# fujii-team/Henbun

Hardware: AMD Instinct MI355X
Metric: elbo_samples_per_sec (higher is better)
Workload: dtype f32; 1 GPU; cfg2 SVGP ELBO step: 1-D UnitRBF, N=1e6, M=512 inducing, minibatch 8192 per GPU, diag Normal q(u), diagonal residual, Adam lr 1e-3; global_batch=8192, per_gpu_batch=8192, parallelism=dp1, N=1000000, M=512, dp_exchange=none, dp_ranks=1, contraction=native, tri_pack=False

## Files before the change

henbun_amd/_lib.py:

```python
from __future__ import annotations

import ctypes
import os
from ctypes import c_char_p, c_double, c_int, c_long, c_uint64, c_void_p

_HERE = os.path.dirname(os.path.abspath(__file__))
LIB_PATH = os.path.join(_HERE, "libhenbun_hip.so")


class HipBackendError(RuntimeError):
    """A libhenbun_hip.so entry point returned a non-zero status."""


P, L, I, D, U64 = c_void_p, c_long, c_int, c_double, c_uint64

_SIGS = {
    "hb_version": [],
    "hb_debug_set": [c_char_p, L],
    "hb_debug_clear": [],
    "hb_cholesky_inverse_ws_elems": [L, L, I],
    "hb_cholesky_persistent_shape": [L, L, I],
    "hb_mlp2_sample_supported": [L, L, L, L, L, I],
    "hb_mlp2_sample_ws_elems": [L, L, L],
    "hb_mlp2_sample_fwd_f32": [P, P, P, P, P, I, P, P, L, P, P, P, P, L, L, L, P, P],
    "hb_mlp2_sample_bwd_f32": [P, P, P, P, I, P, P, P, P, P, P, P, P, P, L, L, L, P, P],
    "hb_gram_cholesky_inverse_f32": [I, P, L, P, L, L, L, D, P, P, L, L, P, P, P, I, P],
    "hb_last_error_string": [],
    "hb_device_info": [P, I, P],
    "hb_graph_begin_capture": [P],
    "hb_graph_end_capture": [P, P],
    "hb_graph_launch": [P, P],
    "hb_graph_destroy": [P],
    "hb_rng_init": [P, L, U64, U64, P],
    "hb_rng_randint": [P, L, P, L, L, L, P],
    "hb_sgp_ws_elems": [L, L, L, L, L],
    "hb_sgp_strip_path": [L, L, L, L, L, I],
    "hb_sgp_head_units": [L, L, L, L, L, I, I, I, L],
    "hb_sgp_rider_supported": [L, L, L, L, L, I, I, I, L],
    "hb_sgp_predict_ws_elems": [L, L, L, L, L, I, I, I],
    "hb_sgp_predict_cov_ws_elems": [L, L, L, L, I, I],
    "hb_sgp_stats_ws_elems": [L, L, L, L, I],
    "hb_sgp_select_ws_elems": [L, L, L, I],
    "hb_sgp_kgrad_ws_elems": [L, L, L, L],
    "hb_matmul_gauss_units": [L, L, L],
    "hb_matmul_gram_vjp_ok": [L, L, L, L],
    "hb_matmul_gram_vjp_ws_elems": [L, L, L],
    "hb_matmul_gram_vjp_f32": [P, P, P, L, L, L, L, L, L, L, L, L, I, I, P, L, P, L, L, L, P, P, P, P, P],
    "hb_fullrank_one_launch_shape": [L, L],
    "hb_matmul_gauss_f32": [P, L, P, L, P, P, P, P, D, P, P, P, L, L, L, L, P],
    "hb_sgp_rider_begin": [],
    "hb_sgp_rider_pending": [],
    "hb_sgp_rider_flush": [P],
    "hb_sgp_fwd_gauss_f32": [I, I, P, L, P, P, L, P, P, I, P, P, P, L, P, P, P, P, P, L, L, L, L, L, P, P, P, P, D, P, P, P, L, P],
    "hb_ewise_prog_image_bytes": [],
    "hb_ewise_prog_build": [I, P, P, I, P, P, I, P, P, P, I, P, P, P, P],
    "hb_ewise_jit_available": [],
    "hb_ewise_jit_run": [P, P],
    "hb_ewise_jit_destroy": [P],
    "hb_side_push_gather_draw_f32": [I, P, P, P, L, P, L, L, L, P, P, L, P, P],
    "hb_side_push_diag_fwd_f32": [P, P, P, P, L, P, P, P, L, L, L, L, P, P],
    "hb_side_push_diag_bwd_f32": [P, P, P, P, P, P, P, L, L, L, L, P],
    "hb_side_pending": [],
    "hb_side_flush": [P],
    "hb_side_discard": [],
    "hb_chain_begin": [],
    "hb_chain_end": [P],
    "hb_chain_discard": [],
    "hb_chain_source": [P, L],
    "hb_chain_compile_dry": [],
    "hb_comm_available": [],
    "hb_comm_unique_id": [P],
    "hb_comm_init": [P, I, I, P],
    "hb_comm_destroy": [P],
}
_RESTYPES = {"hb_last_error_string": c_char_p, "hb_sgp_ws_elems": c_long, "hb_ewise_prog_image_bytes": c_long,
             "hb_sgp_head_units": c_long, "hb_matmul_gauss_units": c_long, "hb_matmul_gram_vjp_ws_elems": c_long, "hb_cholesky_inverse_ws_elems": c_long, "hb_mlp2_sample_ws_elems": c_long,
             "hb_sgp_predict_ws_elems": c_long, "hb_sgp_predict_cov_ws_elems": c_long,
             "hb_sgp_stats_ws_elems": c_long, "hb_sgp_select_ws_elems": c_long,
             "hb_sgp_kgrad_ws_elems": c_long}

_TYPED = {
    "hb_ewise": [I, I, P, P, I, P, I, P, P, P],
    "hb_ewise_prog": [I, P, P, I, P, P, I, P, P, P, I, P, P],
    "hb_ewise_prog_run": [P, L, I, P],
    "hb_ewise_jit_build": [I, P, P, I, P, P, I, P, P, P, I, P, P, P, P, P, L],
    "hb_ewise_colprog_build": [I, P, P, I, P, P, I, P, P, P, L, L, P, P, L],
    "hb_gauss_ll": [P, P, P, P, L, P, P, P, P, P, L, P],
    "hb_gauss_ll_post": [P, P, P, P, L, P, P, P, P, D, P, P, L, P],
    "hb_gauss_ll_fold": [P, L, P, P, P, P],
    "hb_reduce": [I, P, P, L, L, L, P, L, P],
    "hb_copy_nd": [P, P, P, P, I, P, P],
    "hb_fill": [P, L, D, P],
    "hb_gather_rows": [P, L, L, P, P, L, P, P, P],
    "hb_gather_rows_multi": [I, P, P, P, L, P, P, L, P, P],
    "hb_gather_rows_multi_draw": [I, P, P, P, L, P, L, L, L, P, P, L, P, P],
    "hb_matutil": [P, P, L, L, L, I, L, L, D, P],
    "hb_rng_normal": [P, L, P, L, P],
    "hb_diag_sample_kl_fwd": [P, P, P, P, L, P, P, P, L, L, L, L, P, P],
    "hb_diag_sample_kl_bwd": [P, P, P, P, P, P, P, L, L, L, L, P],
    "hb_fullrank_sample_kl_fwd": [P, P, P, P, L, P, P, P, L, L, I, P, P],
    "hb_fullrank_sample_kl_fwd1": [P, P, P, P, L, P, P, P, L, L, I, P, P, P],
    "hb_fullrank_sample_kl_bwd": [P, P, P, P, P, P, P, L, L, I, P],
    "hb_vec_to_tri": [P, P, L, L, P],
    "hb_tri_to_vec": [P, P, L, L, P],
    "hb_gram_fwd": [I, P, L, P, L, P, L, L, P, L, L, L, L, D, P],
    "hb_gram_bwd": [I, P, L, P, L, P, L, L, P, P, P, P, L, L, L, L, P, P],
    "hb_gram_ell_fold": [P, L, L, L, L, P, P],
    "hb_matmul": [P, P, P, L, L, L, L, L, L, L, L, L, L, I, I, D, D, P, L, I, I, P, L, P],
    "hb_matmul_colsum": [P, P, P, P, L, L, L, L, L, L, P, L, P],
    "hb_cholesky": [P, P, L, L, P, P],
    "hb_cholesky_inverse": [P, P, P, L, L, P, P, P, I, P],
    "hb_trinv": [P, P, L, L, P, P],
    "hb_sgp_A": [I, P, L, P, P, L, P, P, I, P, L, L, L, L, P],
    "hb_sgp_fwd": [I, I, P, L, P, P, L, P, P, I, P, P, P, L, P, P, P, P, P, L, L, L, L, L, P, P],
    "hb_sgp_bwd": [I, I, P, L, P, P, L, P, P, I, P, P, P, P, P, P, P, P, P, P, P, P, P, L, L, L, L, L, P, P],
    "hb_sgp_predict": [I, P, L, P, P, L, P, P, P, P, I, I, D, P, P, L, L, L, L, L, P, P],
    "hb_sgp_predict_cov": [I, P, L, P, P, L, P, P, P, I, I, D, P, L, L, L, L, L, P, P],
    "hb_sgp_stats": [I, P, P, P, P, L, P, P, P, P, P, P, L, L, L, L, P, P],
    "hb_sgp_select": [I, P, P, L, L, L, L, D, P, P, P, P, P, P],
    "hb_sgp_kgrad": [I, P, P, P, P, L, P, P, P, P, L, L, L, L, P, P],
    "hb_adam_step": [P, P, P, P, L, D, D, D, D, D, P, I, P, L, P, P, P],
    "hb_allreduce_sum": [P, L, P, P],
    "hb_dp_pack": [P, P, P, L, P],
}


def declared_symbols():
    names = list(_SIGS)
    for base in _TYPED:
        names += [base + "_f32", base + "_f64"]
    return names


class _Lib:
    def __init__(self, path: str):
        if not os.path.exists(path):
            raise ImportError(
                "henbun_amd: %s is missing.  Build it with `python -m henbun_amd._build` "
                "(hipcc, gfx950).  There is no CPU fallback." % path
            )
        import torch

        self._dll = ctypes.CDLL(path)
        self._fns = {}
        for name, args in _SIGS.items():
            self._bind(name, args, _RESTYPES.get(name, c_int))
        for base, args in _TYPED.items():
            for suf in ("_f32", "_f64"):
                self._bind(base + suf, args, c_int)
        if self.raw("hb_version")() != 2:
            raise ImportError("henbun_amd: ABI version mismatch in " + path)

    def _bind(self, name, args, restype):
        fn = getattr(self._dll, name)
        fn.argtypes = args
        fn.restype = restype
        self._fns[name] = fn

    def raw(self, name):
        return self._fns[name]

    def last_error(self) -> str:
        s = self._fns["hb_last_error_string"]()
        return s.decode() if s else ""

    def call(self, name, *args):
        rc = self._fns[name](*args)
        if rc != 0:
            raise HipBackendError("%s failed (status %d): %s" % (name, rc, self.last_error()))
        return 0


_lib = None


def lib() -> _Lib:
    global _lib
    if _lib is None:
        _lib = _Lib(LIB_PATH)
    return _lib
```

henbun_amd/csrc/adam.hip:

```cpp
#include "common.cuh"
#include "../../include/henbun_hip.h"
#include "chain.cuh"

template <typename T>
__global__ void __launch_bounds__(256) adam_kernel(T* __restrict__ theta, const T* __restrict__ g, T* __restrict__ m,
                                                   T* __restrict__ v, long n, double lr, double b1, double b2,
                                                   double eps, double gscale, long* t, int tick, const int* info,
                                                   long n_info, const T* dpflag, long* fail) {
  hb_adam_body<T>(theta, g, m, v, n, lr, b1, b2, eps, gscale, t, tick, info, n_info, dpflag, fail,
                  (long)blockIdx.x * blockDim.x + threadIdx.x, (long)gridDim.x * blockDim.x, blockIdx.x == 0, gridDim.x == 1);
}

template <typename T>
__global__ void __launch_bounds__(256) adam_vec_kernel(T* __restrict__ theta, const T* __restrict__ g, T* __restrict__ m,
                                                       T* __restrict__ v, long n, double lr, double b1, double b2,
                                                       double eps, double gscale, long* t, const int* info, long n_info,
                                                       const T* dpflag, long* fail) {
  hb_adam_body_vec<T>(theta, g, m, v, n, lr, b1, b2, eps, gscale, t, info, n_info, dpflag, fail,
                      (long)blockIdx.x * blockDim.x + threadIdx.x, (long)gridDim.x * blockDim.x, blockIdx.x == 0);
}

template <typename T>
__global__ void __launch_bounds__(64) adam_tick_kernel(long* t, const int* info, long n_info, const T* dpflag,
                                                       const long* fail) {
  if (adam_step_blocked<T>(t, info, n_info, dpflag, const_cast<long*>(fail), false)) return;
  if (threadIdx.x == 0 && blockIdx.x == 0) t[0] += 1;
}

template <typename T>
static int adam_launch(T* theta, const T* g, T* m, T* v, long n, double lr, double b1, double b2, double eps,
                       double gscale, long* t, int tick, const int* info, long n_info, const T* dpflag, long* fail,
                       hipStream_t stream) {
  HB_REQUIRE(n >= 0, "hb_adam_step: n < 0");
  HB_REQUIRE(theta && g && m && v && t, "hb_adam_step: NULL pointer");
  HB_REQUIRE(n_info >= 0 && (n_info == 0 || info != nullptr), "hb_adam_step: info/n_info");
  int grid = 0;
  if (hb_chain_recording()) {
    if (n > 0 && n <= HB_CHAIN_ADAM_MAX_N) {
      HbChainJob j;
      j.kind = HB_CHAIN_ADAM;
      j.is64 = sizeof(T) == 8;
      j.p[0] = theta, j.p[1] = g, j.p[2] = m, j.p[3] = v, j.p[4] = t, j.p[5] = info, j.p[6] = dpflag, j.p[7] = fail;
      j.l[0] = n, j.l[1] = n_info, j.l[2] = tick;
      j.d[0] = lr, j.d[1] = b1, j.d[2] = b2, j.d[3] = eps, j.d[4] = gscale;
      return hb_chain_push(j, stream);
    }
    const int crc = hb_chain_flush(stream);
    if (crc) return crc;
  }
  if (n > 0) {
    grid = n <= 2048 ? 1 : hb_stream_grid(n, 256);
    constexpr long VEC = 16 / (long)sizeof(T);
    const bool vec = grid > 1 && (((uintptr_t)theta | (uintptr_t)g | (uintptr_t)m | (uintptr_t)v) % 16) == 0;
    if (vec) {
      grid = hb_stream_grid(n / VEC, 256);
      hipLaunchKernelGGL(adam_vec_kernel<T>, dim3(grid), dim3(256), 0, stream, theta, g, m, v, n, lr, b1, b2, eps, gscale, t,
                         info, n_info, dpflag, fail);
      if (grid == 1) grid = 2;
    } else {
      hipLaunchKernelGGL(adam_kernel<T>, dim3(grid), dim3(256), 0, stream, theta, g, m, v, n, lr, b1, b2, eps, gscale, t,
                         tick, info, n_info, dpflag, fail);
    }
    HB_LAUNCH_CHECK();
  }
  if (grid != 1 && tick) {
    hipLaunchKernelGGL(adam_tick_kernel<T>, dim3(1), dim3(64), 0, stream, t, info, n_info, dpflag, fail);
    HB_LAUNCH_CHECK();
  }
  return 0;
}

extern "C" int hb_adam_step_f32(float* theta, const float* g, float* m, float* v, long n, double lr, double b1,
                                double b2, double eps, double gscale, long* t, int tick, const int* info, long n_info,
                                const float* dpflag, long* fail, void* stream) {
  return adam_launch<float>(theta, g, m, v, n, lr, b1, b2, eps, gscale, t, tick, info, n_info, dpflag, fail,
                            (hipStream_t)stream);
}
extern "C" int hb_adam_step_f64(double* theta, const double* g, double* m, double* v, long n, double lr, double b1,
                                double b2, double eps, double gscale, long* t, int tick, const int* info, long n_info,
                                const double* dpflag, long* fail, void* stream) {
  return adam_launch<double>(theta, g, m, v, n, lr, b1, b2, eps, gscale, t, tick, info, n_info, dpflag, fail,
                             (hipStream_t)stream);
}
```

henbun_amd/csrc/chain.cuh:

```cuda
#ifndef HB_CHAIN_CUH
#define HB_CHAIN_CUH
#include "common.cuh"
#include "ew_prog.cuh"

enum { HB_CHAIN_PROG = 1, HB_CHAIN_ADAM = 2, HB_CHAIN_GLL = 3, HB_CHAIN_SGP_FINISH = 4, HB_CHAIN_GRAM_ELL = 5, HB_CHAIN_GLL_FOLD = 6 };
#define HB_CHAIN_MAX_JOBS 6
#define HB_CHAIN_PROG_MAX_N 4096
#define HB_CHAIN_FINISH_MAX_N 512
#define HB_CHAIN_GLL_MAX_N 4096
#define HB_CHAIN_ADAM_MAX_N 4096
#define HB_CHAIN_ELL_MAX_N 16384
#define HB_CHAIN_GLL_FOLD_MAX_N 4096

struct HbChainJob {
  int kind = 0, is64 = 0;
  const void* p[HB_PROG_MAX_IN + HB_PROG_MAX_OUT] = {};
  long l[8] = {};
  double d[8] = {};
  ProgArgs prog;
  int reduces = 0;
};

bool hb_chain_recording();
int hb_chain_push(const HbChainJob& job, hipStream_t stream);
int hb_chain_flush(hipStream_t stream);

#endif
```

henbun_amd/csrc/chain_bodies.cuh:

```cuda
#ifndef HB_CHAIN_BODIES_CUH
#define HB_CHAIN_BODIES_CUH

#pragma clang fp contract(off)

template <typename T>
__device__ __forceinline__ int adam_step_blocked(const long* t, const int* info, long n_info, const T* dpflag,
                                                 long* fail, bool record) {
  int bad = 0, what = 0;
  if (fail != nullptr && fail[0] != 0) bad = 1;
  if (dpflag != nullptr && dpflag[0] != (T)0) { bad = 1; what = -1; }
  for (long i = threadIdx.x; i < n_info; i += blockDim.x) {
    const int w = info[i];
    if (w != 0) { bad = 1; what = w; }
  }
  const int any = __syncthreads_or(bad);
  if (any && record && fail != nullptr) {
    __shared__ int who;
    if (threadIdx.x == 0) who = blockDim.x;
    __syncthreads();
    if (what != 0) atomicMin(&who, (int)threadIdx.x);
    __syncthreads();
    const int writer = who == (int)blockDim.x ? 0 : who;
    if ((int)threadIdx.x == writer && fail[0] == 0) {
      fail[1] = (long)what;
      fail[0] = t[0] + 1;
    }
  }
  return any;
}

template <typename T>
__device__ __forceinline__ void hb_adam_body(T* __restrict__ theta, const T* __restrict__ g, T* __restrict__ m, T* __restrict__ v,
                                             long n, double lr, double b1, double b2, double eps, double gscale, long* t,
                                             int tick, const int* info, long n_info, const T* dpflag, long* fail, long i0,
                                             long stride, bool record, bool owner) {
  constexpr int U = 8;
  T g0[U], m0[U], v0[U], th0[U];
#pragma unroll
  for (int k = 0; k < U; ++k) {
    const long i = i0 + k * stride, ic = i < n ? i : (n > 0 ? n - 1 : 0);
    g0[k] = g[ic], m0[k] = m[ic], v0[k] = v[ic], th0[k] = theta[ic];
  }
  const long tnow = t[0];
  if (adam_step_blocked<T>(t, info, n_info, dpflag, fail, record)) return;
  const double tt = (double)(tnow + 1);
  const T lr_t = (T)(lr * sqrt(1.0 - pow(b2, tt)) / (1.0 - pow(b1, tt)));
  const T c1 = (T)b1, c2 = (T)b2, d1 = (T)(1.0 - b1), d2 = (T)(1.0 - b2), e = (T)eps, gs = (T)gscale;
#pragma unroll
  for (int k = 0; k < U; ++k) {
    const long i = i0 + k * stride;
    if (i < n) {
      const T gi = g0[k] * gs;
      const T mi = c1 * m0[k] + d1 * gi;
      const T vi = c2 * v0[k] + d2 * gi * gi;
      m[i] = mi;
      v[i] = vi;
      theta[i] = th0[k] - lr_t * mi / (hb_sqrt(vi) + e);
    }
  }
  for (long i = i0 + U * stride; i < n; i += stride) {
    const T gi = g[i] * gs;
    const T mi = c1 * m[i] + d1 * gi;
    const T vi = c2 * v[i] + d2 * gi * gi;
    m[i] = mi;
    v[i] = vi;
    theta[i] -= lr_t * mi / (hb_sqrt(vi) + e);
  }
  if (owner && tick) {
    __syncthreads();
    if (threadIdx.x == 0) t[0] += 1;
  }
}

template <typename T>
__device__ __forceinline__ void hb_adam_body_vec(T* __restrict__ theta, const T* __restrict__ g, T* __restrict__ m, T* __restrict__ v,
                                                 long n, double lr, double b1, double b2, double eps, double gscale, long* t,
                                                 const int* info, long n_info, const T* dpflag, long* fail, long i0, long stride,
                                                 bool record) {
  constexpr int VEC = 16 / (int)sizeof(T), U = 2;
  typedef T VT __attribute__((ext_vector_type(VEC)));
  const long nv = n / VEC;
  VT g0[U], m0[U], v0[U], th0[U];
#pragma unroll
  for (int k = 0; k < U; ++k) {
    const long i = i0 + k * stride, ic = i < nv ? i : (nv > 0 ? nv - 1 : 0);
    g0[k] = reinterpret_cast<const VT*>(g)[ic], m0[k] = reinterpret_cast<const VT*>(m)[ic];
    v0[k] = reinterpret_cast<const VT*>(v)[ic], th0[k] = reinterpret_cast<const VT*>(theta)[ic];
  }
  const long tnow = t[0];
  if (adam_step_blocked<T>(t, info, n_info, dpflag, fail, record)) return;
  const double tt = (double)(tnow + 1);
  const T lr_t = (T)(lr * sqrt(1.0 - pow(b2, tt)) / (1.0 - pow(b1, tt)));
  const T c1 = (T)b1, c2 = (T)b2, d1 = (T)(1.0 - b1), d2 = (T)(1.0 - b2), e = (T)eps, gs = (T)gscale;
  auto upd = [&](VT gv, VT mv, VT vv, VT tv, long i) {
    VT mo, vo, to;
#pragma unroll
    for (int q = 0; q < VEC; ++q) {
      const T gi = gv[q] * gs;
      const T mi = c1 * mv[q] + d1 * gi;
      const T vi = c2 * vv[q] + d2 * gi * gi;
      mo[q] = mi, vo[q] = vi, to[q] = tv[q] - lr_t * mi / (hb_sqrt(vi) + e);
    }
    reinterpret_cast<VT*>(m)[i] = mo;
    reinterpret_cast<VT*>(v)[i] = vo;
    reinterpret_cast<VT*>(theta)[i] = to;
  };
#pragma unroll
  for (int k = 0; k < U; ++k) {
    const long i = i0 + k * stride;
    if (i < nv) upd(g0[k], m0[k], v0[k], th0[k], i);
  }
  for (long i = i0 + U * stride; i < nv; i += stride)
    upd(reinterpret_cast<const VT*>(g)[i], reinterpret_cast<const VT*>(m)[i], reinterpret_cast<const VT*>(v)[i],
        reinterpret_cast<const VT*>(theta)[i], i);
  const long it = nv * VEC + i0;
  if (it < n) {
    const T gi = g[it] * gs;
    const T mi = c1 * m[it] + d1 * gi;
    const T vi = c2 * v[it] + d2 * gi * gi;
    m[it] = mi;
    v[it] = vi;
    theta[it] -= lr_t * mi / (hb_sqrt(vi) + e);
  }
}

template <typename T>
__device__ __forceinline__ void hb_gauss_ll_single_body(const T* __restrict__ x, const T* __restrict__ f, const T* __restrict__ scale,
                                                        const T* __restrict__ var, long n, T* __restrict__ dmu, T* __restrict__ ll,
                                                        T* __restrict__ dscale, T* __restrict__ dvar, T* smem,
                                                        T* __restrict__ fbar = nullptr, T post = T(0)) {
  constexpr int PER = 16;
  const T s = scale ? scale[0] : T(1), v = var[0];
  const T iv = T(1) / v, lc = T(-0.91893853320467274178) - T(0.5) * hb_log(v);
  T xv[PER], fv[PER];
#pragma unroll
  for (int q = 0; q < PER; ++q) {
    const long j = q * 1024 + threadIdx.x;
    const long jc = j < n ? j : n - 1;
    xv[q] = x[jc];
    fv[q] = f[jc];
  }
  T all = T(0), asc = T(0), avr = T(0);
#pragma unroll
  for (int q = 0; q < PER; ++q) {
    const long j = q * 1024 + threadIdx.x;
    const T dlt = xv[q] - fv[q] * s;
    const T g = dlt * iv;
    if (j < n) {
      dmu[j] = g;
      if (fbar) fbar[j] = s * (post * g);
      all += lc - T(0.5) * dlt * g;
      asc += g * fv[q];
      avr += T(-0.5) * iv + T(0.5) * g * g;
    }
  }
  all = block_sum(all, smem);
  asc = block_sum(asc, smem);
  avr = block_sum(avr, smem);
  if (threadIdx.x == 0) {
    ll[0] = all;
    dscale[0] = asc;
    dvar[0] = avr;
  }
}

template <typename T>
__device__ __forceinline__ void hb_gauss_point(T xv, T fv, T s, T iv, T lc, T& g, T& all, T& asc, T& avr) {
  const T dlt = xv - fv * s;
  g = dlt * iv;
  all += lc - T(0.5) * dlt * g;
  asc += g * fv;
  avr += T(-0.5) * iv + T(0.5) * g * g;
}

template <typename T>
__device__ __forceinline__ void hb_gauss_fold_body(const T* __restrict__ partial, long nb, T* __restrict__ ll, T* __restrict__ dscale,
                                                   T* __restrict__ dvar, T* smem) {
  T a0 = T(0), a1 = T(0), a2 = T(0);
  for (long i = threadIdx.x; i < nb; i += blockDim.x) {
    a0 += partial[i];
    a1 += partial[nb + i];
    a2 += partial[2 * nb + i];
  }
  a0 = block_sum(a0, smem);
  a1 = block_sum(a1, smem);
  a2 = block_sum(a2, smem);
  if (threadIdx.x == 0) {
    ll[0] = a0;
    dscale[0] = a1;
    dvar[0] = a2;
  }
}

template <typename T>
__device__ __forceinline__ void sgp_finish_one(const T* __restrict__ part, int gy, long idx, T epsv, T* __restrict__ f,
                                               T* __restrict__ v, T* __restrict__ eps_out, long n, long P, int diagonal) {
  const long e = idx / n, j = idx - e * n;
  const T* pp = part + e * gy * 5 * n + j;
  T s = T(0);
  for (int y = 0; y < gy; ++y) s += pp[(long)y * 5 * n];
  const T vv = T(1) - s;
  v[idx] = vv;
  if (eps_out) eps_out[idx] = epsv;
  const T scale = diagonal ? hb_sqrt(hb_abs(vv)) * epsv : T(0);
  for (long p = 0; p < P; ++p) {
    T mean = T(0);
    for (int y = 0; y < gy; ++y) mean += pp[((long)y * 5 + 1 + p) * n];
    f[(e * P + p) * n + j] = mean + scale;
  }
}

template <typename T>
__device__ __forceinline__ void hb_sgp_finish_body(const T* __restrict__ part, int gy, const T* __restrict__ eps_in, uint64_t* rng,
                                                   long nlanes, T* __restrict__ eps_out, T* __restrict__ f, T* __restrict__ v,
                                                   long total, long n, long P, int diagonal, long t0, long nthreads) {
  const long npairs = (total + 1) / 2;
  if (rng) {
    const long nact = nlanes < npairs ? nlanes : npairs;
    for (long t = t0; t < nact; t += nthreads) {
      HbRng g = rng_load(rng, nlanes, t);
      for (long p = t; p < npairs; p += nlanes) {
        T z0, z1;
        g.normal2(z0, z1);
        sgp_finish_one<T>(part, gy, 2 * p, z0, f, v, eps_out, n, P, diagonal);
        if (2 * p + 1 < total) sgp_finish_one<T>(part, gy, 2 * p + 1, z1, f, v, eps_out, n, P, diagonal);
      }
      rng_store(rng, nlanes, t, g);
    }
  } else {
    for (long idx = t0; idx < total; idx += nthreads)
      sgp_finish_one<T>(part, gy, idx, eps_in ? eps_in[idx] : T(0), f, v, (eps_out != eps_in) ? eps_out : nullptr, n, P, diagonal);
  }
}

template <typename T>
__device__ __forceinline__ void hb_gram_ell_body(const T* __restrict__ partial, long rows, long d, long dl, long c,
                                                 T* __restrict__ ellbar, T* smem) {
  T acc = T(0);
  if (dl == 1) {
#pragma unroll 4
    for (long t = threadIdx.x; t < rows * d; t += blockDim.x) acc += partial[t];
  } else {
#pragma unroll 4
    for (long r = threadIdx.x; r < rows; r += blockDim.x) acc += partial[r * d + c];
  }
  acc = block_sum(acc, smem);
  if (threadIdx.x == 0) ellbar[c] = acc;
}

#pragma clang fp contract(fast)
#endif
```

henbun_amd/csrc/elementwise.hip:

```cpp
#include "common.cuh"
#include "rng_pairs.cuh"
#include "side_jobs.cuh"
#include <string.h>
#include "../../include/henbun_hip.h"

struct EwArgs {
  int ndim;
  int nin, nout;
  int op;
  long n;
  int shape[HB_MAX_DIMS];
  long istride[4][HB_MAX_DIMS];
  const void* in[4];
  void* out[3];
  double p[4];
};

#include "ew_apply.cuh"

template <typename T>
__global__ void __launch_bounds__(256) ew_kernel(EwArgs A) {
  const long stride = (long)gridDim.x * blockDim.x;
  for (long i = (long)blockIdx.x * blockDim.x + threadIdx.x; i < A.n; i += stride) {
    long off[4] = {0, 0, 0, 0};
// ... 487 lines not shown
    A.shape[d] = 1;
    A.is[d] = A.os[d] = 0;
  }
  A.ndim = nd;
  A.n = n;
  hipLaunchKernelGGL(copy_nd_kernel<T>, dim3(hb_stream_grid(n, 256)), dim3(256), 0, stream, in, out, A);
  HB_LAUNCH_CHECK();
  return 0;
}

extern "C" int hb_copy_nd_f32(const float* in, const long* istr, float* out, const long* ostr, int ndim,
                              const long* shape, void* stream) {
  return copy_nd_launch<float>(in, istr, out, ostr, ndim, shape, (hipStream_t)stream);
}
extern "C" int hb_copy_nd_f64(const double* in, const long* istr, double* out, const long* ostr, int ndim,
                              const long* shape, void* stream) {
  return copy_nd_launch<double>(in, istr, out, ostr, ndim, shape, (hipStream_t)stream);
}

template <typename T>
__global__ void __launch_bounds__(256) fill_kernel(T* out, long n, T v) {
  const long stride = (long)gridDim.x * blockDim.x;
  for (long i = (long)blockIdx.x * blockDim.x + threadIdx.x; i < n; i += stride) out[i] = v;
}
extern "C" int hb_fill_f32(float* out, long n, double v, void* stream) {
  if (n <= 0) return 0;
  hipLaunchKernelGGL(fill_kernel<float>, dim3(hb_stream_grid(n, 256)), dim3(256), 0, (hipStream_t)stream, out, n, (float)v);
  HB_LAUNCH_CHECK();
  return 0;
}
extern "C" int hb_fill_f64(double* out, long n, double v, void* stream) {
  if (n <= 0) return 0;
  hipLaunchKernelGGL(fill_kernel<double>, dim3(hb_stream_grid(n, 256)), dim3(256), 0, (hipStream_t)stream, out, n, v);
  HB_LAUNCH_CHECK();
  return 0;
}

template <typename T>
__global__ void __launch_bounds__(256) gather_rows_kernel(const T* __restrict__ src, const long* __restrict__ idx,
                                                          const long* __restrict__ perm, T* __restrict__ dst,
                                                          long n, long row, long nsrc, int* __restrict__ err) {
  const long total = n * row;
  const long stride = (long)gridDim.x * blockDim.x;
  for (long i = (long)blockIdx.x * blockDim.x + threadIdx.x; i < total; i += stride) {
    const long r = i / row, c = i - r * row;
    long j = idx[r];
    if (perm) j = perm[j];
    if (j < 0 || j >= nsrc) {
      if (err) *err = 1;
      dst[i] = T(0);
    } else {
      dst[i] = src[j * row + c];
    }
  }
}
extern "C" int hb_gather_rows_f32(const float* src, long nsrc, long row, const long* idx, const long* perm, long n,
                                  float* dst, int* err, void* stream) {
  HB_REQUIRE(n >= 0 && row >= 0 && nsrc >= 0, "hb_gather_rows: negative extent");
  if (n * row == 0) return 0;
  hipLaunchKernelGGL(gather_rows_kernel<float>, dim3(hb_stream_grid(n * row, 256)), dim3(256), 0, (hipStream_t)stream,
                     src, idx, perm, dst, n, row, nsrc, err);
  HB_LAUNCH_CHECK();
  return 0;
}
extern "C" int hb_gather_rows_f64(const double* src, long nsrc, long row, const long* idx, const long* perm, long n,
                                  double* dst, int* err, void* stream) {
  HB_REQUIRE(n >= 0 && row >= 0 && nsrc >= 0, "hb_gather_rows: negative extent");
  if (n * row == 0) return 0;
  hipLaunchKernelGGL(gather_rows_kernel<double>, dim3(hb_stream_grid(n * row, 256)), dim3(256), 0,
                     (hipStream_t)stream, src, idx, perm, dst, n, row, nsrc, err);
  HB_LAUNCH_CHECK();
  return 0;
}

template <typename T>
__global__ void __launch_bounds__(256) gather_rows_multi_kernel(GatherMultiArgs<T> g, const long* __restrict__ idx,
                                                                const long* __restrict__ perm, long n, long nsrc,
                                                                int* __restrict__ err) {
  const long total = g.start[g.narr];
  const long stride = (long)gridDim.x * blockDim.x;
  for (long i = (long)blockIdx.x * blockDim.x + threadIdx.x; i < total; i += stride) {
    int a = 0;
#pragma unroll
    for (int q = 1; q < HB_GATHER_MAX; ++q)
      if (q < g.narr && i >= g.start[q]) a = q;
    const long li = i - g.start[a];
    const long r = li / g.row[a], c = li - r * g.row[a];
    long j = idx[r];
    if (perm) j = perm[j];
    if (j < 0 || j >= nsrc) {
      if (err) *err = 1;
      g.dst[a][li] = T(0);
    } else {
      g.dst[a][li] = g.src[a][j * g.row[a] + c];
    }
  }
}
template <typename T>
static int gather_rows_multi(int narr, const T* const* srcs, const long* rows, T* const* dsts, long nsrc,
                             const long* idx, const long* perm, long n, int* err, hipStream_t stream) {
  HB_REQUIRE(narr >= 1 && narr <= HB_GATHER_MAX, "hb_gather_rows_multi: %d arrays (max %d)", narr, HB_GATHER_MAX);
  HB_REQUIRE(n >= 0 && nsrc >= 0 && srcs && rows && dsts && idx, "hb_gather_rows_multi: bad arguments");
  GatherMultiArgs<T> g;
  g.narr = narr;
  g.start[0] = 0;
  for (int a = 0; a < HB_GATHER_MAX; ++a) {
    g.src[a] = a < narr ? srcs[a] : nullptr;
    g.dst[a] = a < narr ? dsts[a] : nullptr;
    g.row[a] = a < narr ? rows[a] : 1;
    if (a < narr) HB_REQUIRE(rows[a] >= 1 && srcs[a] && dsts[a], "hb_gather_rows_multi: bad array %d", a);
    g.start[a + 1] = g.start[a] + (a < narr ? n * rows[a] : 0);
  }
  if (g.start[narr] == 0) return 0;
  hipLaunchKernelGGL(gather_rows_multi_kernel<T>, dim3(hb_stream_grid(g.start[narr], 256)), dim3(256), 0, stream, g, idx,
                     perm, n, nsrc, err);
  HB_LAUNCH_CHECK();
  return 0;
}
extern "C" int hb_gather_rows_multi_f32(int narr, const float* const* srcs, const long* rows, float* const* dsts,
                                        long nsrc, const long* idx, const long* perm, long n, int* err, void* stream) {
  return gather_rows_multi<float>(narr, srcs, rows, dsts, nsrc, idx, perm, n, err, (hipStream_t)stream);
}
extern "C" int hb_gather_rows_multi_f64(int narr, const double* const* srcs, const long* rows, double* const* dsts,
                                        long nsrc, const long* idx, const long* perm, long n, int* err, void* stream) {
  return gather_rows_multi<double>(narr, srcs, rows, dsts, nsrc, idx, perm, n, err, (hipStream_t)stream);
}

template <typename T, int G>
__global__ void __launch_bounds__(256) gather_rows_multi_draw_kernel(GatherMultiArgs<T> g, uint64_t* __restrict__ state,
                                                                     long nlanes, long lo, uint64_t range,
                                                                     long* __restrict__ idx_out,
                                                                     const long* __restrict__ perm, long n, long nsrc,
                                                                     int* __restrict__ err) {
  gather_draw_body<T>(g, state, nlanes, lo, range, idx_out, perm, n, nsrc, err, G, (long)blockIdx.x);
}
template <typename T>
static int gather_rows_multi_draw(int narr, const T* const* srcs, const long* rows, T* const* dsts, long nsrc,
                                  uint64_t* state, long nlanes, long lo, long hi, long* idx_out, const long* perm,
                                  long n, int* err, hipStream_t stream, bool defer = false) {
  HB_REQUIRE(narr >= 1 && narr <= HB_GATHER_MAX, "hb_gather_rows_multi_draw: %d arrays (max %d)", narr, HB_GATHER_MAX);
  HB_REQUIRE(n >= 0 && nsrc >= 0 && srcs && rows && dsts && state && idx_out, "hb_gather_rows_multi_draw: bad arguments");
  HB_REQUIRE(n <= nlanes, "hb_gather_rows_multi_draw: n=%ld exceeds the %ld RNG lanes (draw with hb_rng_randint instead)", n,
             nlanes);
  HB_REQUIRE(hi > lo, "hb_gather_rows_multi_draw: empty range [%ld,%ld)", lo, hi);
  GatherMultiArgs<T> g;
  g.narr = narr;
  g.start[0] = 0;
  long wmax = 1;
  for (int a = 0; a < HB_GATHER_MAX; ++a) {
    g.src[a] = a < narr ? srcs[a] : nullptr;
    g.dst[a] = a < narr ? dsts[a] : nullptr;
    g.row[a] = a < narr ? rows[a] : 1;
    if (a < narr) HB_REQUIRE(rows[a] >= 1 && srcs[a] && dsts[a], "hb_gather_rows_multi_draw: bad array %d", a);
    if (a < narr && rows[a] > wmax) wmax = rows[a];
    g.start[a + 1] = g.start[a] + (a < narr ? n * rows[a] : 0);
  }
  if (n == 0) return 0;
  const uint64_t range = (uint64_t)(hi - lo);
  constexpr long VEC = 16 / (long)sizeof(T);
  bool vec16 = true;
  for (int a = 0; a < narr; ++a)
    vec16 = vec16 && rows[a] % VEC == 0 && ((uintptr_t)srcs[a] % 16) == 0 && ((uintptr_t)dsts[a] % 16) == 0;
  const long wsel = vec16 ? wmax / VEC : wmax;
  const int Gsel = wsel <= 2 ? 1 : (wsel <= 8 ? 4 : (wsel <= 32 ? 16 : 64));
  if constexpr (sizeof(T) == 4) {
    if (defer) {
      HbSideJob j;
      j.kind = HB_SIDE_GATHER_DRAW;
      j.gather.G = vec16 ? -Gsel : Gsel;
      j.nblocks = hb_cdiv(n * Gsel, 256);
      if (j.nblocks <= 1024) {
        memcpy(&j.gather.g, &g, sizeof(g));
        j.gather.state = state; j.gather.nlanes = nlanes; j.gather.lo = lo; j.gather.range = range;
        j.gather.idx_out = idx_out; j.gather.perm = perm; j.gather.n = n; j.gather.nsrc = nsrc; j.gather.err = err;
        return hb_side_push(j, stream);
      }
    }
  }
#define HB_GDRAW(G_)                                                                                                   \
  hipLaunchKernelGGL((gather_rows_multi_draw_kernel<T, G_>), dim3((unsigned)hb_cdiv(n * (G_ < 0 ? -(G_) : (G_)), 256)), dim3(256), 0, \
                     stream, g, state, nlanes, lo, range, idx_out, perm, n, nsrc, err)
  if (vec16) {
    if (Gsel == 1)
      HB_GDRAW(-1);
    else if (Gsel == 4)
      HB_GDRAW(-4);
    else if (Gsel == 16)
      HB_GDRAW(-16);
    else
      HB_GDRAW(-64);
  } else if (Gsel == 1)
    HB_GDRAW(1);
  else if (Gsel == 4)
    HB_GDRAW(4);
  else if (Gsel == 16)
    HB_GDRAW(16);
  else
    HB_GDRAW(64);
#undef HB_GDRAW
  HB_LAUNCH_CHECK();
  return 0;
}
extern "C" int hb_gather_rows_multi_draw_f32(int narr, const float* const* srcs, const long* rows, float* const* dsts,
                                             long nsrc, uint64_t* state, long nlanes, long lo, long hi, long* idx_out,
                                             const long* perm, long n, int* err, void* stream) {
  return gather_rows_multi_draw<float>(narr, srcs, rows, dsts, nsrc, state, nlanes, lo, hi, idx_out, perm, n, err,
                                       (hipStream_t)stream);
}
extern "C" int hb_side_push_gather_draw_f32(int narr, const float* const* srcs, const long* rows, float* const* dsts, long nsrc,
                                           uint64_t* state, long nlanes, long lo, long hi, long* idx_out, const long* perm,
                                           long n, int* err, void* stream) {
  return gather_rows_multi_draw<float>(narr, srcs, rows, dsts, nsrc, state, nlanes, lo, hi, idx_out, perm, n, err,
                                       (hipStream_t)stream, true);
}
extern "C" int hb_gather_rows_multi_draw_f64(int narr, const double* const* srcs, const long* rows, double* const* dsts,
                                             long nsrc, uint64_t* state, long nlanes, long lo, long hi, long* idx_out,
                                             const long* perm, long n, int* err, void* stream) {
  return gather_rows_multi_draw<double>(narr, srcs, rows, dsts, nsrc, state, nlanes, lo, hi, idx_out, perm, n, err,
                                        (hipStream_t)stream);
}

#define HB_GLL_BLOCK_ELEMS 1024
template <typename T>
__global__ void __launch_bounds__(256) gauss_ll_kernel(const T* __restrict__ x, const T* __restrict__ f,
                                                       const T* __restrict__ scale, const T* __restrict__ var,
                                                       long n, T* __restrict__ dmu, T* __restrict__ partial,
                                                       T* __restrict__ fbar, T post) {
  __shared__ T smem[16];
  const T s = scale ? scale[0] : T(1), v = var[0];
  const T iv = T(1) / v, lc = T(-0.91893853320467274178) - T(0.5) * hb_log(v);
  T all = T(0), asc = T(0), avr = T(0);
  const long base = (long)blockIdx.x * HB_GLL_BLOCK_ELEMS;
#pragma unroll
  for (int q = 0; q < HB_GLL_BLOCK_ELEMS / 256; ++q) {
    const long j = base + q * 256 + threadIdx.x;
    const long jc = j < n ? j : n - 1;
    const T xv = x[jc], fv = f[jc];
    const T dlt = xv - fv * s;
    const T g = dlt * iv;
    if (j < n) {
      dmu[j] = g;
      if (fbar) fbar[j] = s * (post * g);
      all += lc - T(0.5) * dlt * g;
      asc += g * fv;
      avr += T(-0.5) * iv + T(0.5) * g * g;
    }
  }
  all = block_sum(all, smem);
  asc = block_sum(asc, smem);
  avr = block_sum(avr, smem);
  if (threadIdx.x == 0) {
    partial[blockIdx.x] = all;
    partial[gridDim.x + blockIdx.x] = asc;
    partial[2 * gridDim.x + blockIdx.x] = avr;
  }
}
template <typename T>
__global__ void __launch_bounds__(256) gauss_ll_finish_kernel(const T* __restrict__ partial, int nb, T* __restrict__ ll,
                                                              T* __restrict__ dscale, T* __restrict__ dvar) {
  __shared__ T smem[16];
  T a0 = T(0), a1 = T(0), a2 = T(0);
  for (int i = threadIdx.x; i < nb; i += 256) {
    a0 += partial[i];
    a1 += partial[nb + i];
    a2 += partial[2 * nb + i];
  }
  a0 = block_sum(a0, smem);
  a1 = block_sum(a1, smem);
  a2 = block_sum(a2, smem);
  if (threadIdx.x == 0) {
    ll[0] = a0;
    dscale[0] = a1;
    dvar[0] = a2;
  }
}
#define HB_GLL_SINGLE_N 16384
template <typename T>
__global__ void __launch_bounds__(1024) gauss_ll_single_kernel(const T* __restrict__ x, const T* __restrict__ f,
                                                               const T* __restrict__ scale, const T* __restrict__ var,
                                                               long n, T* __restrict__ dmu, T* __restrict__ ll,
                                                               T* __restrict__ dscale, T* __restrict__ dvar,
                                                               T* __restrict__ fbar, T post) {
  __shared__ T smem[16];
  static_assert(HB_GLL_SINGLE_N == 16 * 1024, "hb_gauss_ll_single_body: 16 elements per thread of a 1024-thread workgroup");
  hb_gauss_ll_single_body<T>(x, f, scale, var, n, dmu, ll, dscale, dvar, smem, fbar, post);
}

template <typename T>
static int gauss_ll(const T* x, const T* f, const T* scale, const T* var, long n, T* ll, T* dmu, T* dscale, T* dvar,
                    T* ws, long ws_elems, hipStream_t stream, double post = 0.0, T* fbar = nullptr) {
  HB_REQUIRE(n >= 0 && x && f && var && ll && dmu && dscale && dvar && ws, "hb_gauss_ll: bad arguments");
  const int nb = n > 0 ? hb_cdiv(n, HB_GLL_BLOCK_ELEMS) : 0;
  HB_REQUIRE(ws_elems >= 3L * (nb > 0 ? nb : 1), "hb_gauss_ll: workspace of 3*ceil(n/%d) elements required",
             HB_GLL_BLOCK_ELEMS);
  if (hb_chain_recording()) {
    if (n > 0 && n <= HB_CHAIN_GLL_MAX_N) {
      HbChainJob j;
      j.kind = HB_CHAIN_GLL;
      j.is64 = sizeof(T) == 8;
      j.p[0] = x, j.p[1] = f, j.p[2] = scale, j.p[3] = var, j.p[4] = dmu, j.p[5] = ll, j.p[6] = dscale, j.p[7] = dvar;
      j.p[8] = fbar;
      j.l[0] = n;
      j.d[0] = post;
      return hb_chain_push(j, stream);
    }
    const int crc = hb_chain_flush(stream);
    if (crc) return crc;
  }
  if (n > 0 && n <= HB_GLL_SINGLE_N) {
    hipLaunchKernelGGL(gauss_ll_single_kernel<T>, dim3(1), dim3(1024), 0, stream, x, f, scale, var, n, dmu, ll, dscale,
                       dvar, fbar, (T)post);
    HB_LAUNCH_CHECK();
    return 0;
  }
  if (nb > 0) {
    hipLaunchKernelGGL(gauss_ll_kernel<T>, dim3(nb), dim3(256), 0, stream, x, f, scale, var, n, dmu, ws, fbar, (T)post);
    HB_LAUNCH_CHECK();
  }
  hipLaunchKernelGGL(gauss_ll_finish_kernel<T>, dim3(1), dim3(256), 0, stream, ws, nb, ll, dscale, dvar);
  HB_LAUNCH_CHECK();
  return 0;
}
extern "C" int hb_gauss_ll_f32(const float* x, const float* f, const float* scale, const float* var, long n, float* ll,
                               float* dmu, float* dscale, float* dvar, float* ws, long ws_elems, void* stream) {
  return gauss_ll<float>(x, f, scale, var, n, ll, dmu, dscale, dvar, ws, ws_elems, (hipStream_t)stream);
}
extern "C" int hb_gauss_ll_f64(const double* x, const double* f, const double* scale, const double* var, long n,
                               double* ll, double* dmu, double* dscale, double* dvar, double* ws, long ws_elems,
                               void* stream) {
  return gauss_ll<double>(x, f, scale, var, n, ll, dmu, dscale, dvar, ws, ws_elems, (hipStream_t)stream);
}
template <typename T>
__global__ void __launch_bounds__(256) gauss_fold_kernel(const T* __restrict__ partial, long nb, T* __restrict__ ll,
                                                         T* __restrict__ dscale, T* __restrict__ dvar) {
  __shared__ T smem[16];
  hb_gauss_fold_body<T>(partial, nb, ll, dscale, dvar, smem);
}
template <typename T>
static int gauss_fold(const T* partial, long nb, T* ll, T* dscale, T* dvar, hipStream_t stream) {
  HB_REQUIRE(partial && nb >= 1 && ll && dscale && dvar, "hb_gauss_ll_fold: bad arguments");
  if (hb_chain_recording()) {
    if (nb <= HB_CHAIN_GLL_FOLD_MAX_N) {
      HbChainJob j;
      j.kind = HB_CHAIN_GLL_FOLD;
      j.is64 = sizeof(T) == 8;
      j.p[0] = partial, j.p[1] = ll, j.p[2] = dscale, j.p[3] = dvar;
      j.l[0] = nb;
      return hb_chain_push(j, stream);
    }
    const int crc = hb_chain_flush(stream);
    if (crc) return crc;
  }
  hipLaunchKernelGGL(gauss_fold_kernel<T>, dim3(1), dim3(256), 0, stream, partial, nb, ll, dscale, dvar);
  HB_LAUNCH_CHECK();
  return 0;
}
extern "C" int hb_gauss_ll_fold_f32(const float* partial, long nb, float* ll, float* dscale, float* dvar, void* stream) {
  return gauss_fold<float>(partial, nb, ll, dscale, dvar, (hipStream_t)stream);
}
extern "C" int hb_gauss_ll_fold_f64(const double* partial, long nb, double* ll, double* dscale, double* dvar, void* stream) {
  return gauss_fold<double>(partial, nb, ll, dscale, dvar, (hipStream_t)stream);
}

extern "C" int hb_gauss_ll_post_f32(const float* x, const float* f, const float* scale, const float* var, long n, float* ll,
                                    float* dmu, float* dscale, float* dvar, double post, float* fbar, float* ws,
                                    long ws_elems, void* stream) {
  HB_REQUIRE(fbar, "hb_gauss_ll_post: fbar is NULL");
  return gauss_ll<float>(x, f, scale, var, n, ll, dmu, dscale, dvar, ws, ws_elems, (hipStream_t)stream, post, fbar);
}
extern "C" int hb_gauss_ll_post_f64(const double* x, const double* f, const double* scale, const double* var, long n,
                                    double* ll, double* dmu, double* dscale, double* dvar, double post, double* fbar,
                                    double* ws, long ws_elems, void* stream) {
  HB_REQUIRE(fbar, "hb_gauss_ll_post: fbar is NULL");
  return gauss_ll<double>(x, f, scale, var, n, ll, dmu, dscale, dvar, ws, ws_elems, (hipStream_t)stream, post, fbar);
}

template <typename T>
__global__ void __launch_bounds__(256) matutil_kernel(const T* __restrict__ in, T* __restrict__ out, long B, long R,
                                                      long C, int mode, long lower, long upper, T alpha) {
  const long total = B * R * C;
  const long stride = (long)gridDim.x * blockDim.x;
  for (long t = (long)blockIdx.x * blockDim.x + threadIdx.x; t < total; t += stride) {
    const long b = t / (R * C);
    const long rem = t - b * R * C;
    const long i = rem / C, j = rem - i * C;
    T v = in[t];
    if (mode == 0) {
      const bool keep = (lower < 0 || i - j <= lower) && (upper < 0 || j - i <= upper);
      v = keep ? v : T(0);
    } else if (mode == 1) {
      if (i == j) v += alpha;
    } else if (mode == 2) {
      v = (i > j) ? v : (i == j ? T(0.5) * v : T(0));
    } else if (mode == 3) {
      v = T(0.5) * (v + in[b * R * C + j * C + i]);
    } else if (mode == 4) {
      v = T(0.5) * (i >= j ? v : in[b * R * C + j * C + i]);
    }
    out[t] = v;
  }
}
template <typename T>
static int matutil_launch(const T* in, T* out, long B, long R, long C, int mode, long lower, long upper, double alpha,
                          hipStream_t stream) {
  HB_REQUIRE(B >= 0 && R >= 0 && C >= 0, "hb_matutil: negative extent");
  HB_REQUIRE(mode >= 0 && mode <= 4, "hb_matutil: bad mode %d", mode);
  HB_REQUIRE((mode != 3 && mode != 4) || (R == C && in != out), "hb_matutil: symmetrise needs square, out-of-place");
  const long n = B * R * C;
  if (n == 0) return 0;
  hipLaunchKernelGGL(matutil_kernel<T>, dim3(hb_stream_grid(n, 256)), dim3(256), 0, stream, in, out, B, R, C, mode,
                     lower, upper, (T)alpha);
  HB_LAUNCH_CHECK();
  return 0;
}
extern "C" int hb_matutil_f32(const float* in, float* out, long B, long R, long C, int mode, long lower, long upper,
                              double alpha, void* stream) {
  return matutil_launch<float>(in, out, B, R, C, mode, lower, upper, alpha, (hipStream_t)stream);
}
extern "C" int hb_matutil_f64(const double* in, double* out, long B, long R, long C, int mode, long lower, long upper,
                              double alpha, void* stream) {
  return matutil_launch<double>(in, out, B, R, C, mode, lower, upper, alpha, (hipStream_t)stream);
}
```

henbun_amd/csrc/gram.hip:

```cpp
#include "common.cuh"
#include "../../include/henbun_hip.h"
#include "chain.cuh"
#include "gram_value.cuh"

template <typename T>
__global__ void __launch_bounds__(256) gram_fwd_kernel(int kind, const T* __restrict__ X, long sX,
                                                       const T* __restrict__ X2, long sX2, const T* __restrict__ ell,
                                                       long sEll, long dl, T* __restrict__ K, long B, long n, long n2,
                                                       long d, T diag_add) {
  const long total = B * n * n2;
  const long stride = (long)gridDim.x * blockDim.x;
  for (long t = (long)blockIdx.x * blockDim.x + threadIdx.x; t < total; t += stride) {
    const long b = t / (n * n2);
    const long rem = t - b * n * n2;
    const long i = rem / n2, j = rem - i * n2;
    const T kv = gram_value<T>(kind, X + b * sX + i * d, X2 + b * sX2 + j * d, ell + b * sEll, dl, d);
    K[t] = (i == j) ? kv + diag_add : kv;
  }
}

template <typename T>
static int gram_fwd(int kind, const T* X, long sX, const T* X2, long sX2, const T* ell, long sEll, long dl, T* K,
                    long B, long n, long n2, long d, double diag_add, hipStream_t stream) {
  HB_REQUIRE(kind >= HB_KERN_RBF && kind <= HB_KERN_SQDIST, "hb_gram_fwd: unknown kernel kind %d", kind);
  HB_REQUIRE(B >= 0 && n >= 0 && n2 >= 0 && d >= 1, "hb_gram_fwd: bad extents");
  HB_REQUIRE(dl == 1 || dl == d, "hb_gram_fwd: lengthscales must have 1 or d=%ld entries, got %ld", d, dl);
  HB_REQUIRE(X && X2 && ell && K, "hb_gram_fwd: NULL pointer");
  const long total = B * n * n2;
  if (total == 0) return 0;
  HB_REQUIRE(sEll == 0 || sEll == dl, "hb_gram_fwd: lengthscale batch stride must be 0 or dl");
  hipLaunchKernelGGL(gram_fwd_kernel<T>, dim3(hb_stream_grid(total, 256)), dim3(256), 0, stream, kind, X, sX, X2, sX2,
                     ell, sEll, dl, K, B, n, n2, d, (T)diag_add);
  HB_LAUNCH_CHECK();
  return 0;
}
extern "C" int hb_gram_fwd_f32(int kind, const float* X, long sX, const float* X2, long sX2, const float* ell,
                               long sEll, long dl, float* K, long B, long n, long n2, long d, double diag_add,
                               void* stream) {
  return gram_fwd<float>(kind, X, sX, X2, sX2, ell, sEll, dl, K, B, n, n2, d, diag_add, (hipStream_t)stream);
}
extern "C" int hb_gram_fwd_f64(int kind, const double* X, long sX, const double* X2, long sX2, const double* ell,
                               long sEll, long dl, double* K, long B, long n, long n2, long d, double diag_add,
                               void* stream) {
  return gram_fwd<double>(kind, X, sX, X2, sX2, ell, sEll, dl, K, B, n, n2, d, diag_add, (hipStream_t)stream);
}

#define HB_GRAM_MAXD 8

template <typename T>
__global__ void __launch_bounds__(256)
gram_bwd_side_kernel(int kind, int side, const T* __restrict__ X, long sX, const T* __restrict__ X2, long sX2,
                     const T* __restrict__ ell, long sEll, long dl, const T* __restrict__ Kbar, T* __restrict__ out,
                     T* __restrict__ ell_partial, long n, long n2, long d) {
  __shared__ T smem[16];
  const long b = blockIdx.y;
  const long row = blockIdx.x;
  ell += b * sEll;
  const long nother = side != 1 ? n2 : n;
  T ilv[HB_GRAM_MAXD];
  for (long k0 = 0; k0 < d; k0 += HB_GRAM_MAXD) {
#pragma unroll
    for (int k = 0; k < HB_GRAM_MAXD; ++k) ilv[k] = k0 + k < d ? T(1) / ell[dl == 1 ? 0 : k0 + k] : T(0);
    T gacc[HB_GRAM_MAXD], lacc[HB_GRAM_MAXD];
#pragma unroll
    for (int k = 0; k < HB_GRAM_MAXD; ++k) gacc[k] = lacc[k] = T(0);
#pragma unroll 4
    for (long o = threadIdx.x; o < nother; o += blockDim.x) {
      const long i = side != 1 ? row : o;
      const long j = side != 1 ? o : row;
      const T* xi = X + b * sX + i * d;
      const T* xj = X2 + b * sX2 + j * d;
      T r2 = T(0), r2m = T(0);
      for (long k = 0; k < d; ++k) {
        const T il = (d <= HB_GRAM_MAXD) ? ilv[k] : T(1) / ell[dl == 1 ? 0 : k];
        const T a = xi[k] * il, bb = xj[k] * il;
        r2 += (a - bb) * (a - bb);
        r2m += (a + bb) * (a + bb);
      }
      const T kb = Kbar[(b * n + i) * n2 + j];
      const T km = kind == HB_KERN_SQDIST ? T(-2) : hb_exp(T(-0.5) * r2);
      const T kp = kind == HB_KERN_CSYM_RBF ? hb_exp(T(-0.5) * r2m) : T(0);
      const T em = kb * km, ep = kb * kp;
      const T kbg = side == 2 ? kb + Kbar[(b * n + j) * n2 + i] : (side == 3 ? kb + kb : kb);
      const T gm = kbg * km, gp = kbg * kp;
#pragma unroll
      for (int k = 0; k < HB_GRAM_MAXD; ++k) {
        if (k0 + k < d) {
          const T il = ilv[k];
          const T a = xi[k0 + k] * il, bb = xj[k0 + k] * il;
          const T dm = a - bb, dp = a + bb;
          if (side != 1)
            gacc[k] += (-dm * gm - dp * gp) * il;
          else
            gacc[k] += (dm * gm - dp * gp) * il;
          lacc[k] += (dm * dm * em + dp * dp * ep) * il;
        }
      }
    }
#pragma unroll
    for (int k = 0; k < HB_GRAM_MAXD; ++k) {
      if (k0 + k < d) {
        const T g = block_sum(gacc[k], smem);
        if (out && threadIdx.x == 0) out[(b * (side != 1 ? n : n2) + row) * d + k0 + k] = g;
        if (ell_partial) {
          const T l = block_sum(lacc[k], smem);
          if (threadIdx.x == 0) ell_partial[(b * (side != 1 ? n : n2) + row) * d + k0 + k] = l;
        }
      }
    }
  }
}

template <typename T>
__global__ void __launch_bounds__(256) gram_ell_finish_kernel(const T* __restrict__ partial, long rows, long d, long dl,
                                                              T* __restrict__ ellbar) {
  __shared__ T smem[16];
  hb_gram_ell_body<T>(partial + (long)blockIdx.y * rows * d, rows, d, dl, (long)blockIdx.x, ellbar + (long)blockIdx.y * dl, smem);
}

template <typename T>
static int gram_bwd(int kind_flags, const T* X, long sX, const T* X2, long sX2, const T* ell, long sEll, long dl,
                    const T* Kbar, T* Xbar, T* X2bar, T* ellbar, long B, long n, long n2, long d, T* ws,
                    hipStream_t stream) {
  const int kind = kind_flags & ~HB_KERN_KBAR_SYMMETRIC;
  HB_REQUIRE(kind >= HB_KERN_RBF && kind <= HB_KERN_SQDIST, "hb_gram_bwd: unknown kernel kind %d", kind);
  HB_REQUIRE(B >= 0 && n >= 0 && n2 >= 0 && d >= 1, "hb_gram_bwd: bad extents");
  HB_REQUIRE(dl == 1 || dl == d, "hb_gram_bwd: lengthscales must have 1 or d entries");
  HB_REQUIRE(sEll == 0 || sEll == dl, "hb_gram_bwd: lengthscale batch stride must be 0 or dl");
  HB_REQUIRE(X && X2 && ell && Kbar, "hb_gram_bwd: NULL pointer");
  HB_REQUIRE(!ellbar || ws, "hb_gram_bwd: ellbar needs workspace");
  HB_REQUIRE(B <= 65535, "hb_gram_bwd: batch too large");
  if (B == 0) return 0;
  if (hb_chain_recording()) {
    const int crc = hb_chain_flush(stream);
    if (crc) return crc;
  }
  if (n == 0 || n2 == 0) {
    if (Xbar && n > 0) HB_HIP(hb_zero_async(Xbar, sizeof(T) * B * n * d, stream));
    if (X2bar && n2 > 0) HB_HIP(hb_zero_async(X2bar, sizeof(T) * B * n2 * d, stream));
    if (ellbar) HB_HIP(hb_zero_async(ellbar, sizeof(T) * dl * (sEll != 0 ? B : 1), stream));
    return 0;
  }
  const bool sym = Xbar && X2bar == Xbar;
  const bool kbar_sym = (kind_flags & HB_KERN_KBAR_SYMMETRIC) != 0;
  HB_REQUIRE(!kbar_sym || sym, "hb_gram_bwd: HB_KERN_KBAR_SYMMETRIC only applies to the one-pass form (X2 == X, X2bar == Xbar)");
  HB_REQUIRE(!sym || (X == X2 && sX == sX2 && n == n2), "hb_gram_bwd: Xbar == X2bar requires X2 == X");
  if (Xbar || ellbar) {
    hipLaunchKernelGGL(gram_bwd_side_kernel<T>, dim3(n, B), dim3(256), 0, stream, kind, sym ? (kbar_sym ? 3 : 2) : 0, X, sX, X2, sX2, ell, sEll,
                       dl, Kbar, Xbar, ellbar ? ws : (T*)nullptr, n, n2, d);
    HB_LAUNCH_CHECK();
    if (ellbar) {
      const long rows_ = sEll != 0 ? n : B * n, groups_ = sEll != 0 ? B : 1;
      if (hb_chain_recording() && rows_ * d * groups_ <= HB_CHAIN_ELL_MAX_N && groups_ * dl <= 16 && !(X2bar && !sym)) {
        HbChainJob j;
        j.kind = HB_CHAIN_GRAM_ELL;
        j.is64 = sizeof(T) == 8;
        j.p[0] = ws, j.p[1] = ellbar;
        j.l[0] = rows_, j.l[1] = d, j.l[2] = dl, j.l[3] = groups_;
        return hb_chain_push(j, stream);
      }
      if (sEll != 0)
        hipLaunchKernelGGL(gram_ell_finish_kernel<T>, dim3(dl, B), dim3(256), 0, stream, ws, n, d, dl, ellbar);
      else
        hipLaunchKernelGGL(gram_ell_finish_kernel<T>, dim3(dl, 1), dim3(256), 0, stream, ws, B * n, d, dl, ellbar);
      HB_LAUNCH_CHECK();
    }
  }
  if (X2bar && !sym) {
    hipLaunchKernelGGL(gram_bwd_side_kernel<T>, dim3(n2, B), dim3(256), 0, stream, kind, 1, X, sX, X2, sX2, ell, sEll,
                       dl, Kbar, X2bar, (T*)nullptr, n, n2, d);
    HB_LAUNCH_CHECK();
  }
  return 0;
}
template <typename T>
static int gram_ell_fold(const T* partial, long rows, long d, long dl, long groups, T* ellbar, hipStream_t stream) {
  HB_REQUIRE(partial && ellbar && rows >= 1 && d >= 1 && groups >= 1 && (dl == 1 || dl == d), "hb_gram_ell_fold: bad arguments");
  if (hb_chain_recording() && rows * d * groups <= HB_CHAIN_ELL_MAX_N && groups * dl <= 16) {
    HbChainJob j;
    j.kind = HB_CHAIN_GRAM_ELL;
    j.is64 = sizeof(T) == 8;
    j.p[0] = partial, j.p[1] = ellbar;
    j.l[0] = rows, j.l[1] = d, j.l[2] = dl, j.l[3] = groups;
    return hb_chain_push(j, stream);
  }
  if (hb_chain_recording()) {
    const int crc = hb_chain_flush(stream);
    if (crc) return crc;
  }
  hipLaunchKernelGGL(gram_ell_finish_kernel<T>, dim3(dl, groups), dim3(256), 0, stream, partial, rows, d, dl, ellbar);
  HB_LAUNCH_CHECK();
  return 0;
}
extern "C" int hb_gram_ell_fold_f32(const float* partial, long rows, long d, long dl, long groups, float* ellbar, void* stream) {
  return gram_ell_fold<float>(partial, rows, d, dl, groups, ellbar, (hipStream_t)stream);
}
extern "C" int hb_gram_ell_fold_f64(const double* partial, long rows, long d, long dl, long groups, double* ellbar, void* stream) {
  return gram_ell_fold<double>(partial, rows, d, dl, groups, ellbar, (hipStream_t)stream);
}

extern "C" int hb_gram_bwd_f32(int kind, const float* X, long sX, const float* X2, long sX2, const float* ell,
                               long sEll, long dl, const float* Kbar, float* Xbar, float* X2bar, float* ellbar,
                               long B, long n, long n2, long d, float* ws, void* stream) {
  return gram_bwd<float>(kind, X, sX, X2, sX2, ell, sEll, dl, Kbar, Xbar, X2bar, ellbar, B, n, n2, d, ws,
                         (hipStream_t)stream);
}
extern "C" int hb_gram_bwd_f64(int kind, const double* X, long sX, const double* X2, long sX2, const double* ell,
                               long sEll, long dl, const double* Kbar, double* Xbar, double* X2bar, double* ellbar,
                               long B, long n, long n2, long d, double* ws, void* stream) {
  return gram_bwd<double>(kind, X, sX, X2, sX2, ell, sEll, dl, Kbar, Xbar, X2bar, ellbar, B, n, n2, d, ws,
                          (hipStream_t)stream);
}
```

henbun_amd/csrc/jit.hip:

```cpp
#include "common.cuh"
#include "../../include/henbun_hip.h"
#include "ew_prog.cuh"
#include "chain.cuh"
#include <dlfcn.h>
#include <stdarg.h>
#include <stdio.h>
#include <string.h>
#include <hip/hiprtc.h>
#include <map>
#include <mutex>
#include <string>
#include <vector>
#include "_gen/ew_jit_prelude.inc"

namespace {

struct Rtc {
  bool ok = false;
  hiprtcResult (*create)(hiprtcProgram*, const char*, const char*, int, const char**, const char**) = nullptr;
  hiprtcResult (*compile)(hiprtcProgram, int, const char**) = nullptr;
  hiprtcResult (*log_size)(hiprtcProgram, size_t*) = nullptr;
  hiprtcResult (*log)(hiprtcProgram, char*) = nullptr;
  hiprtcResult (*code_size)(hiprtcProgram, size_t*) = nullptr;
  hiprtcResult (*code)(hiprtcProgram, char*) = nullptr;
  hiprtcResult (*destroy)(hiprtcProgram*) = nullptr;
};

Rtc load_rtc() {
  Rtc r;
  void* h = nullptr;
  for (const char* name : {"libhiprtc.so", "libhiprtc.so.7", "/opt/rocm/lib/libhiprtc.so"}) {
    h = dlopen(name, RTLD_NOW | RTLD_LOCAL);
    if (h) break;
  }
  if (!h) return r;
#define HB_RTC_SYM(field, sym)                                   \
  r.field = reinterpret_cast<decltype(r.field)>(dlsym(h, sym)); \
  if (!r.field) return r;
  HB_RTC_SYM(create, "hiprtcCreateProgram")
  HB_RTC_SYM(compile, "hiprtcCompileProgram")
  HB_RTC_SYM(log_size, "hiprtcGetProgramLogSize")
  HB_RTC_SYM(log, "hiprtcGetProgramLog")
  HB_RTC_SYM(code_size, "hiprtcGetCodeSize")
  HB_RTC_SYM(code, "hiprtcGetCode")
  HB_RTC_SYM(destroy, "hiprtcDestroyProgram")
#undef HB_RTC_SYM
  r.ok = true;
  return r;
}
const Rtc& rtc() {
  static const Rtc r = load_rtc();
  return r;
}

struct Compiled {
  hipModule_t module = nullptr;
  hipFunction_t fn = nullptr;
};
std::mutex g_mu;
std::map<std::string, Compiled> g_cache;

struct JitProgram {
  ProgArgs A;
  int reduces = 0, is64 = 0;
  bool colprog = false;
  hipFunction_t fn = nullptr;
  std::vector<void*> ptrs;
  std::vector<void*> argv;
  unsigned grid = 1;
  long n = 0;
};

void appendf(std::string& s, const char* fmt, ...) {
  char buf[512];
  va_list ap;
  va_start(ap, fmt);
  vsnprintf(buf, sizeof(buf), fmt, ap);
  va_end(ap);
  s += buf;
}

std::string literal(double v) {
  char b[64];
  if (v != v)
    snprintf(b, sizeof(b), "__builtin_nan(\"\")");
  else if (v - v != 0.0)
    snprintf(b, sizeof(b), "%s__builtin_inf()", v < 0 ? "-" : "");
  else
    snprintf(b, sizeof(b), "%a", v);
  return b;
}

void emit_program(std::string& s, const ProgArgs& A, const char* loop) {
  for (int k = 0; k < A.nout; ++k)
    if (A.out_reg[k] & HB_PROG_SUM) appendf(s, "  T racc%d = T(0);\n", k);
  appendf(s, "  %s\n", loop);
  s += "    long rem = i;\n";
  for (int d = A.ndim - 1; d >= 0; --d) {
    if (d == 0)
      appendf(s, "    const long x%d = rem;\n", d);
    else
      appendf(s, "    const long x%d = rem %% %dL; rem /= %dL;\n", d, A.shape[d], A.shape[d]);
  }
  int maxreg = A.nin;
  for (int q = 0; q < A.ninstr; ++q) {
    const int top = A.code[q][1] + (A.code[q][0] == HB_EW_GAUSS_LOGPDF_GRAD ? 3 : 1);
    if (top > maxreg) maxreg = top;
  }
  for (int k = 0; k < A.nin; ++k) {
    appendf(s, "    T r%d = in%d[0", k, k);
    for (int d = 0; d < A.ndim; ++d)
      if (A.istr[k][d] != 0) appendf(s, " + x%d * %ldL", d, A.istr[k][d]);
    s += "];\n";
  }
  for (int r = A.nin; r < maxreg; ++r) appendf(s, "    T r%d = T(0);\n", r);
  for (int q = 0; q < A.ninstr; ++q) {
    const int op = A.code[q][0], dst = A.code[q][1];
    const bool grad = op == HB_EW_GAUSS_LOGPDF_GRAD;
    appendf(s, "    { T o0 = T(0), o1 = T(0), o2 = T(0); const double p[2] = {%s, %s};\n", literal(A.params[q][0]).c_str(),
            literal(A.params[q][1]).c_str());
    if (grad)
      appendf(s, "      ew_apply<T>(%d, r%d, r%d, r%d, r%d, p, o0, o1, o2); r%d = o0; r%d = o1; r%d = o2;\n"
                 "      HB_JIT_OPAQUE(r%d); HB_JIT_OPAQUE(r%d); HB_JIT_OPAQUE(r%d); }\n", op,
              (int)A.code[q][2], (int)A.code[q][3], (int)A.code[q][4], (int)A.params[q][0], dst, dst + 1, dst + 2, dst,
              dst + 1, dst + 2);
    else
      appendf(s, "      ew_apply<T>(%d, r%d, r%d, r%d, T(0), p, o0, o1, o2); r%d = o0; HB_JIT_OPAQUE(r%d); }\n", op,
              (int)A.code[q][2], (int)A.code[q][3], (int)A.code[q][4], dst, dst);
  }
  for (int k = 0; k < A.nout; ++k) {
    if (A.out_reg[k] & HB_PROG_SUM) {
      appendf(s, "    racc%d += r%d;\n", k, A.out_reg[k] & (HB_PROG_SUM - 1));
      continue;
    }
    std::string pred, off = "0";
    for (int d = 0; d < A.ndim; ++d) {
      if (A.ostr[k][d] == 0 && A.shape[d] > 1) {
        char b[32];
        snprintf(b, sizeof(b), "%sx%d == 0", pred.empty() ? "" : " && ", d);
        pred += b;
      } else if (A.ostr[k][d] != 0) {
        char b[64];
        snprintf(b, sizeof(b), " + x%d * %ldL", d, A.ostr[k][d]);
        off += b;
      }
    }
    if (pred.empty())
      appendf(s, "    out%d[%s] = r%d;\n", k, off.c_str(), A.out_reg[k]);
    else
      appendf(s, "    if (%s) out%d[%s] = r%d;\n", pred.c_str(), k, off.c_str(), A.out_reg[k]);
  }
  s += "  }\n";
  for (int k = 0; k < A.nout; ++k)
    if (A.out_reg[k] & HB_PROG_SUM)
      appendf(s, "  { const T t = block_sum(racc%d, smem); if (threadIdx.x == 0) out%d[0] = t; }\n", k, k);
}

std::string generate(const ProgArgs& A, const char* T, bool reduces) {
  std::string s = HB_EW_JIT_PRELUDE;
  s += "\n#define HB_JIT_OPAQUE(x) asm volatile(\"\" : \"+v\"(x))";
  appendf(s, "\ntypedef %s T;\nextern \"C\" __global__ void __launch_bounds__(256) hb_jit_kernel(", T);
  for (int k = 0; k < A.nin; ++k) appendf(s, "%sconst T* in%d", k ? ", " : "", k);
  for (int k = 0; k < A.nout; ++k) appendf(s, "%sT* out%d", (A.nin || k) ? ", " : "", k);
  s += ") {\n";
  if (reduces) s += "  __shared__ T smem[16];\n";
  char loop[160];
  snprintf(loop, sizeof(loop), "const long stride = (long)gridDim.x * 256;\n  for (long i = (long)blockIdx.x * 256 + threadIdx.x; i < %ldL; i += stride) {", A.n);
  emit_program(s, A, loop);
  s += "}\n";
  return s;
}

int compile_to_code(const std::string& src, std::vector<char>* code) {
  const Rtc& R = rtc();
  hiprtcProgram prog = nullptr;
  HB_REQUIRE(R.create(&prog, src.c_str(), "hb_jit_kernel.hip", 0, nullptr, nullptr) == HIPRTC_SUCCESS,
             "hb_ewise_jit_build: hiprtcCreateProgram failed");
  const char* opts[] = {"--offload-arch=gfx950", "-O3", "-std=c++17"};
  const hiprtcResult rc = R.compile(prog, 3, opts);
  if (rc != HIPRTC_SUCCESS) {
    size_t ls = 0;
    R.log_size(prog, &ls);
    std::string log(ls + 1, '\0');
    if (ls) R.log(prog, &log[0]);
    R.destroy(&prog);
    HB_REQUIRE(false, "hb_ewise_jit_build: hiprtc compile failed (%d): %.300s", (int)rc, log.c_str());
  }
  size_t cs = 0;
  R.code_size(prog, &cs);
  code->resize(cs);
  R.code(prog, code->data());
  R.destroy(&prog);
  return 0;
}

int compile_source(const std::string& src, Compiled* out) {
  std::lock_guard<std::mutex> lock(g_mu);
  auto it = g_cache.find(src);
  if (it != g_cache.end()) {
    *out = it->second;
    return 0;
  }
  std::vector<char> code;
  int rc = compile_to_code(src, &code);
  if (rc) return rc;
  Compiled c;
  HB_HIP(hipModuleLoadData(&c.module, code.data()));
  HB_HIP(hipModuleGetFunction(&c.fn, c.module, "hb_jit_kernel"));
  g_cache.emplace(src, c);
  *out = c;
  return 0;
}

template <typename T>
int jit_build(int ninstr, const int* code, const double* params, int nin, const void* const* in, const long* istrides,
              int nout, void* const* out, const int* out_regs, const long* ostrides, int ndim, const long* shape,
              void** handle_out, long* n_out, int* reduces_out, char* source_out, long source_cap) {
  HB_REQUIRE(n_out && reduces_out, "hb_ewise_jit_build: NULL pointer");
  HB_REQUIRE(rtc().ok, "hb_ewise_jit_build: hiprtc is not available in this process (see hb_ewise_jit_available)");
  if (handle_out) *handle_out = nullptr;
  ProgArgs A;
  long n = 0;
  int reduces = 0;
  int rc = hb_ewise_prog_build(ninstr, code, params, nin, in, istrides, nout, out, out_regs, ostrides, ndim, shape, &A, &n,
                               &reduces);
  if (rc) return rc;
  *n_out = n;
  *reduces_out = reduces;
  if (n == 0) return 0;
  const std::string src = generate(A, sizeof(T) == 4 ? "float" : "double", reduces != 0);
  if (source_out && source_cap > 0) {
    const size_t skip = sizeof(HB_EW_JIT_PRELUDE) - 1;
    snprintf(source_out, (size_t)source_cap, "%s", src.c_str() + skip);
  }
  if (!handle_out) {
    std::vector<char> code;
    return compile_to_code(src, &code);
  }
  Compiled c;
  rc = compile_source(src, &c);
  if (rc) return rc;
  JitProgram* p = new JitProgram;
  p->A = A;
  p->reduces = reduces;
  p->is64 = sizeof(T) == 8;
  p->fn = c.fn;
  p->n = n;
  p->grid = reduces ? 1u : (unsigned)hb_stream_grid(n, 256);
  for (int k = 0; k < nin; ++k) p->ptrs.push_back(const_cast<void*>(in[k]));
  for (int k = 0; k < nout; ++k) p->ptrs.push_back(out[k]);
  for (size_t k = 0; k < p->ptrs.size(); ++k) p->argv.push_back(&p->ptrs[k]);
  *handle_out = p;
  return 0;
}

constexpr int COLPROG_MAX_ROWS = 16, COLPROG_MAX_INSTR = 64, COLPROG_MAX_IN = 16, COLPROG_MAX_OUT = 16, COLPROG_MAX_REGS = 96;

template <typename T>
int colprog_build(int ninstr, const int* code, const double* params, int nin, const void* const* in, const long* istrides,
                  int nout, void* const* out, const int* out_regs, const long* ostrides, long R, long n, void** handle_out,
                  char* source_out, long source_cap) {
  HB_REQUIRE(rtc().ok, "hb_ewise_colprog_build: hiprtc is not available in this process (see hb_ewise_jit_available)");
  if (handle_out) *handle_out = nullptr;
  HB_REQUIRE(R >= 1 && R <= COLPROG_MAX_ROWS && n >= 0, "hb_ewise_colprog_build: R must be 1..%d, n >= 0", COLPROG_MAX_ROWS);
  HB_REQUIRE(ninstr >= 1 && ninstr <= COLPROG_MAX_INSTR && nin >= 0 && nin <= COLPROG_MAX_IN && nout >= 1 && nout <= COLPROG_MAX_OUT,
             "hb_ewise_colprog_build: program too large (%d instructions, %d inputs, %d outputs)", ninstr, nin, nout);
  HB_REQUIRE(code && params && out && out_regs && ostrides && (nin == 0 || (in && istrides)), "hb_ewise_colprog_build: NULL pointer");
  if (n == 0) return 0;
  int height[COLPROG_MAX_REGS] = {0};
  for (int k = 0; k < nin; ++k) {
    HB_REQUIRE(istrides[2 * k + 1] == 0 || istrides[2 * k + 1] == 1, "hb_ewise_colprog_build: column stride must be 0 or 1");
    HB_REQUIRE(istrides[2 * k] == 0 || istrides[2 * k + 1] == 1, "hb_ewise_colprog_build: a row stride needs column stride 1");
    HB_REQUIRE(handle_out == nullptr || in[k], "hb_ewise_colprog_build: NULL input");
    height[k] = istrides[2 * k] != 0 ? (int)R : 1;
  }
  for (int q = 0; q < ninstr; ++q) {
    const int op = code[5 * q], dst = code[5 * q + 1];
    HB_REQUIRE(dst >= nin && dst < COLPROG_MAX_REGS && height[dst] == 0, "hb_ewise_colprog_build: instruction %d: bad destination %d", q, dst);
    HB_REQUIRE(op != HB_EW_GAUSS_LOGPDF_GRAD && op >= HB_COLPROG_MAX && op < 256, "hb_ewise_colprog_build: instruction %d: op %d", q, op);
    int h = 1;
    const int nops = op < 0 ? 1 : 3;
    for (int j = 0; j < nops; ++j) {
      const int r = code[5 * q + 2 + j];
      if (r < 0 && op >= 0 && j > 0) continue;
      HB_REQUIRE(r >= 0 && r < COLPROG_MAX_REGS && height[r] != 0, "hb_ewise_colprog_build: instruction %d reads undefined register %d", q, r);
      if (height[r] > h) h = height[r];
    }
    height[dst] = op < 0 ? 1 : h;
  }
  for (int k = 0; k < nout; ++k) {
    const int r = out_regs[k];
    HB_REQUIRE(r >= 0 && r < COLPROG_MAX_REGS && height[r] != 0, "hb_ewise_colprog_build: output %d: undefined register %d", k, r);
    HB_REQUIRE(ostrides[2 * k + 1] == 0 || ostrides[2 * k + 1] == 1, "hb_ewise_colprog_build: column stride must be 0 or 1");
    HB_REQUIRE(handle_out == nullptr || out[k], "hb_ewise_colprog_build: NULL output");
  }
  const char* Tn = sizeof(T) == 4 ? "float" : "double";
  std::string s = HB_EW_JIT_PRELUDE;
  s += "\n#define HB_JIT_OPAQUE(x) asm volatile(\"\" : \"+v\"(x))";
  appendf(s, "\ntypedef %s T;\nextern \"C\" __global__ void __launch_bounds__(256) hb_jit_kernel(", Tn);
  for (int k = 0; k < nin; ++k) appendf(s, "%sconst T* __restrict__ in%d", k ? ", " : "", k);
  for (int k = 0; k < nout; ++k) appendf(s, "%sT* __restrict__ out%d", (nin || k) ? ", " : "", k);
  s += ") {\n";
  appendf(s, "  const long stride = (long)gridDim.x * 256;\n  for (long j = (long)blockIdx.x * 256 + threadIdx.x; j < %ldL; j += stride) {\n", n);
  for (int r = 0; r < COLPROG_MAX_REGS; ++r)
    if (height[r]) appendf(s, "    T r%d[%d];\n", r, height[r]);
  for (int k = 0; k < nin; ++k) {
    appendf(s, "#pragma unroll\n    for (int q = 0; q < %d; ++q) r%d[q] = in%d[q * %ldL + j * %ldL];\n", height[k], k, k, istrides[2 * k],
            istrides[2 * k + 1]);
  }
  for (int q = 0; q < ninstr; ++q) {
    const int op = code[5 * q], dst = code[5 * q + 1], a = code[5 * q + 2], b = code[5 * q + 3], c = code[5 * q + 4];
    if (op < 0) {
      appendf(s, "    { T acc = r%d[0];\n", a);
      if (height[a] > 1) {
        if (op == HB_COLPROG_SUM)
          appendf(s, "#pragma unroll\n      for (int q = 1; q < %d; ++q) { acc = acc + r%d[q]; HB_JIT_OPAQUE(acc); }\n", height[a], a);
        else
          appendf(s, "#pragma unroll\n      for (int q = 1; q < %d; ++q) acc = r%d[q] > acc ? r%d[q] : acc;\n", height[a], a, a);
      }
      appendf(s, "      r%d[0] = acc; }\n", dst);
      continue;
    }
    appendf(s, "#pragma unroll\n    for (int q = 0; q < %d; ++q) { T o0 = T(0), o1 = T(0), o2 = T(0); const double p[2] = {%s, %s};\n", height[dst],
            literal(params[2 * q]).c_str(), literal(params[2 * q + 1]).c_str());
    auto operand = [&](int r) {
      char t[32];
      if (r < 0)
        snprintf(t, sizeof(t), "T(0)");
      else
        snprintf(t, sizeof(t), "r%d[%s]", r, height[r] > 1 ? "q" : "0");
      return std::string(t);
    };
    appendf(s, "      ew_apply<T>(%d, %s, %s, %s, T(0), p, o0, o1, o2); r%d[q] = o0; HB_JIT_OPAQUE(r%d[q]); }\n", op, operand(a).c_str(),
            operand(b).c_str(), operand(c).c_str(), dst, dst);
  }
  for (int k = 0; k < nout; ++k) {
    const int r = out_regs[k];
    const long rs = ostrides[2 * k], cs = ostrides[2 * k + 1];
    if (cs == 0) s += "    if (j == 0)\n";
    appendf(s, "#pragma unroll\n    for (int q = 0; q < %d; ++q) out%d[q * %ldL + j * %ldL] = r%d[%s];\n", rs != 0 ? (int)R : 1, k, rs, cs, r,
            height[r] > 1 ? "q" : "0");
  }
  s += "  }\n}\n";
  if (source_out && source_cap > 0) snprintf(source_out, (size_t)source_cap, "%s", s.c_str() + (sizeof(HB_EW_JIT_PRELUDE) - 1));
  if (!handle_out) {
    std::vector<char> co;
    return compile_to_code(s, &co);
  }
  Compiled c;
  const int rc = compile_source(s, &c);
  if (rc) return rc;
  JitProgram* p = new JitProgram;
  p->colprog = true;
  p->is64 = sizeof(T) == 8;
  p->fn = c.fn;
  p->n = n;
  p->grid = (unsigned)hb_stream_grid(n, 256);
  for (int k = 0; k < nin; ++k) p->ptrs.push_back(const_cast<void*>(in[k]));
  for (int k = 0; k < nout; ++k) p->ptrs.push_back(out[k]);
  for (size_t k = 0; k < p->ptrs.size(); ++k) p->argv.push_back(&p->ptrs[k]);
  *handle_out = p;
  return 0;
}

}

extern "C" int hb_ewise_colprog_build_f32(int ninstr, const int* code, const double* params, int nin, const void* const* in,
                                          const long* istrides, int nout, void* const* out, const int* out_regs,
                                          const long* ostrides, long R, long n, void** handle_out, char* source_out,
                                          long source_cap) {
  return colprog_build<float>(ninstr, code, params, nin, in, istrides, nout, out, out_regs, ostrides, R, n, handle_out, source_out,
                              source_cap);
}
extern "C" int hb_ewise_colprog_build_f64(int ninstr, const int* code, const double* params, int nin, const void* const* in,
                                          const long* istrides, int nout, void* const* out, const int* out_regs,
                                          const long* ostrides, long R, long n, void** handle_out, char* source_out,
                                          long source_cap) {
  return colprog_build<double>(ninstr, code, params, nin, in, istrides, nout, out, out_regs, ostrides, R, n, handle_out, source_out,
                               source_cap);
}

extern "C" int hb_ewise_jit_available(void) { return rtc().ok ? 1 : 0; }

extern "C" int hb_ewise_jit_build_f32(int ninstr, const int* code, const double* params, int nin, const void* const* in,
                                      const long* istrides, int nout, void* const* out, const int* out_regs,
                                      const long* ostrides, int ndim, const long* shape, void** handle_out, long* n_out,
                                      int* reduces_out, char* source_out, long source_cap) {
  return jit_build<float>(ninstr, code, params, nin, in, istrides, nout, out, out_regs, ostrides, ndim, shape, handle_out,
                          n_out, reduces_out, source_out, source_cap);
}
extern "C" int hb_ewise_jit_build_f64(int ninstr, const int* code, const double* params, int nin, const void* const* in,
                                      const long* istrides, int nout, void* const* out, const int* out_regs,
                                      const long* ostrides, int ndim, const long* shape, void** handle_out, long* n_out,
                                      int* reduces_out, char* source_out, long source_cap) {
  return jit_build<double>(ninstr, code, params, nin, in, istrides, nout, out, out_regs, ostrides, ndim, shape, handle_out,
                           n_out, reduces_out, source_out, source_cap);
}

namespace {

struct ChainState {
  bool recording = false;
  std::vector<HbChainJob> jobs;
};
thread_local ChainState g_chain;

struct HbChainArgs {
  const void* p[64];
  long l[48];
  double d[16];
};

struct ChainLaunch {
  hipFunction_t fn = nullptr;
};

int chain_source(const std::vector<HbChainJob>& jobs, std::string* out, HbChainArgs* args, int* np_out, int* nl_out, int* nd_out) {
  const bool is64 = jobs[0].is64 != 0;
  std::string s;
  int np = 0, nl = 0, nd = 0;
  auto P = [&](const void* v) { HbChainArgs& a = *args; a.p[np] = v; return np++; };
  auto L = [&](long v) { HbChainArgs& a = *args; a.l[nl] = v; return nl++; };
  auto D = [&](double v) { HbChainArgs& a = *args; a.d[nd] = v; return nd++; };
  for (size_t q = 0; q < jobs.size(); ++q) {
    const HbChainJob& j = jobs[q];
    HB_REQUIRE((j.is64 != 0) == is64, "hb_chain: jobs of different element types in one chain");
    HB_REQUIRE(np + 20 <= 64 && nl + 8 <= 48 && nd + 8 <= 16, "hb_chain: argument block exhausted");
    if (q) s += "  __syncthreads();\n";
    s += "  {\n";
    if (j.kind == HB_CHAIN_PROG) {
      const ProgArgs& G = j.prog;
      for (int k = 0; k < G.nin; ++k) appendf(s, "  const T* in%d = (const T*)A.p[%d];\n", k, P(j.p[k]));
      for (int k = 0; k < G.nout; ++k) appendf(s, "  T* out%d = (T*)A.p[%d];\n", k, P(j.p[G.nin + k]));
      char loop[96];
      snprintf(loop, sizeof(loop), "for (long i = threadIdx.x; i < %ldL; i += 1024) {", G.n);
      emit_program(s, G, loop);
    } else if (j.kind == HB_CHAIN_ADAM) {
      const int p0 = P(j.p[0]); P(j.p[1]); P(j.p[2]); P(j.p[3]); P(j.p[4]); P(j.p[5]); P(j.p[6]); P(j.p[7]);
      const int l0 = L(j.l[0]); L(j.l[1]); L(j.l[2]);
      const int d0 = D(j.d[0]); D(j.d[1]); D(j.d[2]); D(j.d[3]); D(j.d[4]);
      appendf(s, "  hb_adam_body<T>((T*)A.p[%d], (const T*)A.p[%d], (T*)A.p[%d], (T*)A.p[%d], A.l[%d], A.d[%d], A.d[%d], A.d[%d], "
                 "A.d[%d], A.d[%d], (long*)A.p[%d], (int)A.l[%d], (const int*)A.p[%d], A.l[%d], (const T*)A.p[%d], (long*)A.p[%d], "
                 "(long)threadIdx.x, 1024L, true, true);\n",
              p0, p0 + 1, p0 + 2, p0 + 3, l0, d0, d0 + 1, d0 + 2, d0 + 3, d0 + 4, p0 + 4, l0 + 2, p0 + 5, l0 + 1, p0 + 6, p0 + 7);
    } else if (j.kind == HB_CHAIN_GLL) {
      const int p0 = P(j.p[0]); P(j.p[1]); P(j.p[2]); P(j.p[3]); P(j.p[4]); P(j.p[5]); P(j.p[6]); P(j.p[7]); P(j.p[8]);
      const int l0 = L(j.l[0]);
      const int d0 = D(j.d[0]);
      appendf(s, "  hb_gauss_ll_single_body<T>((const T*)A.p[%d], (const T*)A.p[%d], (const T*)A.p[%d], (const T*)A.p[%d], A.l[%d], "
                 "(T*)A.p[%d], (T*)A.p[%d], (T*)A.p[%d], (T*)A.p[%d], smem, (T*)A.p[%d], (T)A.d[%d]);\n",
              p0, p0 + 1, p0 + 2, p0 + 3, l0, p0 + 4, p0 + 5, p0 + 6, p0 + 7, p0 + 8, d0);
    } else if (j.kind == HB_CHAIN_GLL_FOLD) {
      const int p0 = P(j.p[0]); P(j.p[1]); P(j.p[2]); P(j.p[3]);
      const int l0 = L(j.l[0]);
      appendf(s, "  hb_gauss_fold_body<T>((const T*)A.p[%d], A.l[%d], (T*)A.p[%d], (T*)A.p[%d], (T*)A.p[%d], smem);\n", p0, l0, p0 + 1,
              p0 + 2, p0 + 3);
    } else if (j.kind == HB_CHAIN_SGP_FINISH) {
      const int p0 = P(j.p[0]); P(j.p[1]); P(j.p[2]); P(j.p[3]); P(j.p[4]); P(j.p[5]);
      const int l0 = L(j.l[0]); L(j.l[1]); L(j.l[2]); L(j.l[3]); L(j.l[4]); L(j.l[5]);
      appendf(s, "  hb_sgp_finish_body<T>((const T*)A.p[%d], (int)A.l[%d], (const T*)A.p[%d], (uint64_t*)A.p[%d], A.l[%d], (T*)A.p[%d], "
                 "(T*)A.p[%d], (T*)A.p[%d], A.l[%d], A.l[%d], A.l[%d], (int)A.l[%d], (long)threadIdx.x, 1024L);\n",
              p0, l0, p0 + 1, p0 + 2, l0 + 1, p0 + 3, p0 + 4, p0 + 5, l0 + 2, l0 + 3, l0 + 4, l0 + 5);
    } else if (j.kind == HB_CHAIN_GRAM_ELL) {
      const int p0 = P(j.p[0]); P(j.p[1]);
      const int l0 = L(j.l[0]); L(j.l[1]); L(j.l[2]); L(j.l[3]);
      appendf(s, "  for (long grp = 0; grp < A.l[%d]; ++grp)\n    for (long c = 0; c < A.l[%d]; ++c)\n"
                 "      hb_gram_ell_body<T>((const T*)A.p[%d] + grp * A.l[%d] * A.l[%d], A.l[%d], A.l[%d], A.l[%d], c, "
                 "(T*)A.p[%d] + grp * A.l[%d], smem);\n",
              l0 + 3, l0 + 2, p0, l0, l0 + 1, l0, l0 + 1, l0 + 2, p0 + 1, l0 + 2);
    } else {
      HB_REQUIRE(false, "hb_chain: unknown job kind %d", j.kind);
    }
    s += "  }\n";
  }
  s += "}\n";
  std::string h = HB_EW_JIT_PRELUDE;
  h += "\n#define HB_JIT_OPAQUE(x) asm volatile(\"\" : \"+v\"(x))";
  appendf(h, "\nstruct HbChainArgs { const void* p[%d]; long l[%d]; double d[%d]; };", np > 0 ? np : 1, nl > 0 ? nl : 1, nd > 0 ? nd : 1);
  appendf(h, "\ntypedef %s T;\nextern \"C\" __global__ void __launch_bounds__(1024) hb_jit_kernel(const HbChainArgs Ain) {\n",
          is64 ? "double" : "float");
  h += "  __shared__ T smem[16];\n  const HbChainArgs A = Ain;\n";
  *out = h + s;
  *np_out = np, *nl_out = nl, *nd_out = nd;
  return 0;
}

}

bool hb_chain_recording() { return g_chain.recording; }

int hb_chain_flush(hipStream_t stream) {
  if (g_chain.jobs.empty()) return 0;
  std::vector<HbChainJob> jobs;
  jobs.swap(g_chain.jobs);
  std::string src;
  HbChainArgs args = {};
  int np = 0, nl = 0, nd = 0;
  int rc = chain_source(jobs, &src, &args, &np, &nl, &nd);
  if (rc) return rc;
  Compiled c;
  rc = compile_source(src, &c);
  if (rc) return rc;
  unsigned char packed[sizeof(HbChainArgs)];
  const size_t bp = sizeof(void*) * (size_t)(np > 0 ? np : 1), bl = sizeof(long) * (size_t)(nl > 0 ? nl : 1),
               bd = sizeof(double) * (size_t)(nd > 0 ? nd : 1);
  memcpy(packed, args.p, bp);
  memcpy(packed + bp, args.l, bl);
  memcpy(packed + bp + bl, args.d, bd);
  size_t size = bp + bl + bd;
  void* config[] = {HIP_LAUNCH_PARAM_BUFFER_POINTER, packed, HIP_LAUNCH_PARAM_BUFFER_SIZE, &size, HIP_LAUNCH_PARAM_END};
  HB_HIP(hipModuleLaunchKernel(c.fn, 1, 1, 1, 1024, 1, 1, 0, stream, nullptr, config));
  return 0;
}

static void chain_job_slots(const HbChainJob& j, int* p, int* l, int* d) {
  switch (j.kind) {
    case HB_CHAIN_PROG: *p = j.prog.nin + j.prog.nout, *l = 0, *d = 0; break;
    case HB_CHAIN_ADAM: *p = 8, *l = 3, *d = 5; break;
    case HB_CHAIN_GLL: *p = 9, *l = 1, *d = 1; break;
    case HB_CHAIN_GLL_FOLD: *p = 4, *l = 1, *d = 0; break;
    case HB_CHAIN_SGP_FINISH: *p = 6, *l = 6, *d = 0; break;
    case HB_CHAIN_GRAM_ELL: *p = 2, *l = 4, *d = 0; break;
    default: *p = 20, *l = 8, *d = 8; break;
  }
}

int hb_chain_push(const HbChainJob& job, hipStream_t stream) {
  int np = 0, nl = 0, nd = 0;
  for (const HbChainJob& q : g_chain.jobs) {
    int p, l, d;
    chain_job_slots(q, &p, &l, &d);
    np += p, nl += l, nd += d;
  }
  const bool full = np + 20 > 64 || nl + 8 > 48 || nd + 8 > 16;
  if (g_chain.jobs.size() == HB_CHAIN_MAX_JOBS || (!g_chain.jobs.empty() && (g_chain.jobs[0].is64 != job.is64 || full))) {
    const int rc = hb_chain_flush(stream);
    if (rc) return rc;
  }
  g_chain.jobs.push_back(job);
  return 0;
}

extern "C" int hb_chain_begin(void) {
  HB_REQUIRE(!g_chain.recording && g_chain.jobs.empty(), "hb_chain_begin: a chain is already being recorded on this thread");
  g_chain.recording = rtc().ok;
  return 0;
}
extern "C" int hb_chain_end(void* stream) {
  g_chain.recording = false;
  return hb_chain_flush((hipStream_t)stream);
}
extern "C" int hb_chain_discard(void) {
  const int n = (int)g_chain.jobs.size();
  g_chain.jobs.clear();
  g_chain.recording = false;
  return n;
}
extern "C" int hb_chain_source(char* out, long cap) {
  HB_REQUIRE(out && cap > 0, "hb_chain_source: bad buffer");
  out[0] = 0;
  if (g_chain.jobs.empty()) return 0;
  std::string src;
  HbChainArgs args = {};
  int np = 0, nl = 0, nd = 0;
  const int rc = chain_source(g_chain.jobs, &src, &args, &np, &nl, &nd);
  if (rc) return rc;
  snprintf(out, (size_t)cap, "%s", src.c_str() + (sizeof(HB_EW_JIT_PRELUDE) - 1));
  return 0;
}

extern "C" int hb_chain_compile_dry(void) {
  std::vector<HbChainJob> jobs;
  jobs.swap(g_chain.jobs);
  g_chain.recording = false;
  if (jobs.empty()) return 0;
  std::string src;
  HbChainArgs args = {};
  int np = 0, nl = 0, nd = 0;
  int rc = chain_source(jobs, &src, &args, &np, &nl, &nd);
  if (rc) return rc;
  std::vector<char> code;
  return compile_to_code(src, &code);
}

extern "C" int hb_ewise_jit_run(void* handle, void* stream) {
  if (!handle) return 0;
  JitProgram* p = static_cast<JitProgram*>(handle);
  if (hb_chain_recording()) {
    if (p->n <= HB_CHAIN_PROG_MAX_N && !p->colprog) {
      HbChainJob j;
      j.kind = HB_CHAIN_PROG;
      j.is64 = p->is64;
      j.prog = p->A;
      j.reduces = p->reduces;
      for (size_t k = 0; k < p->ptrs.size(); ++k) j.p[k] = p->ptrs[k];
      return hb_chain_push(j, (hipStream_t)stream);
    }
    const int rc = hb_chain_flush((hipStream_t)stream);
    if (rc) return rc;
  }
  HB_HIP(hipModuleLaunchKernel(p->fn, p->grid, 1, 1, 256, 1, 1, 0, (hipStream_t)stream, p->argv.data(), nullptr));
  return 0;
}

extern "C" int hb_ewise_jit_destroy(void* handle) {
  delete static_cast<JitProgram*>(handle);
  return 0;
}
```

henbun_amd/csrc/sgp.hip:

```cpp
#include "common.cuh"
#include "sgp_strip.cuh"
#include "chain.cuh"
#include "chol_persist.cuh"
#include <type_traits>
#include "gemm_tile.cuh"
#include "rng_pairs.cuh"
#include "../../include/henbun_hip.h"

#define SGP_BM 64
#define SGP_BN 128
#define SGP_DREG 4

extern "C" int hb_matmul_f32(const float*, const float*, float*, long, long, long, long, long, long, long, long, long,
                             long, int, int, double, double, const float*, long, int, int, float*, long, void*);
extern "C" int hb_matmul_f64(const double*, const double*, double*, long, long, long, long, long, long, long, long,
                             long, long, int, int, double, double, const double*, long, int, int, double*, long,
                             void*);

template <typename T>
struct SgpArgs {
  const T* x;
  long sx;
  const T* z;
  const T* ell;
// ... 1581 lines not shown
      compute(fa, ts);
      __builtin_amdgcn_sched_barrier(0);
      load(fa, ts + 2);
      __builtin_amdgcn_sched_barrier(0);
      compute(fb, ts + 1);
      __builtin_amdgcn_sched_barrier(0);
    }
  }

  if (a.part) {
#pragma unroll
    for (int q = 0; q < 5; ++q) cs[q] += __shfl_xor(cs[q], 32);
    __syncthreads();
    float* red = reinterpret_cast<float*>(&K3[0][0][0]);
    if (lane < 32) {
#pragma unroll
      for (int q = 0; q < 5; ++q) red[(w * 5 + q) * 32 + lane] = cs[q];
    }
    __syncthreads();
    if (tid < 32 && col0 + tid < n) {
      float* pp = a.part + e * 5 * a.n + col0 + tid;
      for (int q = 0; q < 1 + npart; ++q) {
        float sum = 0.f;
#pragma unroll
        for (int ww = 0; ww < SGP_STRIP_THREADS / 64; ++ww) sum += red[(ww * 5 + q) * 32 + tid];
        pp[(long)q * n] = sum;
      }
    }
  }
}

static inline bool hb_sgp_no_strip() {
  return hb_debug_get("sgp_no_strip", 0) != 0;
}
static inline bool sgp_strip_ok(long E, long n, long M, long d, const void* W) {
  const long tiled_wgs = E * hb_cdiv(n, SGP_BN) * ((hb_cdiv(M, SGP_BM) + 1) / 2);
  const bool force = hb_debug_get("sgp_force_strip", 0) != 0;
  return M >= 32 && M <= SGP_SM_MAX && M % 32 == 0 && d <= SGP_DREG && ((uintptr_t)W % 16 == 0) && (tiled_wgs < 1024 || force);
}

extern "C" int hb_sgp_strip_path(long E, long n, long M, long d, long P, int prec) {
  if (hb_sgp_no_strip()) return 0;
  if (!(M >= 32 && M <= SGP_SM_MAX && M % 32 == 0 && d >= 1 && d <= SGP_DREG && P <= 4 && n > 0 && E >= 1)) return 0;
  if (prec == HB_PREC_BF16X3) return 1;
  const bool old_rule = hb_debug_get("sgp_tiled_crossover", 0) != 0;
  if (!old_rule) return (E * hb_cdiv(n, SGP_SN) <= (1L << 22) && (long)hb_cdiv(n, SGP_SN) * (2 * d + P) <= 31 * M) ? 1 : 0;
  const long tiled_wgs = E * hb_cdiv(n, SGP_BN) * ((hb_cdiv(M, SGP_BM) + 1) / 2);
  return (tiled_wgs < 1024 && E * hb_cdiv(n, SGP_SN) <= 4096) ? 1 : 0;
}

static int sgp_A_strip_launch(SgpArgs<float> a, long E, hipStream_t stream) {
  dim3 grid = sgp_grid(hb_cdiv(a.n, SGP_SN), 1, E, a.efast);
  const bool form3 = (!a.part || a.P <= 1) && hb_debug_get("sgp_strip_form2", 0) == 0;
  static int cus = 0;
  if (cus == 0 && (hb_device_info(nullptr, 0, &cus) || cus <= 0)) cus = 256;
  const bool form16 = a.M >= 384 && a.M % 32 == 0 && E * hb_cdiv(a.n, SGP_SN) <= cus + cus / 4 && hb_debug_get("sgp_form16", 0) != 0;
#define HB_STRIP(D_)                                                                                          \
  do {                                                                                                        \
    if (a.W3)                                                                                                 \
      hipLaunchKernelGGL((sgp_A_strip3_kernel<D_>), grid, dim3(SGP_STRIP_THREADS), 0, stream, a);             \
    else if (a.Wf && form3 && form16)                                                                         \
      hipLaunchKernelGGL((sgp_A_strip16_kernel<D_>), grid, dim3(SGP_S16_THREADS), 0, stream, a);              \
    else if (a.Wf && form3)                                                                                   \
      hipLaunchKernelGGL((sgp_A_strip2t_kernel<D_>), grid, dim3(SGP_STRIP_THREADS), 0, stream, a);            \
    else if (a.Wf)                                                                                            \
      hipLaunchKernelGGL((sgp_A_strip2_kernel<D_>), grid, dim3(SGP_STRIP_THREADS), 0, stream, a);             \
    else                                                                                                      \
      hipLaunchKernelGGL((sgp_A_strip_kernel<D_, false>), grid, dim3(SGP_STRIP_THREADS), 0, stream, a);       \
  } while (0)
  if (a.d == 1)
    HB_STRIP(1);
  else if (a.d == 2)
    HB_STRIP(2);
  else if (a.d == 3)
    HB_STRIP(3);
  else
    HB_STRIP(4);
#undef HB_STRIP
  HB_LAUNCH_CHECK();
  return 0;
}
static int sgp_A_strip_launch(SgpArgs<double>, long, hipStream_t) { return -1; }

template <typename T>
static int sgp_A_launch(const SgpArgs<T>& a, dim3 grid, hipStream_t stream) {
  const bool lds_z = a.d <= SGP_DREG && a.M * a.d <= SGP_ZS_MAX;
  const bool vec = lds_z && a.M % 16 == 0 && ((uintptr_t)a.W % 16 == 0);
#define HB_SGP_A(D_)                                                                          \
  do {                                                                                        \
    if (vec)                                                                                  \
      hipLaunchKernelGGL((sgp_A_kernel<T, D_, true>), grid, dim3(256), 0, stream, a);         \
    else                                                                                      \
      hipLaunchKernelGGL((sgp_A_kernel<T, D_, false>), grid, dim3(256), 0, stream, a);        \
  } while (0)
  if (lds_z && a.d == 1)
    HB_SGP_A(1);
  else if (lds_z && a.d == 2)
    HB_SGP_A(2);
  else if (lds_z && a.d == 3)
    HB_SGP_A(3);
  else if (lds_z && a.d == 4)
    HB_SGP_A(4);
  else
    hipLaunchKernelGGL((sgp_A_kernel<T, 0, false>), grid, dim3(256), 0, stream, a);
#undef HB_SGP_A
  HB_LAUNCH_CHECK();
  return 0;
}

template <typename T>
__global__ void __launch_bounds__(256) sgp_finish_kernel(const T* __restrict__ A, const T* __restrict__ u,
                                                         const T* __restrict__ eps, T* __restrict__ f,
                                                         T* __restrict__ v, long n, long M, long P, int mode) {
  __shared__ T red[5][8][33];
  const long e = blockIdx.y;
  A += e * M * n;
  u += e * P * M;
  f += e * P * n;
  v += e * n;
  if (eps) eps += e * n;
  const int cx = threadIdx.x & 31, ry = threadIdx.x >> 5;
  const long j = (long)blockIdx.x * 32 + cx;
  const bool ok = j < n;
  const long jc = ok ? j : n - 1;
  T scale = T(0);
  for (long p0 = 0; p0 < P || p0 == 0; p0 += 4) {
    const int np = (int)((P - p0) < 4 ? (P - p0) : 4);
    T sq = T(0), mac[4] = {T(0), T(0), T(0), T(0)};
#pragma unroll 4
    for (long m = ry; m < M; m += 8) {
      const T av = A[m * n + jc];
      sq += av * av;
#pragma unroll
      for (int q = 0; q < 4; ++q)
        if (q < np) mac[q] += u[(p0 + q) * M + m] * av;
    }
    red[4][ry][cx] = sq;
#pragma unroll
    for (int q = 0; q < 4; ++q) red[q][ry][cx] = mac[q];
    __syncthreads();
    if (ry == 0 && ok) {
      if (p0 == 0) {
        T ssum = T(0);
#pragma unroll
        for (int q = 0; q < 8; ++q) ssum += red[4][q][cx];
        const T vv = T(1) - ssum;
        v[j] = vv;
        if (mode == HB_SGP_DIAGONAL) scale = hb_sqrt(hb_abs(vv)) * eps[j];
      }
      for (int q = 0; q < np; ++q) {
        T mean = T(0);
#pragma unroll
        for (int w = 0; w < 8; ++w) mean += red[q][w][cx];
        f[(p0 + q) * n + j] = mean + scale;
      }
    }
    __syncthreads();
  }
}

template <typename T>
__global__ void __launch_bounds__(256) sgp_finish_part_kernel(const T* __restrict__ part, int gy,
                                                              const T* __restrict__ eps_in, uint64_t* rng,
                                                              long nlanes, T* __restrict__ eps_out, T* __restrict__ f,
                                                              T* __restrict__ v, long total, long n, long P, int mode) {
  hb_sgp_finish_body<T>(part, gy, eps_in, rng, nlanes, eps_out, f, v, total, n, P, mode == HB_SGP_DIAGONAL,
                        (long)blockIdx.x * blockDim.x + threadIdx.x, (long)gridDim.x * blockDim.x);
}

template <typename T>
__global__ void __launch_bounds__(256) sgp_rng_fill_kernel(uint64_t* state, long nlanes, T* out, long n) {
  const long t = (long)blockIdx.x * blockDim.x + threadIdx.x;
  const long npairs = (n + 1) / 2;
  if (t >= nlanes || t >= npairs) return;
  HbRng g = rng_load(state, nlanes, t);
  for (long p = t; p < npairs; p += nlanes) {
    T z0, z1;
    g.normal2(z0, z1);
    out[2 * p] = (T)z0;
    if (2 * p + 1 < n) out[2 * p + 1] = (T)z1;
  }
  rng_store(state, nlanes, t, g);
}

extern "C" long hb_sgp_ws_elems(long E, long n, long M, long d, long P) {
  (void)P;
  const long gy = (M + SGP_BM - 1) / SGP_BM;
  const long mm = 32 * E * M * M, part = 5 * E * gy * n;
  return E * n + E * M * d + (mm > part ? mm : part);
}

static inline int sgp_grid_y(long E, long n, int nRB) {
  const long paired = (long)hb_cdiv(n, SGP_BN) * ((nRB + 1) / 2) * E;
  return (paired < 384 && nRB > 1) ? nRB : (nRB + 1) / 2;
}

template <typename T>
struct SgpHead {
  const T* y = nullptr;
  const T* scale = nullptr;
  const T* var = nullptr;
  double post = 0.0;
  T* dmu = nullptr;
  T* fbar = nullptr;
  T* part = nullptr;
  long units = 0;
};
static inline bool sgp_fused_finish_ok(long E, long n, long M, long d, long P, int prec, bool has_wfrag, bool draw, long rng_lanes) {
  const bool nofuse = hb_debug_get("sgp_no_fused_finish", 0) != 0 || hb_debug_get("sgp_strip_form2", 0) != 0;
  return !nofuse && has_wfrag && prec == HB_PREC_NATIVE && hb_sgp_strip_path(E, n, M, d, P, prec) && P <= 1 && n % 2 == 0 &&
         (!draw || rng_lanes >= (E * n + 1) / 2);
}
extern "C" long hb_sgp_head_units(long E, long n, long M, long d, long P, int prec, int has_wfrag, int draw, long rng_lanes) {
  if (P != 1 || !sgp_fused_finish_ok(E, n, M, d, P, prec, has_wfrag != 0, draw != 0, rng_lanes)) return 0;
  return E * hb_cdiv(n, SGP_SN);
}

template <typename T>
static int sgp_fwd(int kind, int mode, const T* x, long sx, const T* z, const T* ell, long dl, const T* W, const T* Wf,
                   int prec, const T* u, const T* eps_in, uint64_t* rng, long rng_lanes, T* eps_out, T* A, T* A_frag, T* f,
                   T* v, long E, long n, long M, long d, long P, T* ws, hipStream_t stream, const SgpHead<T>* head = nullptr) {
  HB_REQUIRE(!A_frag || (sizeof(T) == 4 && Wf && ws && hb_sgp_strip_path(E, n, M, d, P, prec)),
             "hb_sgp_fwd: a fragment-major A needs the column-strip form (fp32, Wfrag, hb_sgp_strip_path)");
  if (hb_chain_recording()) {
    const int crc = hb_chain_flush(stream);
    if (crc) return crc;
  }
  HB_REQUIRE(prec == HB_PREC_NATIVE || prec == HB_PREC_BF16X3, "hb_sgp_fwd: unknown precision %d", prec);
  HB_REQUIRE(prec == HB_PREC_NATIVE || (sizeof(T) == 4 && Wf && M % 32 == 0 && M <= SGP_SM_MAX && d <= SGP_DREG && P <= 4 && ws),
             "hb_sgp_fwd: bf16x3 needs fp32, the bf16 images in Wfrag, M %% 32 == 0, M <= %d, d <= %d, P <= 4", SGP_SM_MAX, SGP_DREG);
  HB_REQUIRE(kind == HB_KERN_RBF, "hb_sgp_fwd: only the UnitRBF kernel is fused (kind=%d)", kind);
  HB_REQUIRE(mode == HB_SGP_NEGLECTED || mode == HB_SGP_DIAGONAL, "hb_sgp_fwd: unknown mode %d", mode);
  HB_REQUIRE(E >= 0 && n >= 0 && M >= 0 && d >= 1 && P >= 0, "hb_sgp_fwd: bad extents");
  HB_REQUIRE(dl == 1 || dl == d, "hb_sgp_fwd: lengthscales must have 1 or d entries");
  HB_REQUIRE(x && z && ell && W && u && (A || A_frag) && f && v, "hb_sgp_fwd: NULL pointer");
  HB_REQUIRE(E <= 65535, "hb_sgp_fwd: too many experts");
  HB_REQUIRE(M * n < 2147483647L && M * M < 2147483647L && n * d < 2147483647L, "hb_sgp_fwd: matrix too large for 32-bit indexing");
  if (E * n == 0) return 0;
  const bool draw = mode == HB_SGP_DIAGONAL && !eps_in;
  if (draw) HB_REQUIRE(rng && rng_lanes > 0 && eps_out, "hb_sgp_fwd: need eps_in, or rng and eps_out");
  HB_REQUIRE(!head || (M > 0 && P == 1 && ws && Wf), "hb_sgp_fwd_gauss: needs Wfrag, a workspace and P == 1");
  const int nRB = hb_cdiv(M, SGP_BM);
  const int gy = sgp_grid_y(E, n, nRB);
  if (M > 0 && P <= 4 && ws) {
    SgpArgs<T> a;
    a.x = x; a.sx = sx; a.z = z; a.ell = ell; a.dl = dl; a.W = W; a.Wf = Wf; a.u = u; a.A = A;
    a.n = n; a.M = M; a.d = d; a.P = P;
    a.W3 = prec == HB_PREC_BF16X3 ? (const void*)(Wf + 2 * E * M * M) : nullptr;
    a.plane3 = E * M * M;
    a.Af = A_frag;
    a.part = ws + E * n + E * M * d;
    const bool strip = sizeof(T) == 4 && ((Wf && hb_sgp_strip_path(E, n, M, d, P, prec)) ||
                                          (sgp_strip_ok(E, n, M, d, W) && !hb_sgp_no_strip()));
    const int gyp = strip ? 1 : gy;
    int rc;
    a.fin = 0;
    if (strip) {
      if (sizeof(T) == 4 && sgp_fused_finish_ok(E, n, M, d, P, prec, a.Wf != nullptr && !a.W3, draw, rng_lanes)) {
        a.fin = 1;
        a.fin_diag = mode == HB_SGP_DIAGONAL;
        a.fin_eps_in = mode == HB_SGP_DIAGONAL ? eps_in : (const T*)nullptr;
        a.fin_rng = draw ? rng : (uint64_t*)nullptr;
        a.fin_lanes = rng_lanes;
        a.fin_eps_out = mode == HB_SGP_DIAGONAL ? eps_out : (T*)nullptr;
        a.fin_f = f;
        a.fin_v = v;
        if (head) {
          HB_REQUIRE(P == 1 && head->units == E * hb_cdiv(n, SGP_SN), "hb_sgp_fwd_gauss: units must be hb_sgp_head_units(...)");
          a.head = 1;
          a.hy = head->y, a.hscale = head->scale, a.hvar = head->var;
          a.hdmu = head->dmu, a.hfbar = head->fbar, a.hpost = (T)head->post;
          a.hpart = head->part, a.hunits = head->units;
        }
      }
      HB_REQUIRE(!head || a.fin, "hb_sgp_fwd_gauss: this call cannot carry the head (hb_sgp_head_units(...) == 0)");
      if constexpr (std::is_same<T, float>::value) {
        if (g_rider.armed) {
          HB_REQUIRE(a.fin && !a.W3 && d <= SGP_E_DMAX, "hb_sgp_fwd after hb_sgp_rider_begin: this call cannot ride (hb_sgp_rider_supported)");
          sgp_grid(hb_cdiv(a.n, SGP_SN), 1, E, a.efast);
          g_rider.a = a, g_rider.E = E, g_rider.valid = true, g_rider.armed = false;
          return 0;
        }
      }
      rc = sgp_A_strip_launch(a, E, stream);
      if (rc) return rc;
      if (a.fin) return 0;
    } else {
      dim3 grid = sgp_grid(hb_cdiv(n, SGP_BN), gy, E, a.efast);
      rc = sgp_A_launch<T>(a, grid, stream);
    }
    if (rc) return rc;
    const long total = E * n;
    if (hb_chain_recording() && total <= HB_CHAIN_FINISH_MAX_N) {
      HbChainJob j;
      j.kind = HB_CHAIN_SGP_FINISH;
      j.is64 = sizeof(T) == 8;
      j.p[0] = a.part;
      j.p[1] = mode == HB_SGP_DIAGONAL ? eps_in : (const T*)nullptr;
      j.p[2] = draw ? rng : (uint64_t*)nullptr;
      j.p[3] = mode == HB_SGP_DIAGONAL ? eps_out : (T*)nullptr;
      j.p[4] = f;
      j.p[5] = v;
      j.l[0] = gyp, j.l[1] = rng_lanes, j.l[2] = total, j.l[3] = n, j.l[4] = P, j.l[5] = mode == HB_SGP_DIAGONAL;
      return hb_chain_push(j, stream);
    }
    const int fgrid = draw ? hb_cdiv(rng_lanes, 256) : hb_stream_grid((total + 1) / 2, 256);
    hipLaunchKernelGGL(sgp_finish_part_kernel<T>, dim3(fgrid), dim3(256), 0, stream, a.part, gyp,
                       mode == HB_SGP_DIAGONAL ? eps_in : (const T*)nullptr, draw ? rng : (uint64_t*)nullptr, rng_lanes,
                       mode == HB_SGP_DIAGONAL ? eps_out : (T*)nullptr, f, v, total, n, P, mode);
    HB_LAUNCH_CHECK();
    return 0;
  }
  const T* eps = eps_in;
  if (mode == HB_SGP_DIAGONAL) {
    if (draw) {
      hipLaunchKernelGGL(sgp_rng_fill_kernel<T>, dim3(hb_cdiv(rng_lanes, 256)), dim3(256), 0, stream, rng, rng_lanes,
                         eps_out, E * n);
      HB_LAUNCH_CHECK();
      eps = eps_out;
    } else if (eps_out && eps_out != eps_in) {
      HB_HIP(hb_copy_async(eps_out, eps_in, sizeof(T) * E * n, stream));
    }
  }
  if (M > 0) {
    SgpArgs<T> a;
    a.x = x; a.sx = sx; a.z = z; a.ell = ell; a.dl = dl; a.W = W; a.Wf = nullptr; a.u = u; a.A = A;
    a.n = n; a.M = M; a.d = d; a.P = P;
    a.W3 = nullptr; a.plane3 = 0; a.Af = nullptr;
    a.part = nullptr;
    dim3 grid = sgp_grid(hb_cdiv(n, SGP_BN), gy, E, a.efast);
    int rc = sgp_A_launch<T>(a, grid, stream);
    if (rc) return rc;
  }
  hipLaunchKernelGGL(sgp_finish_kernel<T>, dim3(hb_cdiv(n, 32), (unsigned)E), dim3(256), 0, stream, A, u, eps, f, v, n,
                     M, P, mode);
  HB_LAUNCH_CHECK();
  return 0;
}

template <typename T>
static int sgp_A_only(int kind, const T* x, long sx, const T* z, const T* ell, long dl, const T* W, const T* Wf, int prec,
                      T* A, long E, long n, long M, long d, hipStream_t stream) {
  HB_REQUIRE(prec == HB_PREC_NATIVE || prec == HB_PREC_BF16X3, "hb_sgp_A: unknown precision %d", prec);
  HB_REQUIRE(prec == HB_PREC_NATIVE || (sizeof(T) == 4 && Wf && M % 32 == 0 && M <= SGP_SM_MAX && d <= SGP_DREG),
             "hb_sgp_A: bf16x3 needs fp32, the bf16 images in Wfrag, M %% 32 == 0, M <= %d, d <= %d", SGP_SM_MAX, SGP_DREG);
  HB_REQUIRE(kind == HB_KERN_RBF, "hb_sgp_A: only the UnitRBF kernel is fused (kind=%d)", kind);
  HB_REQUIRE(E >= 0 && n >= 0 && M >= 0 && d >= 1, "hb_sgp_A: bad extents");
  HB_REQUIRE(dl == 1 || dl == d, "hb_sgp_A: lengthscales must have 1 or d entries");
  HB_REQUIRE(x && z && ell && W && A, "hb_sgp_A: NULL pointer");
  HB_REQUIRE(E <= 65535, "hb_sgp_A: too many experts");
  HB_REQUIRE(M * n < 2147483647L && M * M < 2147483647L && n * d < 2147483647L, "hb_sgp_A: matrix too large");
  if (E * n * M == 0) return 0;
  SgpArgs<T> a;
  a.x = x; a.sx = sx; a.z = z; a.ell = ell; a.dl = dl; a.W = W; a.Wf = Wf; a.u = nullptr; a.A = A;
  a.n = n; a.M = M; a.d = d; a.P = 0;
  a.W3 = prec == HB_PREC_BF16X3 ? (const void*)(Wf + 2 * E * M * M) : nullptr;
  a.plane3 = E * M * M;
  a.Af = nullptr;
  a.part = nullptr;
  if (sizeof(T) == 4 && ((sgp_strip_ok(E, n, M, d, W) && !hb_sgp_no_strip()) || prec == HB_PREC_BF16X3))
    return sgp_A_strip_launch(a, E, stream);
  const int nRB = hb_cdiv(M, SGP_BM);
  dim3 grid = sgp_grid(hb_cdiv(n, SGP_BN), sgp_grid_y(E, n, nRB), E, a.efast);
  return sgp_A_launch<T>(a, grid, stream);
}
extern "C" int hb_sgp_A_f32(int kind, const float* x, long sx, const float* z, const float* ell, long dl,
                            const float* W, const float* Wfrag, int prec, float* A, long E, long n, long M, long d,
                            void* stream) {
  return sgp_A_only<float>(kind, x, sx, z, ell, dl, W, Wfrag, prec, A, E, n, M, d, (hipStream_t)stream);
}
extern "C" int hb_sgp_A_f64(int kind, const double* x, long sx, const double* z, const double* ell, long dl,
                            const double* W, const double* Wfrag, int prec, double* A, long E, long n, long M, long d,
                            void* stream) {
  return sgp_A_only<double>(kind, x, sx, z, ell, dl, W, Wfrag, prec, A, E, n, M, d, (hipStream_t)stream);
}

extern "C" int hb_sgp_fwd_f32(int kind, int mode, const float* x, long sx, const float* z, const float* ell, long dl,
                              const float* W, const float* Wfrag, int prec, const float* u, const float* eps_in,
                              uint64_t* rng, long rng_lanes, float* eps_out, float* A, float* A_frag, float* f, float* v,
                              long E, long n, long M, long d, long P, float* ws, void* stream) {
  return sgp_fwd<float>(kind, mode, x, sx, z, ell, dl, W, Wfrag, prec, u, eps_in, rng, rng_lanes, eps_out, A, A_frag, f, v,
                        E, n, M, d, P, ws, (hipStream_t)stream);
}
extern "C" int hb_sgp_fwd_f64(int kind, int mode, const double* x, long sx, const double* z, const double* ell,
                              long dl, const double* W, const double* Wfrag, int prec, const double* u,
                              const double* eps_in, uint64_t* rng, long rng_lanes, double* eps_out, double* A,
                              double* A_frag, double* f, double* v, long E, long n, long M, long d, long P, double* ws,
                              void* stream) {
  return sgp_fwd<double>(kind, mode, x, sx, z, ell, dl, W, Wfrag, prec, u, eps_in, rng, rng_lanes, eps_out, A, A_frag, f,
                         v, E, n, M, d, P, ws, (hipStream_t)stream);
}

extern "C" int hb_sgp_fwd_gauss_f32(int kind, int mode, const float* x, long sx, const float* z, const float* ell, long dl,
                                    const float* W, const float* Wfrag, int prec, const float* u, const float* eps_in,
                                    uint64_t* rng, long rng_lanes, float* eps_out, float* A, float* A_frag, float* f, float* v,
                                    long E, long n, long M, long d, long P, float* ws, const float* y, const float* scale,
                                    const float* var, double post, float* dmu, float* fbar, float* head_part, long units,
                                    void* stream) {
  HB_REQUIRE(y && var && dmu && head_part && units > 0, "hb_sgp_fwd_gauss: NULL pointer");
  SgpHead<float> h;
  h.y = y, h.scale = scale, h.var = var, h.post = post, h.dmu = dmu, h.fbar = fbar, h.part = head_part, h.units = units;
  return sgp_fwd<float>(kind, mode, x, sx, z, ell, dl, W, Wfrag, prec, u, eps_in, rng, rng_lanes, eps_out, A, A_frag, f, v,
                        E, n, M, d, P, ws, (hipStream_t)stream, &h);
}

template <typename T>
__device__ __forceinline__ T sgp_resid_coef(const T* __restrict__ eps, const T* __restrict__ v,
                                            const T* __restrict__ fbar, long n, long P, int mode, long j) {
  if (mode != HB_SGP_DIAGONAL) return T(0);
  T cs = T(0);
  for (long p = 0; p < P; ++p) cs += fbar[p * n + j];
  const T vv = v[j];
  const T av = hb_abs(vv);
  return av > T(0) ? -eps[j] * hb_sign(vv) / hb_sqrt(av) * cs : T(0);
}

template <typename T>
struct SgpBwdArgs {
  const T* W;
  const T* u;
  const T* A;
  const T* fbar;
  const T* eps;
  const T* v;
  T* Kbar;
  long n, M, P;
  int mode;
  long efast;
  const T* x;
  long sx;
  const T* z;
  const T* ell;
  long dl, d;
  const T* WTf;
  const void* WT3;
  long plane3;
  T* part;
  const T* Af;
  T* Kf;
};

template <typename T>
struct SgpRawB {
  T a, u;
};
template <typename T>
struct SgpRawB4 {
  typedef T VT __attribute__((ext_vector_type(16 / sizeof(T))));
  VT a;
  T u;
};

template <typename T, bool FAST>
__global__ void __launch_bounds__(256) sgp_kbar_kernel(SgpBwdArgs<T> a) {
  typedef TileGemm<T, SGP_BM, SGP_BN, 16, 2, 2> G;
  __shared__ __attribute__((aligned(16))) T lds[G::LDS_ELEMS];
  long e;
  int bx;
  sgp_block(a.efast, e, bx);
  const T* W = a.W + e * a.M * a.M;
  const T* u = a.u + e * a.P * a.M;
  const T* A = a.A + e * a.M * a.n;
  const T* fbar = a.fbar + e * a.P * a.n;
  const T* eps = a.eps ? a.eps + e * a.n : nullptr;
  const T* vres = a.v + e * a.n;
  T* Kbar = a.Kbar + e * a.M * a.n;
  const int M = (int)a.M, n = (int)a.n;
  const int col0 = bx * SGP_BN;
  const int nRB = (M + SGP_BM - 1) / SGP_BM;
  const int jcol = col0 + (threadIdx.x % SGP_BN);
  const bool jok = jcol < n;
  const int jc = jok ? jcol : n - 1;
  const int Mm1 = M - 1;
  const T cj = sgp_resid_coef<T>(eps, vres, fbar, a.n, a.P, a.mode, jc);
  const bool preg = a.P == 1;
  const T fb0 = a.P > 0 ? fbar[jc] : T(0);
  constexpr int VECK = TileGemm<T, SGP_BM, SGP_BN, 16, 2, 2>::VEC;
  const int n4 = col0 + (threadIdx.x % (SGP_BN / VECK)) * VECK;
  const int n4c = n4 + VECK <= n ? n4 : (n >= VECK ? n - VECK : 0);
  T c4[VECK], f4[VECK];
#pragma unroll
  for (int q = 0; q < VECK; ++q) {
    const bool ok = FAST && (n4 + q < n);
    c4[q] = ok ? sgp_resid_coef<T>(eps, vres, fbar, a.n, a.P, a.mode, n4 + q) : T(0);
    f4[q] = ok ? fbar[n4 + q] : T(0);
  }

  for (int half = 0; half < 2; ++half) {
    int rb;
    if (!sgp_row_block(half, nRB, rb)) break;
    const int row0 = rb * SGP_BM;
    G g;
    g.zero();
    auto la = [&](int m, int k) -> T {
      const int r = row0 + m;
      return W[k * M + (r < M ? r : Mm1)];
    };
    auto fa = [&](T raw, int m, int k) -> T {
      const int r = row0 + m;
      return ((r < M) & (k >= r)) ? raw : T(0);
    };
    auto lb = [&](int k, int nn) -> SgpRawB<T> {
      SgpRawB<T> r;
      r.a = A[k * n + jc];
      r.u = u[k];
      return r;
    };
    auto fb = [&](SgpRawB<T> raw, int k, int nn) -> T {
      T val = raw.a * cj;
      if (preg) {
        val += raw.u * fb0;
      } else {
        for (long p = 0; p < a.P; ++p) val += u[p * M + k] * fbar[p * n + jc];
      }
      return jok ? val : T(0);
    };
    if constexpr (FAST) {
      typedef typename G::VT VT;
      constexpr int VEC = G::VEC;
      auto la4 = [&](int m, int k) -> VT {
        const int r = row0 + m;
        return *reinterpret_cast<const VT*>(&W[k * M + (r < M ? r : M - VEC)]);
      };
      auto fa4 = [&](VT raw, int m, int k) -> VT {
        VT v;
#pragma unroll
        for (int q = 0; q < VEC; ++q) v[q] = ((row0 + m + q < M) & (k >= row0 + m + q)) ? raw[q] : T(0);
        return v;
      };
      auto lb4 = [&](int k, int nn) -> SgpRawB4<T> {
        SgpRawB4<T> r;
        r.a = *reinterpret_cast<const typename SgpRawB4<T>::VT*>(&A[k * n + n4c]);
        r.u = u[k];
        return r;
      };
      auto fb4 = [&](SgpRawB4<T> raw, int k, int nn) -> VT {
        VT v;
#pragma unroll
        for (int q = 0; q < VEC; ++q) v[q] = raw.a[q] * c4[q] + raw.u * f4[q];
        return v;
      };
      g.template run_vec<HB_MC, HB_MC>(row0, M, la4, fa4, lb4, fb4, lds);
    } else {
      g.template run<false, false>(row0, M, la, fa, lb, fb, lds);
    }
    g.for_each([&](int row, int col, T v) {
      const int r = row0 + row, cc = col0 + col;
      if (r < M && cc < n) Kbar[(long)r * n + cc] = v;
    });
  }
}

__device__ __forceinline__ float hb_half_wave_sum_dpp(float v) {
  auto dpp = [](float x, int ctrl_unused) { return x; };
  (void)dpp;
  int vi;
#define HB_DPP_ADD(CTRL, ROWMASK)                                                                        \
  vi = __builtin_amdgcn_update_dpp(0, __builtin_bit_cast(int, v), CTRL, ROWMASK, 0xF, true);             \
  v += __builtin_bit_cast(float, vi);
  HB_DPP_ADD(0xB1, 0xF)
  HB_DPP_ADD(0x4E, 0xF)
  HB_DPP_ADD(0x141, 0xF)
  HB_DPP_ADD(0x140, 0xF)
  HB_DPP_ADD(0x142, 0xA)
#undef HB_DPP_ADD
  return v;
}

template <int D, bool BF3>
__global__ void __launch_bounds__(SGP_STRIP_THREADS, (BF3 || D >= 3) ? 2 : 4) sgp_kbar_strip_kernel(SgpBwdArgs<float> a) {
  typedef float V4 __attribute__((ext_vector_type(4)));
  typedef __bf16 B8 __attribute__((ext_vector_type(8)));
  typedef Mma<float> MM;
  constexpr int KS_BYTES = BF3 ? 3 * SGP_SN * SGP_S3LD * 2 : SGP_SN * SGP_SLD * 4;
  __shared__ __attribute__((aligned(16))) unsigned char ks_raw[KS_BYTES];
  __shared__ float lred[(SGP_STRIP_THREADS / 64) * D];
  __shared__ __attribute__((aligned(16))) float zs[SGP_SM_MAX * D];
  __shared__ __attribute__((aligned(16))) float xss[SGP_SN * D];
  __shared__ float us[4][SGP_SM_MAX];
  __shared__ float cjs[SGP_SN], fbs[4][SGP_SN];
  float (*Ks)[SGP_SLD] = reinterpret_cast<float (*)[SGP_SLD]>(ks_raw);
  __bf16 (*K3)[SGP_SN][SGP_S3LD] = reinterpret_cast<__bf16 (*)[SGP_SN][SGP_S3LD]>(ks_raw);
  long e;
  int bx;
  sgp_block(a.efast, e, bx);
  const float* __restrict__ x = a.x + e * a.sx;
  const float* __restrict__ z = a.z + e * a.M * D;
  const float* __restrict__ ell = a.ell + e * a.dl;
  const float* __restrict__ A = a.A ? a.A + e * a.M * a.n : nullptr;
  const float* __restrict__ fbar = a.fbar + e * a.P * a.n;
  float* __restrict__ Kbar = a.Kbar ? a.Kbar + e * a.M * a.n : nullptr;
  const int M = (int)a.M, n = (int)a.n, P = (int)a.P;
  const int col0 = bx * SGP_SN, nS = (n + SGP_SN - 1) / SGP_SN;
  const int tid = threadIdx.x, lane = tid & 63, w = __builtin_amdgcn_readfirstlane(tid >> 6), li = lane & 31, h = lane >> 5;
  const int nq = 2 * D + P;
  float* __restrict__ part = a.part + ((e * nS + bx) * (long)nq) * M;

  float sc[D];
#pragma unroll
  for (int dd = 0; dd < D; ++dd) sc[dd] = float(SGP_EXP2_SCALE) / ell[a.dl == 1 ? 0 : dd];
  {
    constexpr int NTH = SGP_STRIP_THREADS;
    constexpr int ZIT = (SGP_SM_MAX * D) / NTH, UIT = SGP_SM_MAX / NTH;
    float zt[ZIT], ut[4][UIT];
#pragma unroll
    for (int it = 0; it < ZIT; ++it) {
// ... 1120 lines not shown
```

include/henbun_hip.h:

```cpp
#ifndef HENBUN_HIP_H
#define HENBUN_HIP_H

#include <stdint.h>

#ifdef __cplusplus
extern "C" {
#endif

#define HB_ABI_VERSION 2

int hb_version(void);
const char* hb_last_error_string(void);
int hb_debug_set(const char* key, long value);
int hb_debug_clear(void);
int hb_device_info(char* buf, int buflen, int* cu_count);

int hb_graph_begin_capture(void* stream);
int hb_graph_end_capture(void* stream, void** exec_out);
int hb_graph_launch(void* exec, void* stream);
int hb_graph_destroy(void* exec);

enum {
  HB_EW_NEG = 1, HB_EW_EXP, HB_EW_LOG, HB_EW_SQRT, HB_EW_SQUARE, HB_EW_ABS, HB_EW_SIGN,
  HB_EW_SIGMOID, HB_EW_RELU, HB_EW_SOFTPLUS, HB_EW_TANH, HB_EW_RECIP, HB_EW_RSQRT,
// ... 14 lines not shown
                 void* const* out, int ndim, const long* shape, const double* params, void* stream);

int hb_gauss_ll_f32(const float* x, const float* f, const float* scale, const float* var, long n, float* ll,
                    float* dmu, float* dscale, float* dvar, float* ws, long ws_elems, void* stream);
int hb_gauss_ll_f64(const double* x, const double* f, const double* scale, const double* var, long n,
                    double* ll, double* dmu, double* dscale, double* dvar, double* ws, long ws_elems,
                    void* stream);
int hb_gauss_ll_post_f32(const float* x, const float* f, const float* scale, const float* var, long n, float* ll,
                         float* dmu, float* dscale, float* dvar, double post, float* fbar, float* ws, long ws_elems,
                         void* stream);
int hb_gauss_ll_post_f64(const double* x, const double* f, const double* scale, const double* var, long n, double* ll,
                         double* dmu, double* dscale, double* dvar, double post, double* fbar, double* ws, long ws_elems,
                         void* stream);

enum { HB_EW_PROG_SUM = 256 };
int hb_ewise_prog_f32(int ninstr, const int* code, const double* params, int nin, const void* const* in,
                      const long* istrides, int nout, void* const* out, const int* out_regs,
                      const long* ostrides, int ndim, const long* shape, void* stream);
int hb_ewise_prog_f64(int ninstr, const int* code, const double* params, int nin, const void* const* in,
                      const long* istrides, int nout, void* const* out, const int* out_regs,
                      const long* ostrides, int ndim, const long* shape, void* stream);
long hb_ewise_prog_image_bytes(void);
int hb_ewise_prog_build(int ninstr, const int* code, const double* params, int nin, const void* const* in,
                        const long* istrides, int nout, void* const* out, const int* out_regs,
                        const long* ostrides, int ndim, const long* shape, void* image_host, long* n_out,
                        int* reduces_out);
int hb_ewise_prog_run_f32(const void* image_dev, long n, int reduces, void* stream);
int hb_ewise_prog_run_f64(const void* image_dev, long n, int reduces, void* stream);
int hb_ewise_jit_available(void);
int hb_ewise_jit_build_f32(int ninstr, const int* code, const double* params, int nin, const void* const* in,
                           const long* istrides, int nout, void* const* out, const int* out_regs,
                           const long* ostrides, int ndim, const long* shape, void** handle_out, long* n_out,
                           int* reduces_out, char* source_out, long source_cap);
int hb_ewise_jit_build_f64(int ninstr, const int* code, const double* params, int nin, const void* const* in,
                           const long* istrides, int nout, void* const* out, const int* out_regs,
                           const long* ostrides, int ndim, const long* shape, void** handle_out, long* n_out,
                           int* reduces_out, char* source_out, long source_cap);
int hb_ewise_jit_run(void* handle, void* stream);
int hb_ewise_jit_destroy(void* handle);
enum { HB_COLPROG_SUM = -1, HB_COLPROG_MAX = -2 };
int hb_ewise_colprog_build_f32(int ninstr, const int* code, const double* params, int nin, const void* const* in,
                               const long* istrides, int nout, void* const* out, const int* out_regs,
                               const long* ostrides, long R, long n, void** handle_out, char* source_out,
                               long source_cap);
int hb_ewise_colprog_build_f64(int ninstr, const int* code, const double* params, int nin, const void* const* in,
                               const long* istrides, int nout, void* const* out, const int* out_regs,
                               const long* ostrides, long R, long n, void** handle_out, char* source_out,
                               long source_cap);

enum { HB_RED_SUM = 0, HB_RED_MAX = 1 };
int hb_reduce_f32(int op, const float* in, float* out, long K1, long R, long K2, float* ws,
                  long ws_elems, void* stream);
int hb_reduce_f64(int op, const double* in, double* out, long K1, long R, long K2, double* ws,
                  long ws_elems, void* stream);

int hb_copy_nd_f32(const float* in, const long* istr, float* out, const long* ostr, int ndim,
                   const long* shape, void* stream);
int hb_copy_nd_f64(const double* in, const long* istr, double* out, const long* ostr, int ndim,
                   const long* shape, void* stream);

int hb_fill_f32(float* out, long n, double v, void* stream);
int hb_fill_f64(double* out, long n, double v, void* stream);

int hb_gather_rows_f32(const float* src, long nsrc, long row, const long* idx, const long* perm,
                       long n, float* dst, int* err, void* stream);
int hb_gather_rows_f64(const double* src, long nsrc, long row, const long* idx, const long* perm,
                       long n, double* dst, int* err, void* stream);
int hb_gather_rows_multi_f32(int narr, const float* const* srcs, const long* rows, float* const* dsts,
                             long nsrc, const long* idx, const long* perm, long n, int* err, void* stream);
int hb_gather_rows_multi_f64(int narr, const double* const* srcs, const long* rows, double* const* dsts,
                             long nsrc, const long* idx, const long* perm, long n, int* err, void* stream);

int hb_gather_rows_multi_draw_f32(int narr, const float* const* srcs, const long* rows, float* const* dsts,
                                  long nsrc, uint64_t* state, long nlanes, long lo, long hi, long* idx_out,
                                  const long* perm, long n, int* err, void* stream);
int hb_gather_rows_multi_draw_f64(int narr, const double* const* srcs, const long* rows, double* const* dsts,
                                  long nsrc, uint64_t* state, long nlanes, long lo, long hi, long* idx_out,
                                  const long* perm, long n, int* err, void* stream);

int hb_matutil_f32(const float* in, float* out, long B, long R, long C, int mode, long lower,
                   long upper, double alpha, void* stream);
int hb_matutil_f64(const double* in, double* out, long B, long R, long C, int mode, long lower,
                   long upper, double alpha, void* stream);

int hb_rng_init(uint64_t* state, long nlanes, uint64_t seed, uint64_t stream_id, void* stream);
int hb_rng_normal_f32(uint64_t* state, long nlanes, float* out, long n, void* stream);
int hb_rng_normal_f64(uint64_t* state, long nlanes, double* out, long n, void* stream);
int hb_rng_randint(uint64_t* state, long nlanes, long* out, long n, long lo, long hi, void* stream);

int hb_diag_sample_kl_fwd_f32(const float* mu, const float* s, const float* u_in, uint64_t* rng,
                              long rng_lanes, float* u_out, float* x, float* kl, long n, long L,
                              long ld_mu, long ld_s, float* ws, void* stream);
int hb_diag_sample_kl_fwd_f64(const double* mu, const double* s, const double* u_in, uint64_t* rng,
                              long rng_lanes, double* u_out, double* x, double* kl, long n, long L,
                              long ld_mu, long ld_s, double* ws, void* stream);
int hb_diag_sample_kl_bwd_f32(const float* s, const float* u, const float* x, const float* xbar,
                              const float* klbar, float* mubar, float* sbar, long n, long L, long ld_s,
                              long ld_out, void* stream);
int hb_diag_sample_kl_bwd_f64(const double* s, const double* u, const double* x, const double* xbar,
                              const double* klbar, double* mubar, double* sbar, long n, long L, long ld_s,
                              long ld_out, void* stream);
int hb_fullrank_sample_kl_fwd_f32(const float* mu, const float* S, const float* u_in, uint64_t* rng,
                                  long rng_lanes, float* u_out, float* x, float* kl, long rows,
                                  long size, int packed, float* ws, void* stream);
int hb_fullrank_sample_kl_fwd_f64(const double* mu, const double* S, const double* u_in,
                                  uint64_t* rng, long rng_lanes, double* u_out, double* x,
                                  double* kl, long rows, long size, int packed, double* ws,
                                  void* stream);
int hb_fullrank_one_launch_shape(long rows, long size);
int hb_fullrank_sample_kl_fwd1_f32(const float* mu, const float* S, const float* u_in, uint64_t* rng,
                                   long rng_lanes, float* u_out, float* x, float* kl, long rows, long size,
                                   int packed, float* ws, unsigned* sync, void* stream);
int hb_fullrank_sample_kl_fwd1_f64(const double* mu, const double* S, const double* u_in, uint64_t* rng,
                                   long rng_lanes, double* u_out, double* x, double* kl, long rows, long size,
                                   int packed, double* ws, unsigned* sync, void* stream);
int hb_fullrank_sample_kl_bwd_f32(const float* S, const float* u, const float* x, const float* xbar,
                                  const float* klbar, float* mubar, float* Sbar, long rows,
                                  long size, int packed, void* stream);
int hb_fullrank_sample_kl_bwd_f64(const double* S, const double* u, const double* x,
                                  const double* xbar, const double* klbar, double* mubar,
                                  double* Sbar, long rows, long size, int packed, void* stream);
int hb_vec_to_tri_f32(const float* v, float* tri, long B, long N, void* stream);
int hb_vec_to_tri_f64(const double* v, double* tri, long B, long N, void* stream);
int hb_tri_to_vec_f32(const float* tri, float* v, long B, long N, void* stream);
int hb_tri_to_vec_f64(const double* tri, double* v, long B, long N, void* stream);

enum { HB_KERN_RBF = 0, HB_KERN_CSYM_RBF = 1, HB_KERN_SQDIST = 2 ,
       HB_KERN_KBAR_SYMMETRIC = 256  };
int hb_gram_fwd_f32(int kind, const float* X, long sX, const float* X2, long sX2, const float* ell,
                    long sEll, long dl, float* K, long B, long n, long n2, long d, double diag_add,
                    void* stream);
int hb_gram_fwd_f64(int kind, const double* X, long sX, const double* X2, long sX2,
                    const double* ell, long sEll, long dl, double* K, long B, long n, long n2, long d,
                    double diag_add, void* stream);
int hb_gram_bwd_f32(int kind, const float* X, long sX, const float* X2, long sX2, const float* ell,
                    long sEll, long dl, const float* Kbar, float* Xbar, float* X2bar, float* ellbar,
                    long B, long n, long n2, long d, float* ws, void* stream);
int hb_gram_bwd_f64(int kind, const double* X, long sX, const double* X2, long sX2,
                    const double* ell, long sEll, long dl, const double* Kbar, double* Xbar,
                    double* X2bar, double* ellbar, long B, long n, long n2, long d, double* ws,
                    void* stream);

enum {
  HB_MM_LOWER_OUT = 1,
  HB_MM_TRIL_OUT = 2,
  HB_MM_PHI_OUT = 4,
  HB_MM_SYM_OUT = 8,
  HB_MM_ACTGRAD = 16   ,
  HB_MM_SYMLOW_OUT = 32,
  HB_MM_COLSUM_B = 64
};
enum { HB_ACT_NONE = 0, HB_ACT_SIGMOID = 1, HB_ACT_RELU = 2, HB_ACT_TANH = 3 };
int hb_matmul_f32(const float* A, const float* B, float* C, long batch, long M, long N, long K,
                  long lda, long ldb, long ldc, long sA, long sB, long sC, int transA, int transB,
                  double alpha, double beta, const float* bias, long sBias, int act, int flags,
                  float* ws, long ws_elems, void* stream);
int hb_matmul_f64(const double* A, const double* B, double* C, long batch, long M, long N, long K,
                  long lda, long ldb, long ldc, long sA, long sB, long sC, int transA, int transB,
                  double alpha, double beta, const double* bias, long sBias, int act, int flags,
                  double* ws, long ws_elems, void* stream);

int hb_matmul_colsum_f32(const float* A, const float* B, float* C, float* colsum, long M, long N, long K, long lda, long ldb,
                         long ldc, float* ws, long ws_elems, void* stream);
int hb_matmul_colsum_f64(const double* A, const double* B, double* C, double* colsum, long M, long N, long K, long lda,
                         long ldb, long ldc, double* ws, long ws_elems, void* stream);

int hb_mlp2_sample_supported(long n, long din, long hid, long nout, long rng_lanes, int has_u);
long hb_mlp2_sample_ws_elems(long n, long din, long hid);
int hb_mlp2_sample_fwd_f32(const float* y, const float* w0, const float* b0, const float* w1, const float* b1, int act,
                           const float* u_in, uint64_t* rng, long rng_lanes, float* x, float* kl, float* u_out, float* o,
                           long n, long din, long hid, float* ws, void* stream);
int hb_mlp2_sample_bwd_f32(const float* y, const float* w0, const float* b0, const float* w1, int act, const float* o,
                           const float* u, const float* x, const float* xbar, const float* klbar, float* dw0, float* db0,
                           float* dw1, float* db1, long n, long din, long hid, float* ws, void* stream);

int hb_cholesky_f32(const float* A, float* L, long B, long M, int* info, void* stream);
int hb_cholesky_f64(const double* A, double* L, long B, long M, int* info, void* stream);

long hb_cholesky_inverse_ws_elems(long B, long M, int elem_bytes);
int hb_cholesky_persistent_shape(long B, long M, int elem_bytes);
int hb_gram_cholesky_inverse_f32(int kind, const float* X, long sX, const float* ell, long sEll, long dl, long d,
                                 double diag_add, float* L, float* W, long B, long M, int* info, float* ws,
                                 float* Wfrag, int frag_bf16x3, void* stream);
int hb_cholesky_inverse_f32(const float* A, float* L, float* W, long B, long M, int* info, float* ws,
                            float* Wfrag, int frag_bf16x3, void* stream);
int hb_cholesky_inverse_f64(const double* A, double* L, double* W, long B, long M, int* info,
                            double* ws, double* Wfrag, int frag_bf16x3, void* stream);
int hb_trinv_f32(const float* L, float* W, long B, long M, float* ws, void* stream);
int hb_trinv_f64(const double* L, double* W, long B, long M, double* ws, void* stream);

enum { HB_SGP_NEGLECTED = 0, HB_SGP_DIAGONAL = 1, HB_SGP_FULLRANK = 2  };
enum { HB_SGP_S_DIAG = 0, HB_SGP_S_TRIL = 1 };
enum { HB_PREC_NATIVE = 0, HB_PREC_BF16X3 = 1 };
long hb_sgp_ws_elems(long E, long n, long M, long d, long P);
int hb_sgp_strip_path(long E, long n, long M, long d, long P, int prec);
int hb_sgp_fwd_f32(int kind, int mode, const float* x, long sx, const float* z, const float* ell,
                   long dl, const float* W, const float* Wfrag, int prec, const float* u,
                   const float* eps_in, uint64_t* rng, long rng_lanes, float* eps_out, float* A,
                   float* A_frag, float* f, float* v, long E, long n, long M, long d, long P, float* ws,
                   void* stream);
int hb_sgp_fwd_f64(int kind, int mode, const double* x, long sx, const double* z, const double* ell,
                   long dl, const double* W, const double* Wfrag, int prec, const double* u,
                   const double* eps_in, uint64_t* rng, long rng_lanes, double* eps_out, double* A,
                   double* A_frag, double* f, double* v, long E, long n, long M, long d, long P,
                   double* ws, void* stream);
long hb_sgp_head_units(long E, long n, long M, long d, long P, int prec, int has_wfrag, int draw, long rng_lanes);
int hb_sgp_fwd_gauss_f32(int kind, int mode, const float* x, long sx, const float* z, const float* ell, long dl,
                         const float* W, const float* Wfrag, int prec, const float* u, const float* eps_in,
                         uint64_t* rng, long rng_lanes, float* eps_out, float* A, float* A_frag, float* f, float* v,
                         long E, long n, long M, long d, long P, float* ws, const float* y, const float* scale,
                         const float* var, double post, float* dmu, float* fbar, float* head_part, long units,
                         void* stream);
int hb_sgp_rider_supported(long E, long n, long M, long d, long P, int prec, int has_wfrag, int draw, long rng_lanes);
int hb_sgp_rider_begin(void);
int hb_sgp_rider_pending(void);
int hb_sgp_rider_flush(void* stream);
int hb_matmul_gram_vjp_ok(long M, long K, long batch, long d);
long hb_matmul_gram_vjp_ws_elems(long batch, long M, long d);
int hb_matmul_gram_vjp_f32(const float* A, const float* B, float* C, long batch, long M, long K, long lda, long ldb,
                           long ldc, long sA, long sB, long sC, int transA, int transB, const float* X, long sX,
                           const float* ell, long sEll, long dl, long d, float* Xbar, float* ell_partial,
                           float* part, unsigned* counters, void* stream);
int hb_gram_ell_fold_f32(const float* partial, long rows, long d, long dl, long groups, float* ellbar, void* stream);
int hb_gram_ell_fold_f64(const double* partial, long rows, long d, long dl, long groups, double* ellbar, void* stream);
long hb_matmul_gauss_units(long n, long K, long N);
int hb_matmul_gauss_f32(const float* A, long lda, const float* B, long ldb, const float* bias, const float* y,
                        const float* scale, const float* var, double post, float* dmu, float* fbar, float* part,
                        long units, long n, long K, long N, void* stream);
int hb_gauss_ll_fold_f32(const float* partial, long nb, float* ll, float* dscale, float* dvar, void* stream);
int hb_gauss_ll_fold_f64(const double* partial, long nb, double* ll, double* dscale, double* dvar, void* stream);
int hb_sgp_A_f32(int kind, const float* x, long sx, const float* z, const float* ell, long dl,
                 const float* W, const float* Wfrag, int prec, float* A, long E, long n, long M, long d,
                 void* stream);
int hb_sgp_A_f64(int kind, const double* x, long sx, const double* z, const double* ell, long dl,
                 const double* W, const double* Wfrag, int prec, double* A, long E, long n, long M,
                 long d, void* stream);
long hb_sgp_predict_ws_elems(long E, long n, long M, long d, long P, int s_kind, int has_wfrag, int dtype_bytes);
int hb_sgp_predict_f32(int kind, const float* x, long sx, const float* z, const float* ell, long dl, const float* W,
                       const float* Wfrag, const float* m, const float* s, int s_kind, int mode, double jitter, float* mean,
                       float* var, long E, long n, long M, long d, long P, float* ws, void* stream);
int hb_sgp_predict_f64(int kind, const double* x, long sx, const double* z, const double* ell, long dl, const double* W,
                       const double* Wfrag, const double* m, const double* s, int s_kind, int mode, double jitter,
                       double* mean, double* var, long E, long n, long M, long d, long P, double* ws, void* stream);
long hb_sgp_predict_cov_ws_elems(long E, long n, long M, long P, int s_kind, int dtype_bytes);
int hb_sgp_predict_cov_f32(int kind, const float* x, long sx, const float* z, const float* ell, long dl, const float* W,
                           const float* Wfrag, const float* s, int s_kind, int mode, double jitter, float* cov, long E, long n,
                           long M, long d, long P, float* ws, void* stream);
int hb_sgp_predict_cov_f64(int kind, const double* x, long sx, const double* z, const double* ell, long dl, const double* W,
                           const double* Wfrag, const double* s, int s_kind, int mode, double jitter, double* cov, long E,
                           long n, long M, long d, long P, double* ws, void* stream);
long hb_sgp_stats_ws_elems(long N, long M, long d, long P, int dtype_bytes);
int hb_sgp_stats_f32(int kind, const float* X, const float* Y, const float* z, const float* ell, long dl, const float* W,
                     const float* Wfrag, double* Phi, double* b, double* yy, double* a2sum, long N, long M, long d, long P,
                     float* ws, void* stream);
int hb_sgp_stats_f64(int kind, const double* X, const double* Y, const double* z, const double* ell, long dl, const double* W,
                     const double* Wfrag, double* Phi, double* b, double* yy, double* a2sum, long N, long M, long d, long P,
                     double* ws, void* stream);
long hb_sgp_select_ws_elems(long N, long M, long d, int dtype_bytes);
int hb_sgp_select_f32(int kind, const float* X, const float* ell, long dl, long N, long M, long d, double threshold, long* idx,
                      float* pivots, long* count, double* trace, float* ws, void* stream);
int hb_sgp_select_f64(int kind, const double* X, const double* ell, long dl, long N, long M, long d, double threshold,
                      long* idx, double* pivots, long* count, double* trace, double* ws, void* stream);
long hb_sgp_kgrad_ws_elems(long N, long M, long d, long P);
int hb_sgp_kgrad_f32(int kind, const float* X, const float* Y, const double* z, const double* ell, long dl, const double* Q,
                     const double* R, double* zbar, double* ellbar, long N, long M, long d, long P, double* ws, void* stream);
int hb_sgp_kgrad_f64(int kind, const double* X, const double* Y, const double* z, const double* ell, long dl, const double* Q,
                     const double* R, double* zbar, double* ellbar, long N, long M, long d, long P, double* ws, void* stream);
int hb_sgp_bwd_f32(int kind, int mode, const float* x, long sx, const float* z, const float* ell,
                   long dl, const float* W, const float* Wfrag, int prec, const float* u, const float* eps,
                   const float* A, const float* A_frag, const float* v, const float* fbar, float* Kbar,
                   float* Kbar_frag, float* Lbar, float* ubar, float* zbar, float* ellbar, float* xbar,
                   long E, long n, long M, long d, long P, float* ws, void* stream);
int hb_sgp_bwd_f64(int kind, int mode, const double* x, long sx, const double* z, const double* ell,
                   long dl, const double* W, const double* Wfrag, int prec, const double* u,
                   const double* eps, const double* A, const double* A_frag, const double* v,
                   const double* fbar, double* Kbar, double* Kbar_frag, double* Lbar, double* ubar,
                   double* zbar, double* ellbar, double* xbar, long E, long n, long M, long d, long P,
                   double* ws, void* stream);

int hb_adam_step_f32(float* theta, const float* g, float* m, float* v, long n, double lr, double b1,
                     double b2, double eps, double gscale, long* t, int tick, const int* info,
                     long n_info, const float* dpflag, long* fail, void* stream);
int hb_adam_step_f64(double* theta, const double* g, double* m, double* v, long n, double lr,
                     double b1, double b2, double eps, double gscale, long* t, int tick,
                     const int* info, long n_info, const double* dpflag, long* fail, void* stream);

int hb_side_push_gather_draw_f32(int narr, const float* const* srcs, const long* rows, float* const* dsts, long nsrc,
                                 uint64_t* state, long nlanes, long lo, long hi, long* idx_out, const long* perm,
                                 long n, int* err, void* stream);
int hb_side_push_diag_fwd_f32(const float* mu, const float* s, const float* u_in, uint64_t* rng, long rng_lanes,
                              float* u_out, float* x, float* kl, long n, long L, long ld_mu, long ld_s, float* ws,
                              void* stream);
int hb_side_push_diag_bwd_f32(const float* s, const float* u, const float* x, const float* xbar, const float* klbar,
                              float* mubar, float* sbar, long n, long L, long ld_s, long ld_out, void* stream);
int hb_side_pending(void);
int hb_side_flush(void* stream);
int hb_side_discard(void);

int hb_chain_begin(void);
int hb_chain_end(void* stream);
int hb_chain_discard(void);
int hb_chain_source(char* out, long cap);
int hb_chain_compile_dry(void);

#define HB_COMM_ID_BYTES 128
int hb_comm_available(void);
int hb_comm_unique_id(char* id128);
int hb_comm_init(const char* id128, int rank, int world, void** comm_out);
int hb_comm_destroy(void* comm);
int hb_allreduce_sum_f32(float* buf, long n, void* comm, void* stream);
int hb_allreduce_sum_f64(double* buf, long n, void* comm, void* stream);
int hb_dp_pack_f32(float* tail, const float* objective, const int* info, long n_info, void* stream);
int hb_dp_pack_f64(double* tail, const double* objective, const int* info, long n_info, void* stream);

#ifdef __cplusplus
}
#endif
#endif
```

Before: 41.27 million samples/s.

## Hoist chained-kernel global loads ahead of dependencies using byte-span hazard tracking

Each chained job now records the byte span and read/write role of every pointer. When a chain holds an Adam step, a new hoisting code generator uses these spans to issue the loads of later jobs (Adam operands, fold partials, ell partials) at kernel start. Values that earlier jobs will produce are forwarded through shared-memory windows and mirror slots. This hides global-memory latency inside the single fused chain kernel, at the cost of more shared memory, more registers and a more complex generator. An optional clock64 stamp probe and an accessor for it are also added.

```diff
diff --git a/henbun_amd/_lib.py b/henbun_amd/_lib.py
--- a/henbun_amd/_lib.py
+++ b/henbun_amd/_lib.py
@@ -68,6 +68,7 @@
     "hb_chain_discard": [],
     "hb_chain_source": [P, L],
     "hb_chain_compile_dry": [],
+    "hb_chain_stamps": [P, L],
     "hb_comm_available": [],
     "hb_comm_unique_id": [P],
     "hb_comm_init": [P, I, I, P],
diff --git a/henbun_amd/csrc/adam.hip b/henbun_amd/csrc/adam.hip
--- a/henbun_amd/csrc/adam.hip
+++ b/henbun_amd/csrc/adam.hip
@@ -43,6 +43,10 @@
       j.p[0] = theta, j.p[1] = g, j.p[2] = m, j.p[3] = v, j.p[4] = t, j.p[5] = info, j.p[6] = dpflag, j.p[7] = fail;
       j.l[0] = n, j.l[1] = n_info, j.l[2] = tick;
       j.d[0] = lr, j.d[1] = b1, j.d[2] = b2, j.d[3] = eps, j.d[4] = gscale;
+      const long nb = n * (long)sizeof(T);
+      j.span(0, nb, HB_CHAIN_RW), j.span(1, nb, HB_CHAIN_READ), j.span(2, nb, HB_CHAIN_RW), j.span(3, nb, HB_CHAIN_RW);
+      j.span(4, sizeof(long), HB_CHAIN_RW), j.span(5, n_info * (long)sizeof(int), HB_CHAIN_READ);
+      j.span(6, sizeof(T), HB_CHAIN_READ), j.span(7, 2 * sizeof(long), HB_CHAIN_RW);
       return hb_chain_push(j, stream);
     }
     const int crc = hb_chain_flush(stream);
diff --git a/henbun_amd/csrc/chain.cuh b/henbun_amd/csrc/chain.cuh
--- a/henbun_amd/csrc/chain.cuh
+++ b/henbun_amd/csrc/chain.cuh
@@ -12,6 +12,8 @@
 #define HB_CHAIN_ELL_MAX_N 16384
 #define HB_CHAIN_GLL_FOLD_MAX_N 4096
 
+enum { HB_CHAIN_READ = 1, HB_CHAIN_WRITE = 2, HB_CHAIN_RW = 3 };
+
 struct HbChainJob {
   int kind = 0, is64 = 0;
   const void* p[HB_PROG_MAX_IN + HB_PROG_MAX_OUT] = {};
@@ -19,6 +21,12 @@
   double d[8] = {};
   ProgArgs prog;
   int reduces = 0;
+  long ext[HB_PROG_MAX_IN + HB_PROG_MAX_OUT] = {};
+  unsigned char role[HB_PROG_MAX_IN + HB_PROG_MAX_OUT] = {};
+  void span(int k, long bytes, int r) {
+    ext[k] = p[k] != nullptr && bytes > 0 ? bytes : 0;
+    role[k] = (unsigned char)r;
+  }
 };
 
 bool hb_chain_recording();
diff --git a/henbun_amd/csrc/chain_bodies.cuh b/henbun_amd/csrc/chain_bodies.cuh
--- a/henbun_amd/csrc/chain_bodies.cuh
+++ b/henbun_amd/csrc/chain_bodies.cuh
@@ -3,13 +3,38 @@
 
 #pragma clang fp contract(off)
 
-template <typename T>
-__device__ __forceinline__ int adam_step_blocked(const long* t, const int* info, long n_info, const T* dpflag,
-                                                 long* fail, bool record) {
+__device__ __forceinline__ long hb_opaque_zero() {
+  int z = 0;
+  asm volatile("" : "+v"(z));
+  return (long)z;
+}
+
+template <typename T>
+struct HbAdamStatus {
+  long tnow, fail0;
+  T dpf;
+  int w0;
+};
+template <typename T>
+__device__ __forceinline__ void hb_adam_status_load(const long* t, const int* info, long n_info, const T* dpflag, const long* fail,
+                                                    HbAdamStatus<T>& s) {
+  const long z = hb_opaque_zero();
+  const long* fp = fail != nullptr ? fail : t;
+  const T* dp = dpflag != nullptr ? dpflag : reinterpret_cast<const T*>(t);
+  const int* ip = n_info > 0 ? info + ((long)threadIdx.x < n_info ? (long)threadIdx.x : n_info - 1) : reinterpret_cast<const int*>(t);
+  s.tnow = t[z];
+  s.fail0 = fp[z];
+  s.dpf = dp[z];
+  s.w0 = ip[z];
+}
+template <typename T>
+__device__ __forceinline__ int hb_adam_status_blocked(const HbAdamStatus<T>& s, const long* t, const int* info, long n_info,
+                                                      const T* dpflag, long* fail, bool record) {
   int bad = 0, what = 0;
-  if (fail != nullptr && fail[0] != 0) bad = 1;
-  if (dpflag != nullptr && dpflag[0] != (T)0) { bad = 1; what = -1; }
-  for (long i = threadIdx.x; i < n_info; i += blockDim.x) {
+  if (fail != nullptr && s.fail0 != 0) bad = 1;
+  if (dpflag != nullptr && s.dpf != (T)0) { bad = 1; what = -1; }
+  if ((long)threadIdx.x < n_info && s.w0 != 0) { bad = 1; what = s.w0; }
+  for (long i = (long)threadIdx.x + blockDim.x; i < n_info; i += blockDim.x) {
     const int w = info[i];
     if (w != 0) { bad = 1; what = w; }
   }
@@ -28,6 +53,78 @@
   }
   return any;
 }
+template <typename T>
+__device__ __forceinline__ int adam_step_blocked(const long* t, const int* info, long n_info, const T* dpflag,
+                                                 long* fail, bool record) {
+  HbAdamStatus<T> s;
+  hb_adam_status_load<T>(t, info, n_info, dpflag, fail, s);
+  return hb_adam_status_blocked<T>(s, t, info, n_info, dpflag, fail, record);
+}
+
+template <typename T, int D>
+struct HbAdamOps {
+  T g[D], m[D], v[D], th[D];
+};
+template <typename T, int D>
+__device__ __forceinline__ void hb_adam_load_tmv(const T* theta, const T* m, const T* v, long n, long i0, long stride,
+                                                 HbAdamOps<T, D>& o) {
+#pragma unroll
+  for (int k = 0; k < D; ++k) {
+    const long i = i0 + k * stride, ic = i < n ? i : (n > 0 ? n - 1 : 0);
+    o.m[k] = m[ic], o.v[k] = v[ic], o.th[k] = theta[ic];
+  }
+}
+template <typename T, int D>
+__device__ __forceinline__ void hb_adam_load_g(const T* g, long n, long i0, long stride, HbAdamOps<T, D>& o) {
+#pragma unroll
+  for (int k = 0; k < D; ++k) {
+    const long i = i0 + k * stride, ic = i < n ? i : (n > 0 ? n - 1 : 0);
+    o.g[k] = g[ic];
+  }
+}
+template <typename T>
+__device__ __forceinline__ T hb_adam_lr(double lr, double b1, double b2, long tnow) {
+  const double tt = (double)(tnow + 1);
+  return (T)(lr * sqrt(1.0 - pow(b2, tt)) / (1.0 - pow(b1, tt)));
+}
+struct HbNoMirror {
+  template <typename T>
+  __device__ __forceinline__ void operator()(const T*, T) const {}
+};
+
+template <typename T, int D, typename F>
+__device__ __forceinline__ void hb_adam_body(T* __restrict__ theta, const T* __restrict__ g, T* __restrict__ m, T* __restrict__ v,
+                                             long n, T lr_t, double b1, double b2, double eps, double gscale, long i0, long stride,
+                                             const HbAdamOps<T, D>& o, F on_theta) {
+  const T c1 = (T)b1, c2 = (T)b2, d1 = (T)(1.0 - b1), d2 = (T)(1.0 - b2), e = (T)eps, gs = (T)gscale;
+#pragma unroll
+  for (int k = 0; k < D; ++k) {
+    const long i = i0 + k * stride;
+    if (i < n) {
+      const T gi = o.g[k] * gs;
+      const T mi = c1 * o.m[k] + d1 * gi;
+      const T vi = c2 * o.v[k] + d2 * gi * gi;
+      m[i] = mi;
+      v[i] = vi;
+      const T ti = o.th[k] - lr_t * mi / (hb_sqrt(vi) + e);
+      theta[i] = ti;
+      on_theta(theta + i, ti);
+    }
+  }
+  for (long i = i0 + D * stride; i < n; i += stride) {
+    const T gi = g[i] * gs;
+    const T mi = c1 * m[i] + d1 * gi;
+    const T vi = c2 * v[i] + d2 * gi * gi;
+    m[i] = mi;
+    v[i] = vi;
+    const T ti = theta[i] - lr_t * mi / (hb_sqrt(vi) + e);
+    theta[i] = ti;
+    on_theta(theta + i, ti);
+  }
+}
+__device__ __forceinline__ void hb_adam_tick(long* t, long tnow) {
+  if (threadIdx.x == 0) t[0] = tnow + 1;
+}
 
 template <typename T>
 __device__ __forceinline__ void hb_adam_body(T* __restrict__ theta, const T* __restrict__ g, T* __restrict__ m, T* __restrict__ v,
@@ -35,40 +132,17 @@
                                              int tick, const int* info, long n_info, const T* dpflag, long* fail, long i0,
                                              long stride, bool record, bool owner) {
   constexpr int U = 8;
-  T g0[U], m0[U], v0[U], th0[U];
-#pragma unroll
-  for (int k = 0; k < U; ++k) {
-    const long i = i0 + k * stride, ic = i < n ? i : (n > 0 ? n - 1 : 0);
-    g0[k] = g[ic], m0[k] = m[ic], v0[k] = v[ic], th0[k] = theta[ic];
-  }
-  const long tnow = t[0];
-  if (adam_step_blocked<T>(t, info, n_info, dpflag, fail, record)) return;
-  const double tt = (double)(tnow + 1);
-  const T lr_t = (T)(lr * sqrt(1.0 - pow(b2, tt)) / (1.0 - pow(b1, tt)));
-  const T c1 = (T)b1, c2 = (T)b2, d1 = (T)(1.0 - b1), d2 = (T)(1.0 - b2), e = (T)eps, gs = (T)gscale;
-#pragma unroll
-  for (int k = 0; k < U; ++k) {
-    const long i = i0 + k * stride;
-    if (i < n) {
-      const T gi = g0[k] * gs;
-      const T mi = c1 * m0[k] + d1 * gi;
-      const T vi = c2 * v0[k] + d2 * gi * gi;
-      m[i] = mi;
-      v[i] = vi;
-      theta[i] = th0[k] - lr_t * mi / (hb_sqrt(vi) + e);
-    }
-  }
-  for (long i = i0 + U * stride; i < n; i += stride) {
-    const T gi = g[i] * gs;
-    const T mi = c1 * m[i] + d1 * gi;
-    const T vi = c2 * v[i] + d2 * gi * gi;
-    m[i] = mi;
-    v[i] = vi;
-    theta[i] -= lr_t * mi / (hb_sqrt(vi) + e);
-  }
+  HbAdamOps<T, U> o;
+  hb_adam_load_g<T, U>(g, n, i0, stride, o);
+  hb_adam_load_tmv<T, U>(theta, m, v, n, i0, stride, o);
+  HbAdamStatus<T> s;
+  hb_adam_status_load<T>(t, info, n_info, dpflag, fail, s);
+  if (hb_adam_status_blocked<T>(s, t, info, n_info, dpflag, fail, record)) return;
+  const T lr_t = hb_adam_lr<T>(lr, b1, b2, s.tnow);
+  hb_adam_body<T>(theta, g, m, v, n, lr_t, b1, b2, eps, gscale, i0, stride, o, HbNoMirror());
   if (owner && tick) {
     __syncthreads();
-    if (threadIdx.x == 0) t[0] += 1;
+    hb_adam_tick(t, s.tnow);
   }
 }
 
@@ -89,8 +163,7 @@
   }
   const long tnow = t[0];
   if (adam_step_blocked<T>(t, info, n_info, dpflag, fail, record)) return;
-  const double tt = (double)(tnow + 1);
-  const T lr_t = (T)(lr * sqrt(1.0 - pow(b2, tt)) / (1.0 - pow(b1, tt)));
+  const T lr_t = hb_adam_lr<T>(lr, b1, b2, tnow);
   const T c1 = (T)b1, c2 = (T)b2, d1 = (T)(1.0 - b1), d2 = (T)(1.0 - b2), e = (T)eps, gs = (T)gscale;
   auto upd = [&](VT gv, VT mv, VT vv, VT tv, long i) {
     VT mo, vo, to;
@@ -128,7 +201,7 @@
 __device__ __forceinline__ void hb_gauss_ll_single_body(const T* __restrict__ x, const T* __restrict__ f, const T* __restrict__ scale,
                                                         const T* __restrict__ var, long n, T* __restrict__ dmu, T* __restrict__ ll,
                                                         T* __restrict__ dscale, T* __restrict__ dvar, T* smem,
-                                                        T* __restrict__ fbar = nullptr, T post = T(0)) {
+                                                        T* __restrict__ fbar = nullptr, T post = T(0), T* mir = nullptr) {
   constexpr int PER = 16;
   const T s = scale ? scale[0] : T(1), v = var[0];
   const T iv = T(1) / v, lc = T(-0.91893853320467274178) - T(0.5) * hb_log(v);
@@ -161,6 +234,7 @@
     ll[0] = all;
     dscale[0] = asc;
     dvar[0] = avr;
+    if (mir) mir[0] = all, mir[1] = asc, mir[2] = avr;
   }
 }
 
@@ -173,11 +247,27 @@
   avr += T(-0.5) * iv + T(0.5) * g * g;
 }
 
-template <typename T>
-__device__ __forceinline__ void hb_gauss_fold_body(const T* __restrict__ partial, long nb, T* __restrict__ ll, T* __restrict__ dscale,
-                                                   T* __restrict__ dvar, T* smem) {
+template <typename T, int D>
+__device__ __forceinline__ void hb_gauss_fold_load(const T* __restrict__ partial, long nb, T (&h)[3 * D]) {
+#pragma unroll
+  for (int k = 0; k < D; ++k) {
+    const long i = (long)threadIdx.x + (long)k * blockDim.x, ic = i < nb ? i : nb - 1;
+    h[3 * k] = partial[ic], h[3 * k + 1] = partial[nb + ic], h[3 * k + 2] = partial[2 * nb + ic];
+  }
+}
+template <typename T, int D>
+__device__ __forceinline__ void hb_gauss_fold_body(const T (&h)[3 * D], const T* __restrict__ partial, long nb, T* __restrict__ ll,
+                                                   T* __restrict__ dscale, T* __restrict__ dvar, T* smem, T* mir = nullptr) {
   T a0 = T(0), a1 = T(0), a2 = T(0);
-  for (long i = threadIdx.x; i < nb; i += blockDim.x) {
+#pragma unroll
+  for (int k = 0; k < D; ++k) {
+    if ((long)threadIdx.x + (long)k * blockDim.x < nb) {
+      a0 += h[3 * k];
+      a1 += h[3 * k + 1];
+      a2 += h[3 * k + 2];
+    }
+  }
+  for (long i = (long)threadIdx.x + (long)D * blockDim.x; i < nb; i += blockDim.x) {
     a0 += partial[i];
     a1 += partial[nb + i];
     a2 += partial[2 * nb + i];
@@ -189,7 +279,15 @@
     ll[0] = a0;
     dscale[0] = a1;
     dvar[0] = a2;
-  }
+    if (mir) mir[0] = a0, mir[1] = a1, mir[2] = a2;
+  }
+}
+template <typename T>
+__device__ __forceinline__ void hb_gauss_fold_body(const T* __restrict__ partial, long nb, T* __restrict__ ll, T* __restrict__ dscale,
+                                                   T* __restrict__ dvar, T* smem, T* mir = nullptr) {
+  T h[3];
+  hb_gauss_fold_load<T, 1>(partial, nb, h);
+  hb_gauss_fold_body<T, 1>(h, partial, nb, ll, dscale, dvar, smem, mir);
 }
 
 template <typename T>
@@ -233,20 +331,66 @@
   }
 }
 
-template <typename T>
-__device__ __forceinline__ void hb_gram_ell_body(const T* __restrict__ partial, long rows, long d, long dl, long c,
-                                                 T* __restrict__ ellbar, T* smem) {
+template <typename T, int D>
+__device__ __forceinline__ void hb_gram_ell_load(const T* __restrict__ partial, long rows, long d, long dl, long c, T (&h)[D]) {
+  const long cnt = dl == 1 ? rows * d : rows;
+#pragma unroll
+  for (int k = 0; k < D; ++k) {
+    const long t = (long)threadIdx.x + (long)k * blockDim.x, tc = t < cnt ? t : cnt - 1;
+    h[k] = dl == 1 ? partial[tc] : partial[tc * d + c];
+  }
+}
+template <typename T, int D>
+__device__ __forceinline__ void hb_gram_ell_body(const T (&h)[D], const T* __restrict__ partial, long rows, long d, long dl, long c,
+                                                 T* __restrict__ ellbar, T* smem, T* mir = nullptr) {
+  const long cnt = dl == 1 ? rows * d : rows;
   T acc = T(0);
+#pragma unroll
+  for (int k = 0; k < D; ++k)
+    if ((long)threadIdx.x + (long)k * blockDim.x < cnt) acc += h[k];
   if (dl == 1) {
 #pragma unroll 4
-    for (long t = threadIdx.x; t < rows * d; t += blockDim.x) acc += partial[t];
+    for (long t = (long)threadIdx.x + (long)D * blockDim.x; t < cnt; t += blockDim.x) acc += partial[t];
   } else {
 #pragma unroll 4
-    for (long r = threadIdx.x; r < rows; r += blockDim.x) acc += partial[r * d + c];
+    for (long r = (long)threadIdx.x + (long)D * blockDim.x; r < cnt; r += blockDim.x) acc += partial[r * d + c];
   }
   acc = block_sum(acc, smem);
-  if (threadIdx.x == 0) ellbar[c] = acc;
-}
+  if (threadIdx.x == 0) {
+    ellbar[c] = acc;
+    if (mir) mir[0] = acc;
+  }
+}
+template <typename T>
+__device__ __forceinline__ void hb_gram_ell_body(const T* __restrict__ partial, long rows, long d, long dl, long c,
+                                                 T* __restrict__ ellbar, T* smem, T* mir = nullptr) {
+  T h[1];
+  hb_gram_ell_load<T, 1>(partial, rows, d, dl, c, h);
+  hb_gram_ell_body<T, 1>(h, partial, rows, d, dl, c, ellbar, smem, mir);
+}
+
+template <typename T, int D>
+__device__ __forceinline__ void hb_chain_win_load(const T* base, long n, T (&h)[D]) {
+#pragma unroll
+  for (int k = 0; k < D; ++k) {
+    const long i = (long)threadIdx.x + (long)k * blockDim.x;
+    h[k] = base[i < n ? i : hb_opaque_zero()];
+  }
+}
+template <typename T, int D>
+__device__ __forceinline__ void hb_chain_win_store(T* win, long n, const T (&h)[D]) {
+#pragma unroll
+  for (int k = 0; k < D; ++k) {
+    const long i = (long)threadIdx.x + (long)k * blockDim.x;
+    if (i < n) win[i] = h[k];
+  }
+}
+template <typename T>
+__device__ __forceinline__ void hb_chain_mirror(const T* p, T v, const T* base, long n, T* win) {
+  const long ob = (long)p - (long)base;
+  if (ob >= 0 && ob < n * (long)sizeof(T)) win[ob / (long)sizeof(T)] = v;
+}
+__device__ __forceinline__ void hb_chain_sync() { __syncthreads(); }
 
 #pragma clang fp contract(fast)
 #endif
diff --git a/henbun_amd/csrc/elementwise.hip b/henbun_amd/csrc/elementwise.hip
--- a/henbun_amd/csrc/elementwise.hip
+++ b/henbun_amd/csrc/elementwise.hip
@@ -813,6 +813,10 @@
       j.p[8] = fbar;
       j.l[0] = n;
       j.d[0] = post;
+      const long nbytes = n * (long)sizeof(T), one = sizeof(T);
+      j.span(0, nbytes, HB_CHAIN_READ), j.span(1, nbytes, HB_CHAIN_READ), j.span(2, one, HB_CHAIN_READ), j.span(3, one, HB_CHAIN_READ);
+      j.span(4, nbytes, HB_CHAIN_WRITE), j.span(5, one, HB_CHAIN_WRITE), j.span(6, one, HB_CHAIN_WRITE), j.span(7, one, HB_CHAIN_WRITE);
+      j.span(8, nbytes, HB_CHAIN_WRITE);
       return hb_chain_push(j, stream);
     }
     const int crc = hb_chain_flush(stream);
@@ -857,6 +861,8 @@
       j.is64 = sizeof(T) == 8;
       j.p[0] = partial, j.p[1] = ll, j.p[2] = dscale, j.p[3] = dvar;
       j.l[0] = nb;
+      j.span(0, 3 * nb * (long)sizeof(T), HB_CHAIN_READ);
+      j.span(1, sizeof(T), HB_CHAIN_WRITE), j.span(2, sizeof(T), HB_CHAIN_WRITE), j.span(3, sizeof(T), HB_CHAIN_WRITE);
       return hb_chain_push(j, stream);
     }
     const int crc = hb_chain_flush(stream);
diff --git a/henbun_amd/csrc/gram.hip b/henbun_amd/csrc/gram.hip
--- a/henbun_amd/csrc/gram.hip
+++ b/henbun_amd/csrc/gram.hip
@@ -157,6 +157,7 @@
         j.is64 = sizeof(T) == 8;
         j.p[0] = ws, j.p[1] = ellbar;
         j.l[0] = rows_, j.l[1] = d, j.l[2] = dl, j.l[3] = groups_;
+        j.span(0, groups_ * rows_ * d * (long)sizeof(T), HB_CHAIN_READ), j.span(1, groups_ * dl * (long)sizeof(T), HB_CHAIN_WRITE);
         return hb_chain_push(j, stream);
       }
       if (sEll != 0)
@@ -182,6 +183,7 @@
     j.is64 = sizeof(T) == 8;
     j.p[0] = partial, j.p[1] = ellbar;
     j.l[0] = rows, j.l[1] = d, j.l[2] = dl, j.l[3] = groups;
+    j.span(0, groups * rows * d * (long)sizeof(T), HB_CHAIN_READ), j.span(1, groups * dl * (long)sizeof(T), HB_CHAIN_WRITE);
     return hb_chain_push(j, stream);
   }
   if (hb_chain_recording()) {
diff --git a/henbun_amd/csrc/jit.hip b/henbun_amd/csrc/jit.hip
--- a/henbun_amd/csrc/jit.hip
+++ b/henbun_amd/csrc/jit.hip
@@ -73,11 +73,19 @@
 
 void appendf(std::string& s, const char* fmt, ...) {
   char buf[512];
-  va_list ap;
+  va_list ap, ap2;
   va_start(ap, fmt);
-  vsnprintf(buf, sizeof(buf), fmt, ap);
+  va_copy(ap2, ap);
+  const int n = vsnprintf(buf, sizeof(buf), fmt, ap);
   va_end(ap);
-  s += buf;
+  if (n >= 0 && (size_t)n < sizeof(buf)) {
+    s += buf;
+  } else if (n > 0) {
+    std::vector<char> big((size_t)n + 1);
+    vsnprintf(big.data(), big.size(), fmt, ap2);
+    s += big.data();
+  }
+  va_end(ap2);
 }
 
 std::string literal(double v) {
@@ -91,7 +99,24 @@
   return b;
 }
 
-void emit_program(std::string& s, const ProgArgs& A, const char* loop) {
+struct ProgHooks {
+  std::string in_expr[HB_PROG_MAX_IN];
+  std::string out_extra[HB_PROG_MAX_OUT];
+};
+std::string hook_text(const std::string& tmpl, const std::string& ptr, const std::string& val) {
+  std::string r;
+  for (size_t i = 0; i < tmpl.size(); ++i) {
+    if (tmpl[i] == '%' && i + 1 < tmpl.size() && (tmpl[i + 1] == 'P' || tmpl[i + 1] == 'V')) {
+      r += tmpl[i + 1] == 'P' ? ptr : val;
+      ++i;
+    } else {
+      r += tmpl[i];
+    }
+  }
+  return r;
+}
+
+void emit_program(std::string& s, const ProgArgs& A, const char* loop, const ProgHooks* hooks = nullptr) {
   for (int k = 0; k < A.nout; ++k)
     if (A.out_reg[k] & HB_PROG_SUM) appendf(s, "  T racc%d = T(0);\n", k);
   appendf(s, "  %s\n", loop);
@@ -108,6 +133,10 @@
     if (top > maxreg) maxreg = top;
   }
   for (int k = 0; k < A.nin; ++k) {
+    if (hooks && !hooks->in_expr[k].empty()) {
+      appendf(s, "    T r%d = %s;\n", k, hooks->in_expr[k].c_str());
+      continue;
+    }
     appendf(s, "    T r%d = in%d[0", k, k);
     for (int d = 0; d < A.ndim; ++d)
       if (A.istr[k][d] != 0) appendf(s, " + x%d * %ldL", d, A.istr[k][d]);
@@ -145,6 +174,14 @@
         off += b;
       }
     }
+    if (hooks && !hooks->out_extra[k].empty()) {
+      std::string ptr, val;
+      appendf(ptr, "(out%d + (%s))", k, off.c_str());
+      appendf(val, "r%d", A.out_reg[k]);
+      appendf(s, "    %s%s%s{ out%d[%s] = r%d; %s }\n", pred.empty() ? "" : "if (", pred.c_str(), pred.empty() ? "" : ") ", k, off.c_str(),
+              A.out_reg[k], hook_text(hooks->out_extra[k], ptr, val).c_str());
+      continue;
+    }
     if (pred.empty())
       appendf(s, "    out%d[%s] = r%d;\n", k, off.c_str(), A.out_reg[k]);
     else
@@ -152,8 +189,16 @@
   }
   s += "  }\n";
   for (int k = 0; k < A.nout; ++k)
-    if (A.out_reg[k] & HB_PROG_SUM)
-      appendf(s, "  { const T t = block_sum(racc%d, smem); if (threadIdx.x == 0) out%d[0] = t; }\n", k, k);
+    if (A.out_reg[k] & HB_PROG_SUM) {
+      if (hooks && !hooks->out_extra[k].empty()) {
+        char ptr[16];
+        snprintf(ptr, sizeof(ptr), "out%d", k);
+        appendf(s, "  { const T t = block_sum(racc%d, smem); if (threadIdx.x == 0) { out%d[0] = t; %s } }\n", k, k,
+                hook_text(hooks->out_extra[k], ptr, "t").c_str());
+      } else {
+        appendf(s, "  { const T t = block_sum(racc%d, smem); if (threadIdx.x == 0) out%d[0] = t; }\n", k, k);
+      }
+    }
 }
 
 std::string generate(const ProgArgs& A, const char* T, bool reduces) {
@@ -237,8 +282,15 @@
     std::vector<char> code;
     return compile_to_code(src, &code);
   }
+  int ndev = 0;
+  if (hipGetDeviceCount(&ndev) != hipSuccess) ndev = 0, (void)hipGetLastError();
   Compiled c;
-  rc = compile_source(src, &c);
+  if (ndev > 0) {
+    rc = compile_source(src, &c);
+  } else {
+    std::vector<char> code;
+    rc = compile_to_code(src, &code);
+  }
   if (rc) return rc;
   JitProgram* p = new JitProgram;
   p->A = A;
@@ -411,11 +463,23 @@
   double d[16];
 };
 
-struct ChainLaunch {
-  hipFunction_t fn = nullptr;
-};
-
-int chain_source(const std::vector<HbChainJob>& jobs, std::string* out, HbChainArgs* args, int* np_out, int* nl_out, int* nd_out) {
+constexpr int CHAIN_NSTAMP = 16;
+unsigned long long* g_chain_stamps = nullptr;
+const void* chain_stamp_buffer() { return g_chain_stamps; }
+static void chain_job_slots(const HbChainJob& j, int* p, int* l, int* d) {
+  switch (j.kind) {
+    case HB_CHAIN_PROG: *p = j.prog.nin + j.prog.nout, *l = 0, *d = 0; break;
+    case HB_CHAIN_ADAM: *p = 8, *l = 3, *d = 5; break;
+    case HB_CHAIN_GLL: *p = 9, *l = 1, *d = 1; break;
+    case HB_CHAIN_GLL_FOLD: *p = 4, *l = 1, *d = 0; break;
+    case HB_CHAIN_SGP_FINISH: *p = 6, *l = 6, *d = 0; break;
+    case HB_CHAIN_GRAM_ELL: *p = 2, *l = 4, *d = 0; break;
+    default: *p = 20, *l = 8, *d = 8; break;
+  }
+}
+
+int chain_source_plain(const std::vector<HbChainJob>& jobs, std::string* out, HbChainArgs* args, int* np_out, int* nl_out, int* nd_out,
+                       bool stamps) {
   const bool is64 = jobs[0].is64 != 0;
   std::string s;
   int np = 0, nl = 0, nd = 0;
@@ -472,6 +536,15 @@
       HB_REQUIRE(false, "hb_chain: unknown job kind %d", j.kind);
     }
     s += "  }\n";
+    if (stamps) appendf(s, "  const unsigned long long hb_st%d = clock64();\n", (int)q + 2);
+  }
+  if (stamps) {
+    HB_REQUIRE(np < 64, "hb_chain: no pointer slot left for the stamps");
+    const int ps = P(chain_stamp_buffer());
+    appendf(s, "  if (threadIdx.x == 0) {\n    unsigned long long* sb = (unsigned long long*)A.p[%d];\n    sb[0] = %dULL; sb[1] = hb_st0; sb[2] = hb_st0;\n", ps,
+            (int)jobs.size() + 2);
+    for (size_t q = 0; q < jobs.size(); ++q) appendf(s, "    sb[%d] = hb_st%d;\n", (int)q + 3, (int)q + 2);
+    s += "  }\n";
   }
   s += "}\n";
   std::string h = HB_EW_JIT_PRELUDE;
@@ -480,9 +553,388 @@
   appendf(h, "\ntypedef %s T;\nextern \"C\" __global__ void __launch_bounds__(1024) hb_jit_kernel(const HbChainArgs Ain) {\n",
           is64 ? "double" : "float");
   h += "  __shared__ T smem[16];\n  const HbChainArgs A = Ain;\n";
+  if (stamps) h += "  const unsigned long long hb_st0 = clock64();\n";
   *out = h + s;
   *np_out = np, *nl_out = nl, *nd_out = nd;
   return 0;
+}
+
+enum { CH_PLAIN = 0, CH_EXT = 1, CH_SLOT = 2, CH_WIN = 3 };
+constexpr long CHAIN_WIN_BYTES = 40960;
+constexpr int CHAIN_MAX_WIN = 8, CHAIN_MAX_SLOT = 16;
+constexpr int CHAIN_HOIST_REGS = 40;
+
+struct ChainWin {
+  int job, idx;
+  int cap;
+  std::string nexpr;
+};
+struct ChainMirror { int kind, id; };
+struct ChainCls { int kind = CH_PLAIN, id = -1; };
+
+struct ChainPlan {
+  const std::vector<HbChainJob>& jobs;
+  size_t esz;
+  std::vector<int> pbase, lbase, dbase;
+  std::vector<ChainWin> wins;
+  int nslot = 0;
+  long win_bytes = 0;
+  std::vector<std::vector<std::vector<ChainMirror>>> mirrors;
+  std::vector<std::vector<int>> slot_of;
+
+  explicit ChainPlan(const std::vector<HbChainJob>& j) : jobs(j), esz(j[0].is64 ? 8 : 4) {
+    int np = 0, nl = 0, nd = 0;
+    for (const HbChainJob& q : jobs) {
+      pbase.push_back(np), lbase.push_back(nl), dbase.push_back(nd);
+      int a, b, c;
+      chain_job_slots(q, &a, &b, &c);
+      np += a, nl += b, nd += c;
+    }
+    mirrors.assign(jobs.size(), std::vector<std::vector<ChainMirror>>(HB_PROG_MAX_IN + HB_PROG_MAX_OUT));
+    slot_of.assign(jobs.size(), std::vector<int>(HB_PROG_MAX_IN + HB_PROG_MAX_OUT, -1));
+  }
+  static bool overlap(const HbChainJob& a, int i, const HbChainJob& b, int k) {
+    const char *a0 = (const char*)a.p[i], *b0 = (const char*)b.p[k];
+    return a.ext[i] > 0 && b.ext[k] > 0 && a0 < b0 + b.ext[k] && b0 < a0 + a.ext[i];
+  }
+  int capability(int j, int k) const {
+    const HbChainJob& J = jobs[j];
+    switch (J.kind) {
+      case HB_CHAIN_PROG: return k >= J.prog.nin ? 2 : 0;
+      case HB_CHAIN_ADAM: return k == 0 ? 2 : 0;
+      case HB_CHAIN_GLL: return k >= 5 && k <= 7 ? 1 : 0;
+      case HB_CHAIN_GLL_FOLD: return k >= 1 && k <= 3 ? 1 : 0;
+      case HB_CHAIN_GRAM_ELL: return k == 1 && J.ext[1] == (long)esz ? 1 : 0;
+      default: return 0;
+    }
+  }
+  int slot(int j, int k) {
+    if (slot_of[j][k] >= 0) return slot_of[j][k];
+    const int kind = jobs[j].kind;
+    const bool triple = kind == HB_CHAIN_GLL || kind == HB_CHAIN_GLL_FOLD;
+    const int first = kind == HB_CHAIN_GLL ? 5 : kind == HB_CHAIN_GLL_FOLD ? 1 : k, count = triple ? 3 : 1;
+    if (nslot + count > CHAIN_MAX_SLOT) return -1;
+    for (int c = 0; c < count; ++c) slot_of[j][first + c] = nslot + c;
+    nslot += count;
+    return slot_of[j][k];
+  }
+  bool external(int q, int k) const {
+    for (int j = 0; j < q; ++j)
+      for (int o = 0; o < HB_PROG_MAX_IN + HB_PROG_MAX_OUT; ++o)
+        if ((jobs[j].role[o] & HB_CHAIN_WRITE) && overlap(jobs[q], k, jobs[j], o)) return false;
+    return true;
+  }
+  ChainCls classify(int q, int k, long n, const std::string& nexpr) {
+    ChainCls c;
+    const HbChainJob& Q = jobs[q];
+    if (Q.ext[k] <= 0) return c;
+    std::vector<std::pair<int, int>> prod;
+    for (int j = 0; j < q; ++j)
+      for (int o = 0; o < HB_PROG_MAX_IN + HB_PROG_MAX_OUT; ++o)
+        if ((jobs[j].role[o] & HB_CHAIN_WRITE) && overlap(Q, k, jobs[j], o)) prod.push_back({j, o});
+    if (prod.empty()) {
+      c.kind = CH_EXT;
+      return c;
+    }
+    if (prod.size() == 1 && n == 1) {
+      const int j = prod[0].first, o = prod[0].second;
+      if (jobs[j].p[o] == Q.p[k] && jobs[j].ext[o] == (long)esz && capability(j, o) >= 1) {
+        const int sl = slot(j, o);
+        if (sl < 0) return c;
+        mirrors[j][o].push_back({CH_SLOT, sl});
+        c.kind = CH_SLOT, c.id = sl;
+        return c;
+      }
+    }
+    int cap = 1;
+    while (cap < n) cap *= 2;
+    if ((int)wins.size() >= CHAIN_MAX_WIN || n < 1 || win_bytes + (long)cap * (long)esz > CHAIN_WIN_BYTES) return c;
+    for (const auto& jo : prod) {
+      const long off = (const char*)jobs[jo.first].p[jo.second] - (const char*)Q.p[k];
+      if (capability(jo.first, jo.second) != 2 || off % (long)esz != 0) return c;
+    }
+    const int w = (int)wins.size();
+    wins.push_back({q, k, cap, nexpr});
+    win_bytes += (long)cap * (long)esz;
+    for (const auto& jo : prod) mirrors[jo.first][jo.second].push_back({CH_WIN, w});
+    c.kind = CH_WIN, c.id = w;
+    return c;
+  }
+  std::string mirror_text(int j, int k) const {
+    std::string t;
+    for (const ChainMirror& m : mirrors[j][k]) {
+      if (m.kind == CH_SLOT) {
+        appendf(t, "hb_slot[%d] = %%V; ", m.id);
+      } else {
+        const ChainWin& W = wins[m.id];
+        appendf(t, "hb_chain_mirror<T>(%%P, %%V, (const T*)A.p[%d], %s, hb_win%d); ", pbase[W.job] + W.idx, W.nexpr.c_str(), m.id);
+      }
+    }
+    return t;
+  }
+  std::string mir_arg(int j, int k) const {
+    char b[48];
+    if (slot_of[j][k] >= 0)
+      snprintf(b, sizeof(b), "hb_slot + %d", slot_of[j][k]);
+    else
+      snprintf(b, sizeof(b), "(T*)nullptr");
+    return b;
+  }
+};
+
+int chain_source_hoist(const std::vector<HbChainJob>& jobs, std::string* out, HbChainArgs* args, int* np_out, int* nl_out, int* nd_out,
+                       bool stamps) {
+  const bool is64 = jobs[0].is64 != 0;
+  const int NQ = (int)jobs.size();
+  int np = 0, nl = 0, nd = 0;
+  auto P = [&](const void* v) { HbChainArgs& a = *args; a.p[np] = v; return np++; };
+  auto L = [&](long v) { HbChainArgs& a = *args; a.l[nl] = v; return nl++; };
+  auto D = [&](double v) { HbChainArgs& a = *args; a.d[nd] = v; return nd++; };
+  ChainPlan plan(jobs);
+  struct JobCls {
+    ChainCls in[HB_PROG_MAX_IN];
+    bool hoist = false;
+    ChainCls g;
+    bool tmv_ext = false, st_ext = false, part_ext = false;
+    int depth = 1;
+  };
+  std::vector<JobCls> cls(NQ);
+  for (int q = 0; q < NQ; ++q) {
+    const HbChainJob& j = jobs[q];
+    HB_REQUIRE((j.is64 != 0) == is64, "hb_chain: jobs of different element types in one chain");
+    JobCls& c = cls[q];
+    if (j.kind == HB_CHAIN_PROG) {
+      const ProgArgs& G = j.prog;
+      c.hoist = G.n >= 1 && G.n <= 1024;
+      for (int k = 0; k < G.nin && c.hoist; ++k) {
+        long n = 1;
+        for (int d = 0; d < G.ndim; ++d) n += G.istr[k][d] * (long)(G.shape[d] - 1);
+        char b[32];
+        snprintf(b, sizeof(b), "%ldL", n);
+        c.in[k] = plan.classify(q, k, n, b);
+      }
+    } else if (j.kind == HB_CHAIN_ADAM) {
+      c.depth = (int)((j.l[0] + 1023) / 1024);
+      c.tmv_ext = plan.external(q, 0) && plan.external(q, 2) && plan.external(q, 3);
+      c.st_ext = plan.external(q, 4) && plan.external(q, 5) && plan.external(q, 6) && plan.external(q, 7);
+      char b[32];
+      snprintf(b, sizeof(b), "A.l[%d]", plan.lbase[q]);
+      c.g = plan.classify(q, 1, j.l[0], b);
+    } else if (j.kind == HB_CHAIN_GLL_FOLD) {
+      c.part_ext = plan.external(q, 0);
+      c.depth = (int)((j.l[0] + 1023) / 1024);
+    } else if (j.kind == HB_CHAIN_GRAM_ELL) {
+      c.part_ext = plan.external(q, 0);
+      c.depth = (int)(((j.l[2] == 1 ? j.l[0] * j.l[1] : j.l[0]) + 1023) / 1024);
+    }
+    if (c.depth < 1) c.depth = 1;
+  }
+  int held = 0;
+  for (const ChainWin& W : plan.wins) held += (W.cap > 1024 ? W.cap / 1024 : 1) * (is64 ? 2 : 1);
+  auto fits = [&](int values) {
+    const int regs = values * (is64 ? 2 : 1);
+    if (held + regs > CHAIN_HOIST_REGS) return false;
+    held += regs;
+    return true;
+  };
+  for (int pass = 0; pass < 2; ++pass) {
+    for (int q = 0; q < NQ; ++q) {
+      const HbChainJob& j = jobs[q];
+      JobCls& c = cls[q];
+      if ((j.kind == HB_CHAIN_ADAM) != (pass == 0)) continue;
+      if (j.kind == HB_CHAIN_ADAM) {
+        if (c.tmv_ext && !fits(3 * c.depth)) c.tmv_ext = false;
+        if (c.g.kind == CH_EXT && !fits(c.depth)) c.g.kind = CH_PLAIN;
+      } else if (j.kind == HB_CHAIN_GLL_FOLD) {
+        if (c.part_ext && !fits(3 * c.depth)) c.part_ext = false;
+      } else if (j.kind == HB_CHAIN_GRAM_ELL) {
+        if (c.part_ext && !fits(c.depth)) c.part_ext = false;
+      } else if (j.kind == HB_CHAIN_PROG) {
+        for (int k = 0; k < j.prog.nin; ++k)
+          if (c.in[k].kind == CH_EXT && !fits(1)) c.in[k].kind = CH_PLAIN;
+      }
+    }
+  }
+  std::string top, s;
+  for (size_t w = 0; w < plan.wins.size(); ++w) {
+    const ChainWin& W = plan.wins[w];
+    const int dw = W.cap > 1024 ? W.cap / 1024 : 1;
+    appendf(top, "  T hb_wf%d[%d]; hb_chain_win_load<T, %d>((const T*)A.p[%d], %s, hb_wf%d);\n", (int)w, dw, dw, plan.pbase[W.job] + W.idx,
+            W.nexpr.c_str(), (int)w);
+  }
+  for (int q = 0; q < NQ; ++q) {
+    const HbChainJob& j = jobs[q];
+    const JobCls& c = cls[q];
+    HB_REQUIRE(np + 20 <= 64 && nl + 8 <= 48 && nd + 8 <= 16, "hb_chain: argument block exhausted");
+    HB_REQUIRE(np == plan.pbase[q] && nl == plan.lbase[q] && nd == plan.dbase[q], "hb_chain: argument slots out of step");
+    if (q) s += "  __syncthreads();\n";
+    s += "  {\n";
+    if (j.kind == HB_CHAIN_PROG) {
+      const ProgArgs& G = j.prog;
+      ProgHooks hooks;
+      for (int k = 0; k < G.nin; ++k) appendf(s, "  const T* in%d = (const T*)A.p[%d];\n", k, P(j.p[k]));
+      for (int k = 0; k < G.nout; ++k) appendf(s, "  T* out%d = (T*)A.p[%d];\n", k, P(j.p[G.nin + k]));
+      bool any_ext = false;
+      for (int k = 0; k < G.nin; ++k) any_ext = any_ext || c.in[k].kind == CH_EXT;
+      if (any_ext) {
+        appendf(top, "  const long h%di = (long)threadIdx.x < %ldL ? (long)threadIdx.x : 0L;\n  long h%drem = h%di;\n", q, G.n, q, q);
+        for (int d = G.ndim - 1; d >= 0; --d) {
+          if (d == 0)
+            appendf(top, "  const long h%dx%d = h%drem;\n", q, d, q);
+          else
+            appendf(top, "  const long h%dx%d = h%drem %% %dL; h%drem /= %dL;\n", q, d, q, G.shape[d], q, G.shape[d]);
+        }
+      }
+      for (int k = 0; k < G.nin; ++k) {
+        char b[256];
+        if (c.in[k].kind == CH_EXT) {
+          bool uniform = true;
+          for (int d = 0; d < G.ndim; ++d) uniform = uniform && G.istr[k][d] == 0;
+          appendf(top, "  const T h%d_%d = ((const T*)A.p[%d])[%s", q, k, plan.pbase[q] + k, uniform ? "hb_opaque_zero()" : "0");
+          for (int d = 0; d < G.ndim; ++d)
+            if (G.istr[k][d] != 0) appendf(top, " + h%dx%d * %ldL", q, d, G.istr[k][d]);
+          top += "];\n";
+          snprintf(b, sizeof(b), "h%d_%d", q, k);
+          hooks.in_expr[k] = b;
+        } else if (c.in[k].kind == CH_SLOT) {
+          snprintf(b, sizeof(b), "hb_slot[%d]", c.in[k].id);
+          hooks.in_expr[k] = b;
+        } else if (c.in[k].kind == CH_WIN) {
+          std::string e;
+          appendf(e, "hb_win%d[0", c.in[k].id);
+          for (int d = 0; d < G.ndim; ++d)
+            if (G.istr[k][d] != 0) appendf(e, " + x%d * %ldL", d, G.istr[k][d]);
+          hooks.in_expr[k] = e + "]";
+        }
+      }
+      for (int k = 0; k < G.nout; ++k) hooks.out_extra[k] = plan.mirror_text(q, G.nin + k);
+      char loop[96];
+      snprintf(loop, sizeof(loop), "for (long i = threadIdx.x; i < %ldL; i += 1024) {", G.n);
+      emit_program(s, G, loop, &hooks);
+    } else if (j.kind == HB_CHAIN_ADAM) {
+      const int p0 = P(j.p[0]); P(j.p[1]); P(j.p[2]); P(j.p[3]); P(j.p[4]); P(j.p[5]); P(j.p[6]); P(j.p[7]);
+      const int l0 = L(j.l[0]); L(j.l[1]); L(j.l[2]);
+      const int d0 = D(j.d[0]); D(j.d[1]); D(j.d[2]); D(j.d[3]); D(j.d[4]);
+      std::string status, tmv, lr, gload;
+      appendf(top, "  HbAdamOps<T, %d> h%do; HbAdamStatus<T> h%ds;\n", c.depth, q, q);
+      appendf(status, "  hb_adam_status_load<T>((const long*)A.p[%d], (const int*)A.p[%d], A.l[%d], (const T*)A.p[%d], (const long*)A.p[%d], h%ds);\n",
+              p0 + 4, p0 + 5, l0 + 1, p0 + 6, p0 + 7, q);
+      appendf(tmv, "  hb_adam_load_tmv<T, %d>((const T*)A.p[%d], (const T*)A.p[%d], (const T*)A.p[%d], A.l[%d], (long)threadIdx.x, 1024L, h%do);\n",
+              c.depth, p0, p0 + 2, p0 + 3, l0, q);
+      appendf(lr, "  const T h%dlr = hb_adam_lr<T>(A.d[%d], A.d[%d], A.d[%d], h%ds.tnow);\n", q, d0, d0 + 1, d0 + 2, q);
+      if (c.g.kind == CH_WIN)
+        appendf(gload, "  hb_adam_load_g<T, %d>(hb_win%d, A.l[%d], (long)threadIdx.x, 1024L, h%do);\n", c.depth, c.g.id, l0, q);
+      else
+        appendf(gload, "  hb_adam_load_g<T, %d>((const T*)A.p[%d], A.l[%d], (long)threadIdx.x, 1024L, h%do);\n", c.depth, p0 + 1, l0, q);
+      (c.st_ext ? top : s) += status;
+      (c.tmv_ext ? top : s) += tmv;
+      (c.g.kind == CH_EXT ? top : s) += gload;
+      const int lr_slot = c.st_ext && q > 0 && plan.nslot < CHAIN_MAX_SLOT ? plan.nslot++ : -1;
+      if (lr_slot >= 0) {
+        appendf(top, "  if ((threadIdx.x >> 6) == 15) {\n  %s    if ((threadIdx.x & 63) == 0) hb_slot[%d] = h%dlr;\n  }\n", lr.c_str(), lr_slot, q);
+        appendf(s, "  const T h%dlr = hb_slot[%d];\n", q, lr_slot);
+      } else {
+        (c.st_ext ? top : s) += lr;
+      }
+      std::string fn = "HbNoMirror()";
+      const std::string mt = plan.mirror_text(q, 0);
+      if (!mt.empty()) fn = "[&](const T* hp, T hv) { " + hook_text(mt, "hp", "hv") + "}";
+      appendf(s, "  if (!hb_adam_status_blocked<T>(h%ds, (const long*)A.p[%d], (const int*)A.p[%d], A.l[%d], (const T*)A.p[%d], (long*)A.p[%d], true)) {\n",
+              q, p0 + 4, p0 + 5, l0 + 1, p0 + 6, p0 + 7);
+      appendf(s, "    hb_adam_body<T>((T*)A.p[%d], (const T*)A.p[%d], (T*)A.p[%d], (T*)A.p[%d], A.l[%d], h%dlr, A.d[%d], A.d[%d], A.d[%d], "
+                 "A.d[%d], (long)threadIdx.x, 1024L, h%do, %s);\n",
+              p0, p0 + 1, p0 + 2, p0 + 3, l0, q, d0 + 1, d0 + 2, d0 + 3, d0 + 4, q, fn.c_str());
+      appendf(s, "    if (A.l[%d]) hb_adam_tick((long*)A.p[%d], h%ds.tnow);\n  }\n", l0 + 2, p0 + 4, q);
+    } else if (j.kind == HB_CHAIN_GLL) {
+      const int p0 = P(j.p[0]); P(j.p[1]); P(j.p[2]); P(j.p[3]); P(j.p[4]); P(j.p[5]); P(j.p[6]); P(j.p[7]); P(j.p[8]);
+      const int l0 = L(j.l[0]);
+      const int d0 = D(j.d[0]);
+      appendf(s, "  hb_gauss_ll_single_body<T>((const T*)A.p[%d], (const T*)A.p[%d], (const T*)A.p[%d], (const T*)A.p[%d], A.l[%d], "
+                 "(T*)A.p[%d], (T*)A.p[%d], (T*)A.p[%d], (T*)A.p[%d], smem, (T*)A.p[%d], (T)A.d[%d], %s);\n",
+              p0, p0 + 1, p0 + 2, p0 + 3, l0, p0 + 4, p0 + 5, p0 + 6, p0 + 7, p0 + 8, d0, plan.mir_arg(q, 5).c_str());
+    } else if (j.kind == HB_CHAIN_GLL_FOLD) {
+      const int p0 = P(j.p[0]); P(j.p[1]); P(j.p[2]); P(j.p[3]);
+      const int l0 = L(j.l[0]);
+      if (c.part_ext) {
+        appendf(top, "  T h%dp[%d]; hb_gauss_fold_load<T, %d>((const T*)A.p[%d], A.l[%d], h%dp);\n", q, 3 * c.depth, c.depth, p0, l0, q);
+        appendf(s, "  hb_gauss_fold_body<T, %d>(h%dp, (const T*)A.p[%d], A.l[%d], (T*)A.p[%d], (T*)A.p[%d], (T*)A.p[%d], smem, %s);\n", c.depth, q,
+                p0, l0, p0 + 1, p0 + 2, p0 + 3, plan.mir_arg(q, 1).c_str());
+      } else {
+        appendf(s, "  hb_gauss_fold_body<T>((const T*)A.p[%d], A.l[%d], (T*)A.p[%d], (T*)A.p[%d], (T*)A.p[%d], smem, %s);\n", p0, l0, p0 + 1,
+                p0 + 2, p0 + 3, plan.mir_arg(q, 1).c_str());
+      }
+    } else if (j.kind == HB_CHAIN_SGP_FINISH) {
+      const int p0 = P(j.p[0]); P(j.p[1]); P(j.p[2]); P(j.p[3]); P(j.p[4]); P(j.p[5]);
+      const int l0 = L(j.l[0]); L(j.l[1]); L(j.l[2]); L(j.l[3]); L(j.l[4]); L(j.l[5]);
+      appendf(s, "  hb_sgp_finish_body<T>((const T*)A.p[%d], (int)A.l[%d], (const T*)A.p[%d], (uint64_t*)A.p[%d], A.l[%d], (T*)A.p[%d], "
+                 "(T*)A.p[%d], (T*)A.p[%d], A.l[%d], A.l[%d], A.l[%d], (int)A.l[%d], (long)threadIdx.x, 1024L);\n",
+              p0, l0, p0 + 1, p0 + 2, l0 + 1, p0 + 3, p0 + 4, p0 + 5, l0 + 2, l0 + 3, l0 + 4, l0 + 5);
+    } else if (j.kind == HB_CHAIN_GRAM_ELL) {
+      const int p0 = P(j.p[0]); P(j.p[1]);
+      const int l0 = L(j.l[0]); L(j.l[1]); L(j.l[2]); L(j.l[3]);
+      const std::string mir = plan.mir_arg(q, 1);
+      if (c.part_ext) {
+        appendf(top, "  T h%dp[%d]; hb_gram_ell_load<T, %d>((const T*)A.p[%d], A.l[%d], A.l[%d], A.l[%d], 0L, h%dp);\n", q, c.depth, c.depth, p0,
+                l0, l0 + 1, l0 + 2, q);
+        appendf(s, "  hb_gram_ell_body<T, %d>(h%dp, (const T*)A.p[%d], A.l[%d], A.l[%d], A.l[%d], 0L, (T*)A.p[%d], smem, %s);\n", c.depth, q, p0,
+                l0, l0 + 1, l0 + 2, p0 + 1, mir.c_str());
+      }
+      appendf(s, "  for (long grp = 0; grp < A.l[%d]; ++grp)\n    for (long c = %s; c < A.l[%d]; ++c)\n"
+                 "      hb_gram_ell_body<T>((const T*)A.p[%d] + grp * A.l[%d] * A.l[%d], A.l[%d], A.l[%d], A.l[%d], c, "
+                 "(T*)A.p[%d] + grp * A.l[%d], smem, %s);\n",
+              l0 + 3, c.part_ext ? "(grp == 0 ? 1L : 0L)" : "0L", l0 + 2, p0, l0, l0 + 1, l0, l0 + 1, l0 + 2, p0 + 1, l0 + 2,
+              c.part_ext ? "(T*)nullptr" : mir.c_str());
+    } else {
+      HB_REQUIRE(false, "hb_chain: unknown job kind %d", j.kind);
+    }
+    s += "  }\n";
+    if (stamps) appendf(s, "  const unsigned long long hb_st%d = clock64();\n", q + 2);
+  }
+  if (stamps) {
+    HB_REQUIRE(np < 64, "hb_chain: no pointer slot left for the stamps");
+    const int ps = P(chain_stamp_buffer());
+    appendf(s, "  if (threadIdx.x == 0) {\n    unsigned long long* sb = (unsigned long long*)A.p[%d];\n    sb[0] = %dULL; sb[1] = hb_st0; sb[2] = hb_st1;\n", ps, NQ + 2);
+    for (int q = 0; q < NQ; ++q) appendf(s, "    sb[%d] = hb_st%d;\n", q + 3, q + 2);
+    s += "  }\n";
+  }
+  s += "}\n";
+  std::string h = HB_EW_JIT_PRELUDE;
+  h += "\n#define HB_JIT_OPAQUE(x) asm volatile(\"\" : \"+v\"(x))";
+  appendf(h, "\nstruct HbChainArgs { const void* p[%d]; long l[%d]; double d[%d]; };", np > 0 ? np : 1, nl > 0 ? nl : 1, nd > 0 ? nd : 1);
+  appendf(h, "\ntypedef %s T;\nextern \"C\" __global__ void __launch_bounds__(1024) hb_jit_kernel(const HbChainArgs Ain) {\n",
+          is64 ? "double" : "float");
+  h += "  __shared__ T smem[16];\n";
+  if (plan.nslot) appendf(h, "  __shared__ T hb_slot[%d];\n", plan.nslot);
+  for (size_t w = 0; w < plan.wins.size(); ++w) appendf(h, "  __shared__ T hb_win%d[%d];\n", (int)w, plan.wins[w].cap);
+  h += "  const HbChainArgs A = Ain;\n";
+  if (stamps) h += "  const unsigned long long hb_st0 = clock64();\n";
+  h += top;
+  for (size_t w = 0; w < plan.wins.size(); ++w) {
+    const ChainWin& W = plan.wins[w];
+    appendf(h, "  hb_chain_win_store<T, %d>(hb_win%d, %s, hb_wf%d);\n", W.cap > 1024 ? W.cap / 1024 : 1, (int)w, W.nexpr.c_str(), (int)w);
+  }
+  if (!plan.wins.empty()) h += "  hb_chain_sync();\n";
+  if (stamps) h += "  const unsigned long long hb_st1 = clock64();\n";
+  *out = h + s;
+  *np_out = np, *nl_out = nl, *nd_out = nd;
+  return 0;
+}
+
+int chain_source(const std::vector<HbChainJob>& jobs, std::string* out, HbChainArgs* args, int* np_out, int* nl_out, int* nd_out) {
+  const bool stamps = hb_debug_get("chain_stamps", 0) != 0;
+  bool plain = hb_debug_get("chain_hoist", 1) == 0;
+  for (const HbChainJob& j : jobs) {
+    if (j.kind != HB_CHAIN_PROG) continue;
+    for (int d = 0; d < j.prog.ndim; ++d) {
+      for (int k = 0; k < j.prog.nin; ++k) plain = plain || j.prog.istr[k][d] < 0;
+      for (int k = 0; k < j.prog.nout; ++k) plain = plain || j.prog.ostr[k][d] < 0;
+    }
+  }
+  bool has_adam = false;
+  for (const HbChainJob& j : jobs) has_adam = has_adam || j.kind == HB_CHAIN_ADAM;
+  plain = plain || !has_adam;
+  if (plain) return chain_source_plain(jobs, out, args, np_out, nl_out, nd_out, stamps);
+  return chain_source_hoist(jobs, out, args, np_out, nl_out, nd_out, stamps);
 }
 
 }
@@ -496,6 +948,8 @@
   std::string src;
   HbChainArgs args = {};
   int np = 0, nl = 0, nd = 0;
+  HB_REQUIRE(hb_debug_get("chain_stamps", 0) == 0 || g_chain_stamps != nullptr,
+             "hb_chain: chain_stamps is set but hb_chain_stamps has not been called (it allocates the stamp buffer)");
   int rc = chain_source(jobs, &src, &args, &np, &nl, &nd);
   if (rc) return rc;
   Compiled c;
@@ -513,18 +967,6 @@
   return 0;
 }
 
-static void chain_job_slots(const HbChainJob& j, int* p, int* l, int* d) {
-  switch (j.kind) {
-    case HB_CHAIN_PROG: *p = j.prog.nin + j.prog.nout, *l = 0, *d = 0; break;
-    case HB_CHAIN_ADAM: *p = 8, *l = 3, *d = 5; break;
-    case HB_CHAIN_GLL: *p = 9, *l = 1, *d = 1; break;
-    case HB_CHAIN_GLL_FOLD: *p = 4, *l = 1, *d = 0; break;
-    case HB_CHAIN_SGP_FINISH: *p = 6, *l = 6, *d = 0; break;
-    case HB_CHAIN_GRAM_ELL: *p = 2, *l = 4, *d = 0; break;
-    default: *p = 20, *l = 8, *d = 8; break;
-  }
-}
-
 int hb_chain_push(const HbChainJob& job, hipStream_t stream) {
   int np = 0, nl = 0, nd = 0;
   for (const HbChainJob& q : g_chain.jobs) {
@@ -566,6 +1008,20 @@
   const int rc = chain_source(g_chain.jobs, &src, &args, &np, &nl, &nd);
   if (rc) return rc;
   snprintf(out, (size_t)cap, "%s", src.c_str() + (sizeof(HB_EW_JIT_PRELUDE) - 1));
+  return 0;
+}
+
+extern "C" int hb_chain_stamps(unsigned long long* out, long cap) {
+  HB_REQUIRE(out && cap >= 1, "hb_chain_stamps: bad buffer");
+  out[0] = 0;
+  if (!g_chain_stamps) {
+    HB_HIP(hipMalloc((void**)&g_chain_stamps, CHAIN_NSTAMP * sizeof(unsigned long long)));
+    HB_HIP(hipMemset(g_chain_stamps, 0, CHAIN_NSTAMP * sizeof(unsigned long long)));
+  }
+  unsigned long long host[CHAIN_NSTAMP] = {};
+  HB_HIP(hipDeviceSynchronize());
+  HB_HIP(hipMemcpy(host, g_chain_stamps, sizeof(host), hipMemcpyDeviceToHost));
+  for (long k = 0; k < cap && k < CHAIN_NSTAMP; ++k) out[k] = host[k];
   return 0;
 }
 
@@ -594,11 +1050,27 @@
       j.prog = p->A;
       j.reduces = p->reduces;
       for (size_t k = 0; k < p->ptrs.size(); ++k) j.p[k] = p->ptrs[k];
+      const ProgArgs& G = p->A;
+      const long esz = p->is64 ? 8 : 4;
+      auto reach = [&](const long* str) {
+        long lo = 0, hi = 0;
+        for (int d = 0; d < G.ndim; ++d) (str[d] < 0 ? lo : hi) += str[d] * (long)(G.shape[d] - 1);
+        return std::pair<long, long>(lo, hi);
+      };
+      for (int k = 0; k < G.nin; ++k) {
+        const auto r = reach(G.istr[k]);
+        j.span(k, (r.second + 1) * esz, HB_CHAIN_READ);
+      }
+      for (int k = 0; k < G.nout; ++k) {
+        const auto r = reach(G.ostr[k]);
+        j.span(G.nin + k, ((G.out_reg[k] & HB_PROG_SUM) ? 1 : r.second + 1) * esz, HB_CHAIN_WRITE);
+      }
       return hb_chain_push(j, (hipStream_t)stream);
     }
     const int rc = hb_chain_flush((hipStream_t)stream);
     if (rc) return rc;
   }
+  HB_REQUIRE(p->fn != nullptr, "hb_ewise_jit_run: the program was built without a device and cannot be launched");
   HB_HIP(hipModuleLaunchKernel(p->fn, p->grid, 1, 1, 256, 1, 1, 0, (hipStream_t)stream, p->argv.data(), nullptr));
   return 0;
 }
diff --git a/henbun_amd/csrc/sgp.hip b/henbun_amd/csrc/sgp.hip
--- a/henbun_amd/csrc/sgp.hip
+++ b/henbun_amd/csrc/sgp.hip
@@ -1907,6 +1907,9 @@
       j.p[4] = f;
       j.p[5] = v;
       j.l[0] = gyp, j.l[1] = rng_lanes, j.l[2] = total, j.l[3] = n, j.l[4] = P, j.l[5] = mode == HB_SGP_DIAGONAL;
+      const long tb = total * (long)sizeof(T);
+      j.span(0, tb * gyp * 5, HB_CHAIN_READ), j.span(1, tb, HB_CHAIN_READ), j.span(2, 2 * rng_lanes * (long)sizeof(uint64_t), HB_CHAIN_RW);
+      j.span(3, tb, HB_CHAIN_WRITE), j.span(4, tb * P, HB_CHAIN_WRITE), j.span(5, tb, HB_CHAIN_WRITE);
       return hb_chain_push(j, stream);
     }
     const int fgrid = draw ? hb_cdiv(rng_lanes, 256) : hb_stream_grid((total + 1) / 2, 256);
diff --git a/include/henbun_hip.h b/include/henbun_hip.h
--- a/include/henbun_hip.h
+++ b/include/henbun_hip.h
@@ -340,6 +340,7 @@
 int hb_chain_discard(void);
 int hb_chain_source(char* out, long cap);
 int hb_chain_compile_dry(void);
+int hb_chain_stamps(unsigned long long* out, long cap);
 
 #define HB_COMM_ID_BYTES 128
 int hb_comm_available(void);
```

Result: faster. 42.15 million samples/s (median of 6 runs) (+2.1%).
